# Orion-AI-Lab/KuroSiwo

Measured on AMD Instinct MI355X. Metric: SAR tiles/sec (224x224, SNUNet-ECAM change-detection train step), higher is better.
Workload: dtype bf16; 1 GPU; BASELINE.json configs[1]: SNUNet-ECAM CD, 2 dates x 2-ch GRD 224x224, per-GPU batch 32, ce+dice loss, Adam lr 1e-3, fwd+loss+bwd+optimizer; global_batch=32, base_channel=32, parallelism=dp1, hip_streams=3

## Files before the change

### include/ksmi.h

```cpp
#ifndef KSMI_H
#define KSMI_H
#include <stddef.h>
#include <stdint.h>

#ifdef __cplusplus
extern "C" {
#endif

#define KSMI_ABI_VERSION 7
#define KSMI_F32 0
#define KSMI_BF16 1
#define KSMI_E_ARG (-1)
#define KSMI_E_UNSUPPORTED (-2)
#define KSMI_MAX_SRC 6
#define KSMI_MAX_CHUNKS 72

int ksmi_abi_version(void);
const char* ksmi_last_error(void);
int ksmi_set_knob(const char* name, const char* value);
int ksmi_chunk_elems(int dtype);

#define KSMI_OP_CALL 0
#define KSMI_OP_ORDER 1
#define KSMI_OP_WAIT_SIDE 2
// ... 163 lines not shown
                              void* dout_g, const void* out, const void* z, const float* mean, const float* rstd, const float* gamma,
                              void* dz, double count, int64_t npix, int C, int dtype, void* stream);
int ksmi_bn_bwd_fin_apply_add(float* partial, int rows, int Cstride, float* sums, float* dgamma, float* dbeta, int accumulate,
                              void* r_di, const void* g, const void* i, const float* mean, const float* rstd, const float* gamma,
                              float* bias_partial, int bias_rows, double count, int64_t npix, int C, int dtype, void* stream);
int ksmi_channel_sum(const void* x, float* partial, int rows, int64_t npix, int C, int dtype, void* stream);
int ksmi_colsum(const void* x, int64_t rows, int C, float* out, int accumulate, int dtype, void* stream);

int ksmi_maxpool2x2_forward(const void* x, void* y, int B, int H, int W, int C, int dtype, void* stream);
int ksmi_maxpool2x2_backward(const void* x, const void* dy, void* dx, int accumulate,
                             int B, int H, int W, int C, int dtype, void* stream);

int ksmi_ecam_pool(const void* const x[4], float* avg, float* mx, int32_t* argmax,
                   float* workspace, int B, int HW, int C, int dtype, void* stream);
size_t ksmi_ecam_pool_workspace(int B, int HW, int C);
int ksmi_ecam_mlp(const float* avg, const float* mx, const float* ca_fc1, const float* ca_fc2,
                  const float* ca1_fc1, const float* ca1_fc2, float* ca, float* ca1,
                  float* hidden , int B, int C, void* stream);
int ksmi_ecam_final_forward(const void* const x[4], const float* ca, const float* ca1, const float* wf,
                            const float* bias, float* logits, int B, int HW, int C, int ncls, int dtype, void* stream);
int ksmi_ecam_final_backward_reduce(const void* const x[4], const float* dlogits, const float* ca, const float* ca1,
                                    const float* wf, float* dca, float* dca1, float* dwf, float* dbias,
                                    float* workspace, int B, int HW, int C, int ncls, int dtype, void* stream);
size_t ksmi_ecam_bwd_workspace(int B, int HW, int C, int ncls);
int ksmi_ecam_mlp_backward(const float* avg, const float* mx, const float* hidden, const float* ca, const float* ca1,
                           const float* dca, const float* dca1, const float* ca_fc1, const float* ca_fc2,
                           const float* ca1_fc1, const float* ca1_fc2, float* davg, float* dmax,
                           float* g_ca_fc1, float* g_ca_fc2, float* g_ca1_fc1, float* g_ca1_fc2,
                           float* workspace, int B, int C, void* stream);
size_t ksmi_ecam_mlp_bwd_workspace(int B, int C);
int ksmi_ecam_final_backward_dx(void* const dx[4], const float* dlogits, const float* ca, const float* wf,
                                const float* davg, const float* dmax, const int32_t* argmax,
                                int B, int HW, int C, int ncls, int dtype, void* stream);

size_t ksmi_loss_workspace(int B, int HW);
int ksmi_ce_dice_forward(const float* logits, const int64_t* labels, const float* class_w, int with_dice,
                         float* out3, float* workspace, int B, int HW, int ignore_index, void* stream);
int ksmi_ce_dice_backward(const float* logits, const int64_t* labels, const float* class_w, int with_dice,
                          const float* workspace, const float* grad_scale ,
                          float* dlogits, int B, int HW, int ignore_index, void* stream);

#define KSMI_LOSS_DICE 1
#define KSMI_LOSS_LOVASZ 2
#define KSMI_LOSS_FOCAL 3
size_t ksmi_seg_loss_workspace(int kind, int B, int HW);
int ksmi_seg_loss_forward(int kind, const float* logits, const int64_t* labels, const float* class_w, float gamma, float* out3,
                          void* workspace, int B, int HW, int ignore_index, void* stream);
int ksmi_seg_loss_backward(int kind, const float* logits, const int64_t* labels, const float* class_w, float gamma,
                           const void* workspace, const float* grad_scale ,
                           float* dlogits, int B, int HW, int ignore_index, void* stream);

int ksmi_argmax_confusion(const float* logits, const int64_t* labels, int64_t* pred , int64_t* cm,
                          int B, int C, int HW, int ignore_index, void* stream);
int ksmi_argmax_confusion_grouped(const float* logits, const int64_t* labels, int64_t* pred , int64_t* cm ,
                                  const int32_t* slot_a, int64_t* cms_a, const int32_t* slot_b, int64_t* cms_b,
                                  int B, int C, int HW, int ignore_index, void* stream);

int ksmi_adam_step(float* p, const float* g, float* m, float* v, int64_t n, int64_t* step_count,
                   float lr, float beta1, float beta2, float eps, float weight_decay, float grad_scale, void* stream);
int ksmi_adamw_step(float* p, const float* g, float* m, float* v, int64_t n, int64_t* step_count,
                    float lr, float beta1, float beta2, float eps, float weight_decay, float grad_scale, void* stream);
int ksmi_adam_step_mirror(float* p, const float* g, float* m, float* v, int64_t n, int64_t* step_count,
                          float lr, float beta1, float beta2, float eps, float weight_decay, float grad_scale, int decoupled,
                          void* mirror_bf16, void* stream);
int ksmi_sgd_step(float* p, const float* g, float* mom, int64_t n, int64_t* step_count,
                  float lr, float momentum, float weight_decay, float grad_scale, void* stream);
// ... 62 lines not shown
int ksmi_bnrelu_bwd_apply_scaled(void* dout_g, const void* out, const void* z, const float* mean, const float* rstd, const float* gamma,
                                 const float* sums, void* dz, double count, int64_t npix, int C, float alpha, int dtype, void* stream);
int ksmi_absdiff_forward(const void* a, const void* b, void* y, int64_t n, int dtype, void* stream);
int ksmi_absdiff_backward(const void* a, const void* b, const void* dy, void* da, void* db, int accumulate_a, int accumulate_b, int64_t n,
                          int dtype, void* stream);
int ksmi_sr_attention_forward_drop(const void* q, const void* kv, void* out, int B, int Nq, int Nk, int H, int C, float scale,
                                   uint32_t drop_thr, float drop_inv_keep, uint32_t site, const uint32_t* rng_state, int dtype, void* stream);
int ksmi_sr_attention_backward_drop(const void* q, const void* kv, const void* out, const void* dout, void* dq, void* dkv, void* workspace,
                                    int B, int Nq, int Nk, int H, int C, float scale, uint32_t drop_thr, float drop_inv_keep, uint32_t site,
                                    const uint32_t* rng_state, int dtype, void* stream);
int ksmi_bilinear_forward(const void* x, const void* add, void* y, int B, int Hi, int Wi, int Ho, int Wo, int C, int dtype, void* stream);
int ksmi_bilinear_backward(const void* dy, void* dx, int accumulate, int B, int Hi, int Wi, int Ho, int Wo, int C, int dtype, void* stream);
int ksmi_bn_bwd_reduce(const void* dy, const void* x, const float* mean, const float* rstd, float* partial, int rows, int64_t npix, int C,
                       int dtype, void* stream);
int ksmi_bn_bwd_apply(const void* dy, const void* r, const float* mean, const float* rstd, const float* gamma, const float* sums,
                      void* dv, int relu_mask, double count, int64_t npix, int C, int dtype, void* stream);
int ksmi_maxpool3x3s2_forward(const void* x, void* y, int B, int H, int W, int C, int dtype, void* stream);
int ksmi_maxpool3x3s2_backward(const void* x, const void* dy, void* dx, int accumulate, int B, int H, int W, int C, int dtype, void* stream);
int ksmi_maxpool3x3s2_forward_idx(const void* x, void* y, void* idx, int B, int H, int W, int C, int dtype, void* stream);
int ksmi_maxpool3x3s2_backward_idx(const void* idx, const void* dy, void* dx, int accumulate, int B, int H, int W, int C, int dtype, void* stream);
int ksmi_affine(const void* x, const float* scale, const float* shift, void* y, int64_t npix, int C, int relu, float alpha, int dtype,
                void* stream);
int ksmi_out_to_nchw(const void* x, float* y, int B, int C, int Cs, int64_t HW, int act, int dtype, void* stream);
int ksmi_dout_to_nhwc(const float* dy, const float* y, void* dx, int B, int C, int Cs, int64_t HW, int act, int dtype, void* stream);

int ksmi_cast_bf16(const float* src, void* dst, int64_t n, void* stream);
int ksmi_up_gemm_supported(int B, int H, int W, int C, int dtype);
int ksmi_up_wgrad_supported(int B, int H, int W, int C, int dtype);
int ksmi_up_pack_weight(const float* wt, void* wb, int C, void* stream);
#define KSMI_UP_PACK_MAX 16
int ksmi_up_pack_weights_batched(const float* const* wt, void* const* wb, const int* C, int n, void* stream);
int ksmi_up_forward(const void* x, const void* wb, const float* bias, void* y, int B, int H, int W, int C, void* stream);
int ksmi_up_dgrad(const void* dy, const void* wb, void* dx, int accumulate, int B, int H, int W, int C, void* stream);
size_t ksmi_up_wgrad_workspace(int B, int H, int W, int C);
int ksmi_up_wgrad(const void* x, const void* dy, float* workspace, float* grad, int accumulate, int B, int H, int W, int C, void* stream);

int ksmi_gemm_nt(const void* x, int x_rs, const void* w, int w_rs, const float* bias, const void* resid, int r_rs, void* y, int y_rs,
                 int rows, int K, int N, void* stream);
int ksmi_gemm_nn(const void* dy, int dy_rs, const void* w, int w_rs, void* dx, int dx_rs, int rows, int K, int N, int accumulate, void* stream);

int ksmi_bmm_f32(const float* a, const float* b, const float* bias, float* c, int nb1, int nb2, int M, int N, int K,
                 const int64_t* a_strides, const int64_t* b_strides, const int64_t* c_strides, float alpha, int accumulate, void* stream);
int ksmi_softmax_rows_f32(const float* x, float* y, int64_t rows, int n, float scale, void* stream);
int ksmi_softmax_rows_backward_f32(const float* y, const float* dy, float* dx, int64_t rows, int n, float scale, void* stream);
int ksmi_semantic_tokens_forward(const void* x, const float* wa, const float* pos, float* tokens, float* stats, int B, int dates, int N,
                                 int C, int L, int dtype, void* stream);
int ksmi_semantic_tokens_backward(const void* x, const float* wa, const float* stats, const float* dtokens, void* dx, float* dwa_partial,
                                  int B, int dates, int N, int C, int L, int accumulate, int dtype, void* stream);
int ksmi_token_cross_forward(const void* x, const float* gamma, const float* beta, const float* A, const float* Bv, const float* bo, void* y,
                             int B, int dates, int N, int C, int heads, int L, float scale, int dtype, void* stream);
size_t ksmi_token_cross_bwd_workspace(int B, int dates, int N);
int ksmi_token_cross_backward(const void* x, const float* gamma, const float* beta, const float* A, const float* Bv, void* g, float* dA,
                              float* dBv, float* dgamma, float* dbeta, float* dbo, int accumulate_ln, int accumulate_bo, float* workspace,
                              int B, int dates, int N, int C, int heads, int L, float scale, int dtype, void* stream);

int ksmi_sar_preprocess(const float* x, const float* mean, const float* stdv, float* y, int B, int C, int64_t HW, float clamp_input, void* stream);
int ksmi_augment_views(const float* x, const int32_t* params, const int32_t* fallback, const float* mean, const float* stdv, float* y, int B, int C,
                       int H, int W, float clamp_input, uint32_t mult_thr, float mult_lo, float mult_hi, uint32_t gauss_thr, float gauss_var_lo,
                       float gauss_var_hi, uint32_t cut_thr, int cut_holes, int cut_h, int cut_w, int op_order, const uint32_t* rng_state,
                       void* stream);
int ksmi_augment_masks(const void* x, void* y, const int32_t* params, const int32_t* fallback, int32_t* count, int B, int H, int W, int elem_bytes,
                       void* stream);

typedef struct ksmi_tiff_info {
  int32_t width, height, bands;
  int32_t bits, sample_format;
// ... 26 lines not shown
```

### kurosiwo_amd/_lib.py

```python
import ctypes as C
import os

_HERE = os.path.dirname(os.path.abspath(__file__))
LIB_PATH = os.path.join(_HERE, "libksmi.so")

KSMI_F32, KSMI_BF16 = 0, 1
LOSS_DICE, LOSS_LOVASZ, LOSS_FOCAL = 1, 2, 3
MAX_SRC, MAX_CHUNKS = 6, 72
ABI_VERSION = 7


class KsmiError(RuntimeError):
    pass


class Src(C.Structure):
    _fields_ = [("ptr", C.c_void_p), ("scale", C.c_void_p), ("shift", C.c_void_p),
                ("C", C.c_int32), ("c_off", C.c_int32), ("c_len", C.c_int32), ("relu", C.c_int32)]


class Dst(C.Structure):
    _fields_ = [("ptr", C.c_void_p), ("C", C.c_int32), ("c_off", C.c_int32), ("n_begin", C.c_int32),
                ("n_len", C.c_int32), ("accumulate", C.c_int32), ("pad_", C.c_int32)]

# ... 96 lines not shown
    "ksmi_bn_finalize": (_i, [_vp, _i, _i, _i, _d, _vp, _vp, _vp, _vp, _vp, _f, _f, _i, _vp, _vp, _vp, _vp, _vp]),
    "ksmi_bn_add_relu": (_i, [_vp, _vp, _vp, _vp, _vp, _i64, _i, _i, _vp]),
    "ksmi_bn_fused_supported": (_i, [_i, _i, _i]),
    "ksmi_bn_fused_max_rows": (_i, []),
    "ksmi_bn_fin_add_relu": (_i, [_vp, _i, _i, _i, _d, _vp, _vp, _vp, _vp, _vp, _f, _f, _vp, _vp, _vp, _vp, _vp, _vp, _vp, _vp, _i, _i, _i, _i, _vp]),
    "ksmi_bn_bwd_fin_apply_gated": (_i, [_vp, _i, _i, _vp, _vp, _vp, _i, _vp, _vp, _vp, _vp, _vp, _vp, _d, _i64, _i, _i, _vp]),
    "ksmi_bnrelu_bwd_fin_apply": (_i, [_vp, _i, _i, _vp, _vp, _vp, _i, _vp, _vp, _vp, _vp, _vp, _vp, _vp, _d, _i64, _i, _i, _vp]),
    "ksmi_bn_bwd_fin_apply_add": (_i, [_vp, _i, _i, _vp, _vp, _vp, _i, _vp, _vp, _vp, _vp, _vp, _vp, _vp, _i, _d, _i64, _i, _i, _vp]),
    "ksmi_bnrelu_bwd_reduce": (_i, [_vp, _vp, _vp, _vp, _vp, _vp, _i, _i64, _i, _i, _vp]),
    "ksmi_reduce_rows": (_i, [_vp, _i, _i, _i, _i, _vp, _vp, _vp, _i, _vp]),
    "ksmi_reduce_rows_batched": (_i, [_vp, _i, _vp]),
    "ksmi_reduce_rows_batched_wide": (_i, [_vp, _i, _i, _vp]),
    "ksmi_bnrelu_bwd_apply": (_i, [_vp, _vp, _vp, _vp, _vp, _vp, _vp, _vp, _d, _i64, _i, _i, _vp]),
    "ksmi_bn_bwd_apply_gated": (_i, [_vp, _vp, _vp, _vp, _vp, _vp, _vp, _d, _i64, _i, _i, _vp]),
    "ksmi_bn_bwd_apply_add": (_i, [_vp, _vp, _vp, _vp, _vp, _vp, _vp, _vp, _i, _d, _i64, _i, _i, _vp]),
    "ksmi_channel_sum": (_i, [_vp, _vp, _i, _i64, _i, _i, _vp]),
    "ksmi_colsum": (_i, [_vp, _i64, _i, _vp, _i, _i, _vp]),
    "ksmi_gather_rows": (_i, [_vp, _vp, _i, _vp, _vp, _i, _i, _i, _i, _i, _i, _vp]),
    "ksmi_scatter_rows": (_i, [_vp, _vp, _vp, _i, _vp, _vp, _i, _i, _i, _i, _i, _vp]),
    "ksmi_batch_sum": (_i, [_vp, _vp, _i, _i64, _i, _i, _vp]),
    "ksmi_mse_workspace": (C.c_size_t, []),
    "ksmi_mse_loss": (_i, [_vp, _vp, _vp, _f, _vp, _vp, _vp, _i64, _i, _vp]),
    "ksmi_maxpool2x2_forward": (_i, [_vp, _vp, _i, _i, _i, _i, _i, _vp]),
    "ksmi_maxpool2x2_backward": (_i, [_vp, _vp, _vp, _i, _i, _i, _i, _i, _i, _vp]),
    "ksmi_ecam_pool": (_i, [_P4, _vp, _vp, _vp, _vp, _i, _i, _i, _i, _vp]),
    "ksmi_ecam_pool_workspace": (_sz, [_i, _i, _i]),
    "ksmi_ecam_mlp": (_i, [_vp, _vp, _vp, _vp, _vp, _vp, _vp, _vp, _vp, _i, _i, _vp]),
    "ksmi_ecam_final_forward": (_i, [_P4, _vp, _vp, _vp, _vp, _vp, _i, _i, _i, _i, _i, _vp]),
    "ksmi_ecam_final_backward_reduce": (_i, [_P4, _vp, _vp, _vp, _vp, _vp, _vp, _vp, _vp, _vp, _i, _i, _i, _i, _i, _vp]),
    "ksmi_ecam_bwd_workspace": (_sz, [_i, _i, _i, _i]),
    "ksmi_ecam_mlp_backward": (_i, [_vp] * 18 + [_i, _i, _vp]),
    "ksmi_ecam_mlp_bwd_workspace": (_sz, [_i, _i]),
    "ksmi_ecam_final_backward_dx": (_i, [_P4, _vp, _vp, _vp, _vp, _vp, _vp, _i, _i, _i, _i, _i, _vp]),
    "ksmi_loss_workspace": (_sz, [_i, _i]),
    "ksmi_ce_dice_forward": (_i, [_vp, _vp, _vp, _i, _vp, _vp, _i, _i, _i, _vp]),
    "ksmi_ce_dice_backward": (_i, [_vp, _vp, _vp, _i, _vp, _vp, _vp, _i, _i, _i, _vp]),
    "ksmi_seg_loss_workspace": (_sz, [_i, _i, _i]),
    "ksmi_seg_loss_forward": (_i, [_i, _vp, _vp, _vp, _f, _vp, _vp, _i, _i, _i, _vp]),
    "ksmi_seg_loss_backward": (_i, [_i, _vp, _vp, _vp, _f, _vp, _vp, _vp, _i, _i, _i, _vp]),
    "ksmi_argmax_confusion": (_i, [_vp, _vp, _vp, _vp, _i, _i, _i, _i, _vp]),
    "ksmi_argmax_confusion_grouped": (_i, [_vp, _vp, _vp, _vp, _vp, _vp, _vp, _vp, _i, _i, _i, _i, _vp]),
    "ksmi_adam_step": (_i, [_vp, _vp, _vp, _vp, _i64, _vp, _f, _f, _f, _f, _f, _f, _vp]),
    "ksmi_adamw_step": (_i, [_vp, _vp, _vp, _vp, _i64, _vp, _f, _f, _f, _f, _f, _f, _vp]),
    "ksmi_adam_step_mirror": (_i, [_vp, _vp, _vp, _vp, _i64, _vp, _f, _f, _f, _f, _f, _f, _i, _vp, _vp]),
    "ksmi_sgd_step": (_i, [_vp, _vp, _vp, _i64, _vp, _f, _f, _f, _f, _vp]),
    "ksmi_layernorm_forward": (_i, [_vp, _vp, _vp, _vp, _vp, _vp, _i, _i, _f, _i, _vp]),
    "ksmi_layernorm_bwd_blocks": (_i, [_i]),
    "ksmi_layernorm_backward": (_i, [_vp, _vp, _vp, _vp, _vp, _vp, _i, _vp, _i, _i, _i, _vp]),
    "ksmi_gelu_forward": (_i, [_vp, _vp, _i64, _i, _vp]),
    "ksmi_gelu_backward": (_i, [_vp, _vp, _vp, _i64, _i, _vp]),
    "ksmi_add": (_i, [_vp, _vp, _vp, _i64, _i, _vp]),
    "ksmi_relu_backward": (_i, [_vp, _vp, _vp, _i64, _i, _vp]),
    "ksmi_relu_forward": (_i, [_vp, _vp, _i64, _i, _vp]),
    "ksmi_sar_preprocess": (_i, [_vp, _vp, _vp, _vp, _i, _i, _i64, C.c_float, _vp]),
    "ksmi_augment_views": (_i, [_vp, _vp, _vp, _vp, _vp, _vp, _i, _i, _i, _i, _f, C.c_uint32, _f, _f, C.c_uint32, _f, _f, C.c_uint32, _i, _i, _i, _i, _vp, _vp]),
    "ksmi_augment_masks": (_i, [_vp, _vp, _vp, _vp, _vp, _i, _i, _i, _i, _vp]),
    "ksmi_bmm_f32": (_i, [_vp, _vp, _vp, _vp, _i, _i, _i, _i, _i, C.POINTER(C.c_int64), C.POINTER(C.c_int64), C.POINTER(C.c_int64), C.c_float, _i, _vp]),
    "ksmi_softmax_rows_f32": (_i, [_vp, _vp, _i64, _i, C.c_float, _vp]),
    "ksmi_softmax_rows_backward_f32": (_i, [_vp, _vp, _vp, _i64, _i, C.c_float, _vp]),
    "ksmi_semantic_tokens_forward": (_i, [_vp, _vp, _vp, _vp, _vp, _i, _i, _i, _i, _i, _i, _vp]),
    "ksmi_semantic_tokens_backward": (_i, [_vp, _vp, _vp, _vp, _vp, _vp, _i, _i, _i, _i, _i, _i, _i, _vp]),
    "ksmi_token_cross_forward": (_i, [_vp, _vp, _vp, _vp, _vp, _vp, _vp, _i, _i, _i, _i, _i, _i, C.c_float, _i, _vp]),
    "ksmi_token_cross_bwd_workspace": (_sz, [_i, _i, _i]),
    "ksmi_token_cross_backward": (_i, [_vp, _vp, _vp, _vp, _vp, _vp, _vp, _vp, _vp, _vp, _vp, _i, _i, _vp, _i, _i, _i, _i, _i, _i, C.c_float, _i, _vp]),
    "ksmi_tiff_info_read": (_i, [C.c_char_p, C.POINTER(TiffInfo)]),
    "ksmi_tiff_read_f32": (_i, [C.c_char_p, _vp, _i64, C.POINTER(TiffInfo)]),
    "ksmi_tiff_read_native": (_i, [C.c_char_p, _vp, _i64, C.POINTER(TiffInfo)]),
    "ksmi_tile_batch_read": (_i, [C.POINTER(C.c_char_p), _i, _vp, _i, _i, _i]),
    "ksmi_tile_batch_read_bands": (_i, [C.POINTER(C.c_char_p), _i, _vp, _i, _i, _i, _i]),
    "ksmi_tiles_fill_nodata": (_i, [_vp, _i, _i, _i, _i]),
    "ksmi_cast_bf16": (_i, [_vp, _vp, _i64, _vp]),
    "ksmi_up_gemm_supported": (_i, [_i, _i, _i, _i, _i]),
    "ksmi_up_wgrad_supported": (_i, [_i, _i, _i, _i, _i]),
    "ksmi_up_pack_weight": (_i, [_vp, _vp, _i, _vp]),
    "ksmi_up_pack_weights_batched": (_i, [_vp, _vp, _vp, _i, _vp]),
    "ksmi_up_forward": (_i, [_vp, _vp, _vp, _vp, _i, _i, _i, _i, _vp]),
    "ksmi_up_dgrad": (_i, [_vp, _vp, _vp, _i, _i, _i, _i, _i, _vp]),
    "ksmi_up_wgrad_workspace": (C.c_size_t, [_i, _i, _i, _i]),
    "ksmi_up_wgrad": (_i, [_vp, _vp, _vp, _vp, _i, _i, _i, _i, _i, _vp]),
    "ksmi_gemm_nt": (_i, [_vp, _i, _vp, _i, _vp, _vp, _i, _vp, _i, _i, _i, _i, _vp]),
    "ksmi_gemm_nn": (_i, [_vp, _i, _vp, _i, _vp, _i, _i, _i, _i, _i, _vp]),
    "ksmi_im2col": (_i, [_vp, _vp] + [_i] * 11 + [_i, _i, _vp]),
    "ksmi_col2im": (_i, [_vp, _vp, _i] + [_i] * 11 + [_i, _vp]),
    "ksmi_im2col_tc": (_i, [_vp, _vp] + [_i] * 11 + [_i, _vp]),
    "ksmi_col2im_tc": (_i, [_vp, _vp, _i] + [_i] * 11 + [_i, _vp]),
    "ksmi_weight_to_tc": (_i, [_vp, _vp, _i, _i, _i, _i, _i, _vp]),
    "ksmi_grad_from_tc": (_i, [_vp, _vp, _i, _i, _i, _i, _i, _vp]),
    "ksmi_maxpool3x3s2_forward": (_i, [_vp, _vp, _i, _i, _i, _i, _i, _vp]),
    "ksmi_maxpool3x3s2_backward": (_i, [_vp, _vp, _vp, _i, _i, _i, _i, _i, _i, _vp]),
    "ksmi_maxpool3x3s2_forward_idx": (_i, [_vp, _vp, _vp, _i, _i, _i, _i, _i, _vp]),
    "ksmi_maxpool3x3s2_backward_idx": (_i, [_vp, _vp, _vp, _i, _i, _i, _i, _i, _i, _vp]),
    "ksmi_affine": (_i, [_vp, _vp, _vp, _vp, _i64, _i, _i, C.c_float, _i, _vp]),
    "ksmi_dwconv3x3_gelu_forward": (_i, [_vp, _vp, _vp, _vp, _vp, _i, _i, _i, _i, _i, _vp]),
    "ksmi_dwconv3x3_gelu_forward_drop": (_i, [_vp, _vp, _vp, _vp, _vp, _i, _i, _i, _i, C.c_uint32, C.c_float, C.c_uint32, _vp, _i, _vp]),
    "ksmi_gelu_backward_drop": (_i, [_vp, _vp, _vp, _i64, C.c_uint32, C.c_float, C.c_uint32, _vp, _i, _vp]),
    "ksmi_dwconv3x3_backward_input": (_i, [_vp, _vp, _vp, _i, _i, _i, _i, _i, _vp]),
    "ksmi_dwconv3x3_wgrad": (_i, [_vp, _vp, _vp, _i, _i, _i, _i, _i, _i, _vp]),
    "ksmi_sr_attention_forward": (_i, [_vp, _vp, _vp, _i, _i, _i, _i, _i, C.c_float, _i, _vp]),
    "ksmi_sr_attention_bwd_workspace": (C.c_size_t, [_i, _i, _i, _i, _i]),
    "ksmi_sr_attention_backward": (_i, [_vp, _vp, _vp, _vp, _vp, _vp, _vp, _i, _i, _i, _i, _i, C.c_float, _i, _vp]),
    "ksmi_attention_bwd_workspace": (C.c_size_t, [_i, _i, _i, _i, _i]),
    "ksmi_rng_advance": (_i, [_vp, _vp]),
    "ksmi_bn_relu_drop2d": (_i, [_vp, _vp, _vp, _vp, _i, _i64, _i, C.c_uint32, C.c_float, C.c_uint32, _vp, _i, _vp]),
    "ksmi_reduce_rows_scaled": (_i, [_vp, _i, _i, _i, _i, _vp, _vp, _vp, _i, C.c_float, _vp]),
    "ksmi_bnrelu_bwd_apply_scaled": (_i, [_vp, _vp, _vp, _vp, _vp, _vp, _vp, _vp, _d, _i64, _i, C.c_float, _i, _vp]),
    "ksmi_absdiff_forward": (_i, [_vp, _vp, _vp, _i64, _i, _vp]),
    "ksmi_absdiff_backward": (_i, [_vp, _vp, _vp, _vp, _vp, _i, _i, _i64, _i, _vp]),
    "ksmi_dropout_apply": (_i, [_vp, _vp, _vp, _i64, _i, _i, C.c_uint32, C.c_float, C.c_uint32, C.c_uint32, C.c_float, C.c_uint32, _vp, _i, _vp]),
    "ksmi_sr_attention_forward_drop": (_i, [_vp, _vp, _vp, _i, _i, _i, _i, _i, C.c_float, C.c_uint32, C.c_float, C.c_uint32, _vp, _i, _vp]),
    "ksmi_sr_attention_backward_drop": (_i, [_vp, _vp, _vp, _vp, _vp, _vp, _vp, _i, _i, _i, _i, _i, C.c_float, C.c_uint32, C.c_float, C.c_uint32,
# ... 83 lines not shown
```

### kurosiwo_amd/csrc/gemm2.hip

```cpp
#include "common.h"
#include "../../include/ksmi.h"
#include "errors.h"
#include "igemm_epilogue.h"

namespace {

struct Gemm2P {
  const bf16_t* a; int a_rs;
  const bf16_t* w; int w_rs;
  const float* bias; const bf16_t* resid; int r_rs;
  bf16_t* out; int o_rs;
  int rows, red, cols, accumulate;
  int mtiles, ntiles;
  int map_a, map_o, up_H, up_W, up_C, bias_mod;
};

__device__ __forceinline__ size_t up_row_base(int m, int H, int W, int C) {
  const int x = m % W, t = m / W, y = t % H, b = t / H;
  return ((size_t)(b * 2 * H + 2 * y) * (size_t)(2 * W) + (size_t)(2 * x)) * (size_t)C;
}
__device__ __forceinline__ size_t up_col_off(int c, int W, int C) { return c < 2 * C ? (size_t)c : (size_t)(c - 2 * C) + (size_t)(2 * W) * (size_t)C; }


__device__ __forceinline__ void glds16(const unsigned char* src, unsigned dst_wave_base) {
  unsigned keep;
  dst_wave_base = __builtin_amdgcn_readfirstlane(dst_wave_base);
  asm volatile("s_mov_b32 %0, m0\n\ts_mov_b32 m0, %2\n\ts_nop 0\n\tglobal_load_lds_dwordx4 %1, off\n\ts_mov_b32 m0, %0"
               : "=&s"(keep) : "v"(src), "s"(dst_wave_base) : "memory");
}
__device__ __forceinline__ void vm_wait(int n) {
#define KSMI_VMW(k) case k: asm volatile("s_waitcnt vmcnt(" #k ")" ::: "memory"); break;
  switch (n) {
    KSMI_VMW(1) KSMI_VMW(2) KSMI_VMW(3) KSMI_VMW(4) KSMI_VMW(5) KSMI_VMW(6) KSMI_VMW(7) KSMI_VMW(8) KSMI_VMW(9) KSMI_VMW(10)
    KSMI_VMW(11) KSMI_VMW(12) KSMI_VMW(13) KSMI_VMW(14) KSMI_VMW(15) KSMI_VMW(16) KSMI_VMW(17) KSMI_VMW(18) KSMI_VMW(19) KSMI_VMW(20)
    KSMI_VMW(21) KSMI_VMW(22) KSMI_VMW(23) KSMI_VMW(24) KSMI_VMW(25) KSMI_VMW(26) KSMI_VMW(27) KSMI_VMW(28) KSMI_VMW(29) KSMI_VMW(30)
    default: asm volatile("s_waitcnt vmcnt(0)" ::: "memory"); break;
  }
#undef KSMI_VMW
}
__device__ __forceinline__ void lgkm_wait0() { __builtin_amdgcn_s_waitcnt(0xC07F); }
__device__ __forceinline__ void lds_barrier() {
  lgkm_wait0();
  __builtin_amdgcn_s_barrier();
  asm volatile("" ::: "memory");
}

__device__ __forceinline__ int sw_a(int row) { return (row & 1) | ((row & 2) << 2); }
__device__ __forceinline__ int sw_b(int row) { return (row & 3) << 1; }
template <int MT> __device__ __forceinline__ int sw_bt(int row) { return MT == 3 ? 0 : sw_b(row); }

template <int MT>
__device__ __forceinline__ void store_row2(const Gemm2P& p, const f32x4 (&acc)[4][MT], int mt, int m, int c0, const float* bias16) {
  if (m >= p.rows) return;
  float v[16];
#pragma unroll
  for (int t = 0; t < 4; ++t)
#pragma unroll
    for (int r = 0; r < 4; ++r) v[t * 4 + r] = acc[t][mt][r] + bias16[t * 4 + r];
  bf16_t* op = p.map_o ? p.out + up_row_base(m, p.up_H, p.up_W, p.up_C) + up_col_off(c0, p.up_W, p.up_C) : p.out + (size_t)m * p.o_rs + c0;
  if (p.resid) {
    float a[8], b[8];
    vec_unpack<bf16_t>(*(const u32x4*)(p.resid + (size_t)m * p.r_rs + c0), a);
    vec_unpack<bf16_t>(*(const u32x4*)(p.resid + (size_t)m * p.r_rs + c0 + 8), b);
#pragma unroll
    for (int j = 0; j < 8; ++j) { v[j] += a[j]; v[8 + j] += b[j]; }
  }
  if (p.accumulate) {
    float a[8], b[8];
    vec_unpack<bf16_t>(*(const u32x4*)op, a);
    vec_unpack<bf16_t>(*(const u32x4*)(op + 8), b);
#pragma unroll
    for (int j = 0; j < 8; ++j) { v[j] += a[j]; v[8 + j] += b[j]; }
  }
  *(u32x4*)op = vec_pack<bf16_t>(v);
  *(u32x4*)(op + 8) = vec_pack<bf16_t>(v + 8);
}

template <int MT, bool TRW, int NS>
__global__ __launch_bounds__(256, 1) void gemm2_kernel(const Gemm2P p) {
  constexpr int TM = 32 * MT, KS = 64, XB = TM * 128, WB = 128 * 128, STAGE = XB + WB;
  constexpr int NQ = STAGE / 1024, NI = NQ / 4;
  extern __shared__ __attribute__((aligned(16))) unsigned char smem[];
  const int tid = threadIdx.x, lane = tid & 63, wave = tid >> 6, g = lane >> 4, l15 = lane & 15;
  const int wn = wave >> 1, wm = wave & 1;
  const unsigned t = xcd_remap(blockIdx.x, gridDim.x);
  const int mt_i = t / p.ntiles, nt_i = t - mt_i * p.ntiles;
  const int m0 = mt_i * TM, n0 = nt_i * 128;
  const int nsteps = p.red / KS;
  const unsigned lds0 = (unsigned)(uintptr_t)smem;

  const unsigned char* src[NI];
  int step_bytes[NI];
  size_t jump[NI];
  const int jump_step = p.map_a ? (2 * p.up_C) / KS : 0x7fffffff;
#pragma unroll
  for (int i = 0; i < NI; ++i) {
    const int q = wave + 4 * i;
    jump[i] = 0;
    if (q * 8 < TM) {
      const int row = q * 8 + (lane >> 3), slot = lane & 7;
      const int chunk = slot ^ ((row >> 1) & 7);
      int m = m0 + row; if (m >= p.rows) m = p.rows - 1;
      src[i] = (const unsigned char*)(p.a + (p.map_a ? up_row_base(m, p.up_H, p.up_W, p.up_C) : (size_t)m * p.a_rs) + chunk * 8);
      step_bytes[i] = KS * 2;
      jump[i] = p.map_a ? ((size_t)(2 * p.up_W) * p.up_C - (size_t)(2 * p.up_C)) * 2 : 0;
    } else if constexpr (!TRW) {
      const int j = q * 8 - TM + (lane >> 3), slot = lane & 7;
      const int chunk = slot ^ ((j >> 1) & 7);
      const int h = j >> 6, jj = j & 63;
      int n = n0 + h * 64 + ((jj >> 2) & 3) * 16 + (jj >> 4) * 4 + (jj & 3); if (n >= p.cols) n = p.cols - 1;
      src[i] = (const unsigned char*)(p.w + (size_t)n * p.w_rs + chunk * 8);
// ... 64 lines not shown

  const int pre = nsteps < NS ? nsteps : NS;
  for (int s = 0; s < pre; ++s) issue(s, s);
  vm_wait((pre - 1) * NI);
  lds_barrier();
  u32x4 fwA[4], fxA[MT], fwB[4], fxB[MT];
  load_frags(0, 0, fwA, fxA);
  int cur = 0;
  for (int s = 0; s + 1 < nsteps; ++s) {
    lgkm_wait0();
    __builtin_amdgcn_sched_barrier(0);
    load_frags(cur, 1, fwB, fxB);
    __builtin_amdgcn_sched_barrier(0);
    mma_all(acc, fwA, fxA);
    __builtin_amdgcn_sched_barrier(0);
    if (s + NS <= nsteps) vm_wait((NS - 2) * NI); else vm_wait((nsteps - s - 2) * NI);
    lds_barrier();
    if (s + NS < nsteps) issue(s + NS, cur);
    cur = cur + 1 == NS ? 0 : cur + 1;
    load_frags(cur, 0, fwA, fxA);
    __builtin_amdgcn_sched_barrier(0);
    mma_all(acc2, fwB, fxB);
    __builtin_amdgcn_sched_barrier(0);
  }
  load_frags(cur, 1, fwB, fxB);
  mma_all(acc, fwA, fxA);
  mma_all(acc2, fwB, fxB);
#pragma unroll
  for (int a = 0; a < 4; ++a)
#pragma unroll
    for (int b = 0; b < MT; ++b) acc[a][b] += acc2[a][b];

  const int c0 = n0 + wn * 64 + g * 16;
  if (c0 >= p.cols) return;
  float bias16[16];
#pragma unroll
  for (int j = 0; j < 16; ++j) bias16[j] = p.bias ? p.bias[p.bias_mod ? (c0 + j) % p.bias_mod : c0 + j] : 0.f;
#pragma unroll
  for (int mt = 0; mt < MT; ++mt) store_row2<MT>(p, acc, mt, m0 + wm * 16 * MT + mt * 16 + l15, c0, bias16);
}

template <int MT, bool TRW, int NS>
int launch2n(const Gemm2P& p, hipStream_t st) {
  constexpr int lds = NS * (32 * MT * 128 + 128 * 128);
  static_assert(lds <= 160 * 1024, "LDS ring");
  auto kfn = gemm2_kernel<MT, TRW, NS>; KSMI_NOTE(kfn);
  static bool attr = false;
  if (!attr) { (void)hipFuncSetAttribute((const void*)kfn, hipFuncAttributeMaxDynamicSharedMemorySize, lds); attr = true; }
  hipLaunchKernelGGL(kfn, dim3(p.mtiles * p.ntiles), dim3(256), lds, st, p);
  return ksmi_check_launch(TRW ? "gemm2_nn" : "gemm2_nt");
}

struct Tile2 { int mt, ns; };
inline Tile2 pick_tile(int rows, int ntiles) {
  static const int f_mt = ksmi_knob_int("KSMI_GEMM2_MT", 0);
  static const int f_ns = ksmi_knob_int("KSMI_GEMM2_NS", 0);
  static const struct { int mt, ns, slots; double round_us; } cand[] = {
      {2, 3, 512, 13.0}, {4, 3, 256, 13.8}, {2, 2, 768, 15.5}, {3, 2, 512, 16.0}, {5, 3, 256, 16.3}, {6, 3, 256, 18.0},
      {4, 2, 512, 19.0}, {7, 3, 256, 21.0}, {8, 3, 256, 23.0}};
  Tile2 best = {4, 3}; double bc = 1e30;
  for (const auto& c : cand) {
    if ((f_mt && c.mt != f_mt) || (f_ns && f_ns <= 3 && c.ns != f_ns)) continue;
    const long wgs = (long)((rows + 32 * c.mt - 1) / (32 * c.mt)) * ntiles;
    const double cost = (double)((wgs + c.slots - 1) / c.slots) * c.round_us;
    if (cost < bc) { bc = cost; best = {c.mt, c.ns}; }
  }
  if (f_mt && bc == 1e30) best = {f_mt, f_mt >= 5 ? 3 : 2};
  if (f_ns) best.ns = f_ns;
  return best;
}

template <int MT, bool TRW>
int launch2(const Gemm2P& p, int ns, hipStream_t st) {
  constexpr int stage = 32 * MT * 128 + 128 * 128;
  if (ns <= 2) return launch2n<MT, TRW, 2>(p, st);
  if constexpr (5 * stage <= 160 * 1024) { if (ns >= 5) return launch2n<MT, TRW, 5>(p, st); }
  if constexpr (4 * stage <= 160 * 1024) { if (ns >= 4) return launch2n<MT, TRW, 4>(p, st); }
  return launch2n<MT, TRW, 3>(p, st);
}

template <bool TRW>
int dispatch2(Gemm2P& p, hipStream_t st) {
  p.ntiles = p.cols / 128;
  const Tile2 t = pick_tile(p.rows, p.ntiles);
  p.mtiles = (p.rows + 32 * t.mt - 1) / (32 * t.mt);
  switch (t.mt) {
    case 2: return launch2<2, TRW>(p, t.ns, st);
    case 3: return launch2<3, TRW>(p, t.ns, st);
    case 4: return launch2<4, TRW>(p, t.ns, st);
    case 5: return launch2<5, TRW>(p, t.ns, st);
    case 6: return launch2<6, TRW>(p, t.ns, st);
    case 7: return launch2<7, TRW>(p, t.ns, st);
    default: return launch2<8, TRW>(p, t.ns, st);
  }
}

struct Gemm2T {
  const bf16_t* a; int a_rs, a_cols;
  const bf16_t* b; int b_rs, b_cols;
  float* out; int64_t o_rs; int64_t split_stride; int accumulate;
  int rows, rows_per_split, atiles, btiles;
  const unsigned char* zero;
  float* bias; int bias_acc;
  int map_a, up_H, up_W, up_C;
  float* bias_rows; int64_t bias_rs;
};
__device__ __attribute__((aligned(64))) unsigned char gemm2_zero_page[64];
KSMI_DEVICE_SYMBOL_GETTER(gemm2_zero, gemm2_zero_page)

template <int MT, int NS, int SPL, bool BIASA = false>
__global__ __launch_bounds__(256 * SPL, 1) void gemm2_tn_kernel(const Gemm2T p) {
  static_assert(!BIASA || SPL == 1, "A-side column sums: one wave group");
  constexpr int TB = 32 * MT, KS = 64, AB = 64 * 256, BROW = TB * 2, BB = 64 * BROW, STAGE = AB + BB;
  constexpr int NQ = STAGE / 1024, NI = NQ / 4, BGM = BROW / 32 - 1, AU = 16, BU = BROW / 16;
  static_assert(NQ % 4 == 0, "whole DMA rounds");
  extern __shared__ __attribute__((aligned(16))) unsigned char smem[];
  const int tid = threadIdx.x, lane = tid & 63, wave_all = tid >> 6, g = lane >> 4, l15 = lane & 15;
  const int grp = SPL == 1 ? 0 : wave_all >> 2, wave = wave_all & 3;
  const int wn = wave >> 1, wm = wave & 1;
  const int tile = blockIdx.x, split = blockIdx.y;
  const int bt = tile / p.atiles, at = tile - bt * p.atiles;
  const int a0 = at * 128, b0 = bt * TB;
  const int wg_begin = split * p.rows_per_split;
  const int wg_end = min(p.rows, wg_begin + p.rows_per_split);
  const int steps_wg = (max(wg_end - wg_begin, 0) + KS - 1) / KS;
  const int nsteps = (steps_wg + SPL - 1) / SPL;
  const int m_begin = wg_begin + grp * nsteps * KS;
// ... 183 lines not shown
}

}

int ksmi_gemm2_nt(const void* x, int x_rs, const void* w, int w_rs, const float* bias, const void* resid, int r_rs, void* y, int y_rs,
                  int rows, int K, int N, hipStream_t st) {
  static const bool off = ksmi_knob_is_set("KSMI_GEMM2_OFF");
  if (off || K % 64 || N % 128 || rows < 64 || K < 128) return 1;
  Gemm2P p = {(const bf16_t*)x, x_rs, (const bf16_t*)w, w_rs, bias, (const bf16_t*)resid, r_rs, (bf16_t*)y, y_rs, rows, K, N, 0, 0, 0};
  return dispatch2<false>(p, st);
}

int ksmi_gemm2_nn(const void* dy, int dy_rs, const void* w, int w_rs, void* dx, int dx_rs, int rows, int K, int N, int accumulate,
                  hipStream_t st) {
  static const bool off = ksmi_knob_is_set("KSMI_GEMM2_OFF");
  if (off || N % 64 || K % 128 || rows < 64 || N < 128) return 1;
  Gemm2P p = {(const bf16_t*)dy, dy_rs, (const bf16_t*)w, w_rs, nullptr, nullptr, 0, (bf16_t*)dx, dx_rs, rows, N, K, accumulate, 0, 0};
  return dispatch2<true>(p, st);
}

int ksmi_gemm2_up_forward(const void* x, const void* wb, const float* bias, void* y, int B, int H, int W, int C, hipStream_t st) {
  if (C % 64 || C < 128 || B * H * W < 64) return 1;
  Gemm2P p = {(const bf16_t*)x, C, (const bf16_t*)wb, C, bias, nullptr, 0, (bf16_t*)y, 0, B * H * W, C, 4 * C, 0, 0, 0};
  p.map_o = 1; p.up_H = H; p.up_W = W; p.up_C = C; p.bias_mod = C;
  return dispatch2<false>(p, st);
}
int ksmi_gemm2_up_dgrad(const void* dy, const void* wb, void* dx, int accumulate, int B, int H, int W, int C, hipStream_t st) {
  if (C % 128 || C < 128 || B * H * W < 64) return 1;
  Gemm2P p = {(const bf16_t*)dy, 0, (const bf16_t*)wb, C, nullptr, nullptr, 0, (bf16_t*)dx, C, B * H * W, 4 * C, C, accumulate, 0, 0};
  p.map_a = 1; p.up_H = H; p.up_W = W; p.up_C = C;
  return dispatch2<true>(p, st);
}

template <int MT, int NS, int SPL = 1, bool BIASA = false>
static void launch_tn(dim3 grid, const Gemm2T& p, hipStream_t st) {
  constexpr int lds = SPL * NS * (64 * 256 + 64 * 64 * MT);
  static_assert(lds <= 160 * 1024, "LDS ring");
  static_assert(SPL == 1 || (4 * MT + MT) * 256 * 16 <= lds, "exchange area");
  auto kfn = gemm2_tn_kernel<MT, NS, SPL, BIASA>; KSMI_NOTE(kfn);
  static bool attr = false;
  if (!attr) { (void)hipFuncSetAttribute((const void*)kfn, hipFuncAttributeMaxDynamicSharedMemorySize, lds); attr = true; }
  hipLaunchKernelGGL(kfn, grid, dim3(256 * SPL), lds, st, p);
}

bool ksmi_gemm2_tn_spl(int tiles_times_splits, int steps_per_split) {
  static const int f = ksmi_knob_int("KSMI_TN_SPL", 0);
  if (f <= 0) return false;
  if (f == 1) return steps_per_split >= 2;
  return tiles_times_splits <= 256 && steps_per_split >= 12;
}

bool ksmi_gemm2_tn_enabled(int K, int N, int rows_per_split) {
  static const bool off = ksmi_knob_is_set("KSMI_GEMM2_OFF") || ksmi_knob_is_set("KSMI_GEMM2_TN_OFF");
  return !(off || K % 8 || N % 8 || K < 64 || N < 64 || rows_per_split % 64);
}

int ksmi_gemm2_tn(const void* x, int x_rs, const void* dy, int dy_rs, float* slab, int npad, float* grad, int64_t g_rs, int rows, int K, int N,
                  int Kslab, int nsplit, int rows_per_split, int btile, int accumulate, float* bias_grad, int bias_accumulate, hipStream_t st) {
  if (!ksmi_gemm2_tn_enabled(K, N, rows_per_split)) return 1;
  const unsigned char* const zero_page = gemm2_zero();
  if (!zero_page) return ksmi_fail(KSMI_E_UNSUPPORTED, "gemm2: zero page");
  Gemm2T p = {};
  p.rows = rows; p.rows_per_split = rows_per_split; p.zero = zero_page;
  if (nsplit == 1 && grad) {
    p.a = (const bf16_t*)x; p.a_rs = x_rs; p.a_cols = K; p.b = (const bf16_t*)dy; p.b_rs = dy_rs; p.b_cols = N;
    p.out = grad; p.o_rs = g_rs; p.split_stride = 0; p.accumulate = accumulate;
// ... 117 lines not shown
  if (rc) return rc;
  launch_up_wgrad_reduce(slab, nsplit, C, grad, accumulate, st);
  return ksmi_check_launch("up_wgrad_reduce");
}

extern "C" {
int ksmi_up_gemm_supported(int B, int H, int W, int C, int dtype) {
  static const bool off = ksmi_knob_is_set("KSMI_GEMM2_OFF");
  return !off && dtype == KSMI_BF16 && C >= 128 && C % 128 == 0 && (int64_t)B * H * W >= 64 && (int64_t)B * H * W * 112 < ((int64_t)1 << 32) ? 1 : 0;
}
int ksmi_up_wgrad_supported(int B, int H, int W, int C, int dtype) {
  static const bool off = ksmi_knob_is_set("KSMI_GEMM2_OFF");
  return !off && dtype == KSMI_BF16 && C >= 64 && C % 64 == 0 && (int64_t)B * H * W >= 64 && (int64_t)B * H * W * 112 < ((int64_t)1 << 32) ? 1 : 0;
}
int ksmi_up_pack_weight(const float* wt, void* wb, int C, void* stream) { return ksmi_gemm2_up_pack(wt, wb, C, (hipStream_t)stream); }
int ksmi_up_pack_weights_batched(const float* const* wt, void* const* wb, const int* C, int n, void* stream) {
  if (!wt || !wb || !C || n < 1 || n > KSMI_UP_PACK_MAX) return ksmi_fail(KSMI_E_ARG, "up_pack_weights_batched: 1 .. KSMI_UP_PACK_MAX tensors");
  UpPackBatch b = {};
  for (int i = 0; i < n; ++i) {
    if (!wt[i] || !wb[i] || C[i] < 1) return ksmi_fail(KSMI_E_ARG, "up_pack_weights_batched: bad entry");
    b.wt[i] = wt[i]; b.wb[i] = (bf16_t*)wb[i]; b.C[i] = C[i];
  }
  hipLaunchKernelGGL(up_pack_batched_kernel, dim3(256, n), dim3(256), 0, (hipStream_t)stream, b);
  return ksmi_check_launch("up_pack_weights_batched");
}
int ksmi_up_forward(const void* x, const void* wb, const float* bias, void* y, int B, int H, int W, int C, void* stream) {
  const int rc = ksmi_gemm2_up_forward(x, wb, bias, y, B, H, W, C, (hipStream_t)stream);
  return rc == 1 ? ksmi_fail(KSMI_E_UNSUPPORTED, "up_forward: shape not covered (ksmi_up_gemm_supported)") : rc;
}
int ksmi_up_dgrad(const void* dy, const void* wb, void* dx, int accumulate, int B, int H, int W, int C, void* stream) {
  const int rc = ksmi_gemm2_up_dgrad(dy, wb, dx, accumulate, B, H, W, C, (hipStream_t)stream);
  return rc == 1 ? ksmi_fail(KSMI_E_UNSUPPORTED, "up_dgrad: shape not covered (ksmi_up_gemm_supported)") : rc;
}
size_t ksmi_up_wgrad_workspace(int B, int H, int W, int C) { return ksmi_gemm2_up_wgrad_workspace(B, H, W, C); }
int ksmi_up_wgrad(const void* x, const void* dy, float* workspace, float* grad, int accumulate, int B, int H, int W, int C, void* stream) {
  const int rc = ksmi_gemm2_up_wgrad(x, dy, workspace, grad, accumulate, B, H, W, C, (hipStream_t)stream);
  return rc == 1 ? ksmi_fail(KSMI_E_UNSUPPORTED, "up_wgrad: shape not covered (ksmi_up_gemm_supported)") : rc;
}
}
```

### kurosiwo_amd/csrc/head.hip

```cpp
#include "common.h"
#include "../../include/ksmi.h"
#include "errors.h"

namespace {

constexpr int kThreads = 256;
constexpr int kPoolSplit = 64;
constexpr int kBwdSplit = 64;

template <typename T>
__global__ __launch_bounds__(256) void ecam_pool_kernel(const T* x0, const T* x1, const T* x2, const T* x3,
                                                        float* psum, float* pmax, int* pidx, int HW, int C) {
  constexpr int VEC = ElemTraits<T>::kVec;
  const int CV = C / VEC;
  const int npl = kThreads / CV;
  const int b = blockIdx.y, sp = blockIdx.x, S = gridDim.x;
  const int cv = threadIdx.x % CV, pl = threadIdx.x / CV;
  const bool active = (int)threadIdx.x < npl * CV;
  const int per = (HW + S - 1) / S;
  const int p0 = sp * per, p1 = min(HW, p0 + per);
  const T* xs[4] = {x0, x1, x2, x3};
  float s[5][VEC], m[5][VEC];
  int mi[5][VEC];
#pragma unroll
// ... 346 lines not shown
  int i = blockIdx.x * blockDim.x + threadIdx.x;
  if (i < C4 * H1) {
    const int j = i % H1, c = i / H1;
    float a = 0.f;
    for (int b = 0; b < B; ++b) a += ds[b * C5 + c] * (hidden[(size_t)b * 2 * HT + j] + hidden[(size_t)b * 2 * HT + HT + j]);
    gw2[i] = a;
    return;
  }
  i -= C4 * H1;
  if (i < C * H2) {
    const int j = i % H2, c = i / H2;
    float a = 0.f;
    for (int b = 0; b < B; ++b) a += ds[b * C5 + C4 + c] * (hidden[(size_t)b * 2 * HT + H1 + j] + hidden[(size_t)b * 2 * HT + HT + H1 + j]);
    gv2[i] = a;
    return;
  }
  i -= C * H2;
  if (i < H1 * C4) {
    const int c = i % C4, j = i / C4;
    float a = 0.f;
    for (int b = 0; b < B; ++b) a += dh[(b * 2 + 0) * HT + j] * avg[b * C5 + c] + dh[(b * 2 + 1) * HT + j] * mx[b * C5 + c];
    gw1[i] = a;
    return;
  }
  i -= H1 * C4;
  if (i < H2 * C) {
    const int c = i % C, j = i / C;
    float a = 0.f;
    for (int b = 0; b < B; ++b) a += dh[(b * 2 + 0) * HT + H1 + j] * avg[b * C5 + C4 + c] + dh[(b * 2 + 1) * HT + H1 + j] * mx[b * C5 + C4 + c];
    gv1[i] = a;
  }
}

template <typename T, int NCLS>
__global__ __launch_bounds__(256) void ecam_bwd_dx_kernel(T* d0, T* d1, T* d2, T* d3, const float* dl, const float* ca,
                                                          const float* wf, const float* davg, int HW, int C) {
  constexpr int VEC = ElemTraits<T>::kVec;
  extern __shared__ float sm[];
  const int b = blockIdx.y, C4 = 4 * C;
  float* weff = sm;
  float* cst = sm + NCLS * C4;
  const float inv = 1.f / (float)HW;
  for (int i = threadIdx.x; i < NCLS * C4; i += blockDim.x) weff[i] = wf[i] * ca[(size_t)b * C4 + (i % C4)];
  for (int i = threadIdx.x; i < C4; i += blockDim.x) cst[i] = (davg[(size_t)b * 5 * C + i] + davg[(size_t)b * 5 * C + C4 + (i % C)]) * inv;
  __syncthreads();
  const int CV = C / VEC, tpp = 4 * CV;
  const int ppb = blockDim.x / tpp;
  const int q = threadIdx.x % tpp, pl = threadIdx.x / tpp;
  const int s = q / CV, c0 = (q - s * CV) * VEC;
  if (pl >= ppb) return;
  float w[NCLS][VEC], k0[VEC];
#pragma unroll
  for (int j = 0; j < VEC; ++j) {
    k0[j] = cst[s * C + c0 + j];
#pragma unroll
    for (int k = 0; k < NCLS; ++k) w[k][j] = weff[k * C4 + s * C + c0 + j];
  }
  T* dst = (s == 0 ? d0 : s == 1 ? d1 : s == 2 ? d2 : d3) + (int64_t)b * HW * C + c0;
  for (int p = blockIdx.x * ppb + pl; p < HW; p += gridDim.x * ppb) {
    float d[NCLS], v[VEC];
#pragma unroll
    for (int k = 0; k < NCLS; ++k) d[k] = dl[((int64_t)b * NCLS + k) * HW + p];
#pragma unroll
    for (int j = 0; j < VEC; ++j) {
      float a = k0[j];
#pragma unroll
      for (int k = 0; k < NCLS; ++k) a += w[k][j] * d[k];
      v[j] = a;
    }
    *(u32x4*)(dst + (int64_t)p * C) = vec_pack<T>(v);
  }
}

template <typename T>
__global__ void ecam_bwd_max_scatter_kernel(T* d0, T* d1, T* d2, T* d3, const float* dmax, const int* argmax, int B, int HW, int C) {
  const int i = blockIdx.x * blockDim.x + threadIdx.x;
  if (i >= B * C) return;
  const int b = i / C, cc = i - b * C;
  T* ds[4] = {d0, d1, d2, d3};
  for (int s = 0; s < 4; ++s) {
    const int c = s * C + cc;
    T* q = ds[s] + ((int64_t)b * HW + argmax[b * 5 * C + c]) * C + cc;
    ElemTraits<T>::st(q, ElemTraits<T>::ld(q) + dmax[b * 5 * C + c]);
  }
  const int pi = argmax[b * 5 * C + 4 * C + cc];
  const float g = dmax[b * 5 * C + 4 * C + cc];
  for (int s = 0; s < 4; ++s) {
    T* q = ds[s] + ((int64_t)b * HW + pi) * C + cc;
    ElemTraits<T>::st(q, ElemTraits<T>::ld(q) + g);
  }
}

constexpr int kLossSplit = 32;
struct Px3 { float p0, p1, p2; };
__device__ __forceinline__ Px3 softmax3(float a, float b, float c, float& lse) {
  const float m = fmaxf(a, fmaxf(b, c));
  const float e0 = expf(a - m), e1 = expf(b - m), e2 = expf(c - m);
  const float s = e0 + e1 + e2;
  lse = m + logf(s);
  const float r = 1.f / s;
  return {e0 * r, e1 * r, e2 * r};
}

__global__ __launch_bounds__(256) void ce_dice_fwd_kernel(const float* logits, const int64_t* labels, const float* cw,
                                                          float* part, int HW, int ignore_index) {
  const int b = blockIdx.y, sp = blockIdx.x, S = gridDim.x;
  const int per = (HW + S - 1) / S;
  const int p0 = sp * per, p1 = min(HW, p0 + per);
  const float w0 = cw[0], w1 = cw[1], w2 = cw[2];
  const float one = 1.0f + 1e-6f, eps = 1e-6f;
  float wn = 0.f, ws = 0.f, it = 0.f, cd = 0.f;
  const float* lg = logits + (int64_t)b * 3 * HW;
  for (int p = p0 + threadIdx.x; p < p1; p += blockDim.x) {
    const float a = lg[p], bb = lg[HW + p], c = lg[2 * HW + p];
    const int64_t t = labels[(int64_t)b * HW + p];
    float lse;
    const Px3 q = softmax3(a, bb, c, lse);
    const bool valid = t != ignore_index;
    const int t0 = valid ? (int)t : 0;
    const float xt = t0 == 0 ? a : (t0 == 1 ? bb : c);
// ... 191 lines not shown
  float* pg = workspace; float* pd = pg + (size_t)B * kBwdSplit * 3 * 4 * C;
  float* gb = pd + (size_t)B * kBwdSplit * 3; float* db = gb + (size_t)B * 3 * 4 * C;
  KSMI_DT(dtype,
          hipLaunchKernelGGL((ecam_bwd_reduce_kernel<bf16_t, 3>), dim3(kBwdSplit, B), dim3(256), 0, (hipStream_t)stream,
                             (const bf16_t*)x[0], (const bf16_t*)x[1], (const bf16_t*)x[2], (const bf16_t*)x[3], dlogits, pg, pd, HW, C),
          hipLaunchKernelGGL((ecam_bwd_reduce_kernel<float, 3>), dim3(kBwdSplit, B), dim3(256), 0, (hipStream_t)stream,
                             (const float*)x[0], (const float*)x[1], (const float*)x[2], (const float*)x[3], dlogits, pg, pd, HW, C));
  int rc = ksmi_check_launch("ecam_bwd_reduce");
  if (rc) return rc;
  hipLaunchKernelGGL(ecam_bwd_finish_kernel<3>, dim3(B), dim3(256), (size_t)(3 * 4 * C + 3) * sizeof(float), (hipStream_t)stream, pg, pd, ca, ca1,
                     wf, dca, dca1, gb, db, kBwdSplit, C);
  hipLaunchKernelGGL(ecam_bwd_wf_kernel<3>, dim3((3 * 4 * C + 255) / 256), dim3(256), 0, (hipStream_t)stream, gb, db, ca, ca1, dwf, dbias, B, C);
  return ksmi_check_launch("ecam_bwd_finish");
}

size_t ksmi_ecam_mlp_bwd_workspace(int B, int C) {
  return ((size_t)B * 5 * C + (size_t)B * 2 * ((4 * C) / 16 + C / 4)) * sizeof(float);
}

int ksmi_ecam_mlp_backward(const float* avg, const float* mx, const float* hidden, const float* ca, const float* ca1,
                           const float* dca, const float* dca1, const float* ca_fc1, const float* ca_fc2, const float* ca1_fc1,
                           const float* ca1_fc2, float* davg, float* dmax, float* g_ca_fc1, float* g_ca_fc2, float* g_ca1_fc1,
                           float* g_ca1_fc2, float* workspace, int B, int C, void* stream) {
  if (C % 16 || !workspace) return ksmi_fail(KSMI_E_ARG, "ecam_mlp_backward: bad args");
  const int C4 = 4 * C, HT = C4 / 16 + C / 4;
  hipLaunchKernelGGL(ecam_mlp_bwd_kernel, dim3(B), dim3(256), (size_t)(5 * C + 2 * HT) * sizeof(float), (hipStream_t)stream, hidden, ca, ca1, dca,
                     dca1, ca_fc1, ca_fc2, ca1_fc1, ca1_fc2, davg, dmax, workspace, B, C);
  const int items = 2 * (C4 * (C4 / 16) + C * (C / 4));
  hipLaunchKernelGGL(ecam_mlp_wgrad_kernel, dim3((items + 255) / 256), dim3(256), 0, (hipStream_t)stream, avg, mx, hidden, workspace, g_ca_fc1,
                     g_ca_fc2, g_ca1_fc1, g_ca1_fc2, B, C);
  return ksmi_check_launch("ecam_mlp_bwd");
}

int ksmi_ecam_final_backward_dx(void* const dx[4], const float* dlogits, const float* ca, const float* wf, const float* davg,
                                const float* dmax, const int32_t* argmax, int B, int HW, int C, int ncls, int dtype, void* stream) {
  if (ncls != 3 || !ecam_c_ok(C, dtype)) return ksmi_fail(KSMI_E_UNSUPPORTED, "ecam_final_bwd_dx: ncls must be 3");
  const size_t lds = (size_t)(3 * 4 * C + 4 * C) * sizeof(float);
  const int tpp = 4 * C / (dtype == KSMI_BF16 ? 8 : 4);
  if (tpp > 256) return ksmi_fail(KSMI_E_UNSUPPORTED, "ecam_final_bwd_dx: C too large for the (pixel, source, vector) thread map");
  const int ppb = 256 / tpp, trips = 8;
  int gx = (HW + ppb * trips - 1) / (ppb * trips);
  if (gx < 1) gx = 1;
  const dim3 grid(gx, B);
  KSMI_DT(dtype,
          hipLaunchKernelGGL((ecam_bwd_dx_kernel<bf16_t, 3>), grid, dim3(256), lds, (hipStream_t)stream, (bf16_t*)dx[0], (bf16_t*)dx[1],
                             (bf16_t*)dx[2], (bf16_t*)dx[3], dlogits, ca, wf, davg, HW, C),
          hipLaunchKernelGGL((ecam_bwd_dx_kernel<float, 3>), grid, dim3(256), lds, (hipStream_t)stream, (float*)dx[0], (float*)dx[1],
                             (float*)dx[2], (float*)dx[3], dlogits, ca, wf, davg, HW, C));
  int rc = ksmi_check_launch("ecam_bwd_dx");
  if (rc) return rc;
  const int tot = B * C;
  KSMI_DT(dtype,
          hipLaunchKernelGGL(ecam_bwd_max_scatter_kernel<bf16_t>, dim3((tot + 255) / 256), dim3(256), 0, (hipStream_t)stream,
                             (bf16_t*)dx[0], (bf16_t*)dx[1], (bf16_t*)dx[2], (bf16_t*)dx[3], dmax, argmax, B, HW, C),
          hipLaunchKernelGGL(ecam_bwd_max_scatter_kernel<float>, dim3((tot + 255) / 256), dim3(256), 0, (hipStream_t)stream,
                             (float*)dx[0], (float*)dx[1], (float*)dx[2], (float*)dx[3], dmax, argmax, B, HW, C));
  return ksmi_check_launch("ecam_bwd_max_scatter");
}

size_t ksmi_loss_workspace(int B, int HW) { (void)HW; return ((size_t)B * kLossSplit * 4 + 1 + 2 * (size_t)B) * sizeof(float); }

int ksmi_ce_dice_forward(const float* logits, const int64_t* labels, const float* class_w, int with_dice, float* out3,
                         float* workspace, int B, int HW, int ignore_index, void* stream) {
  if (!logits || !labels || !class_w || !out3 || !workspace || B < 1 || HW < 1) return ksmi_fail(KSMI_E_ARG, "ce_dice_forward: bad args");
  float* part = workspace; float* coef = workspace + (size_t)B * kLossSplit * 4;
  hipLaunchKernelGGL(ce_dice_fwd_kernel, dim3(kLossSplit, B), dim3(256), 0, (hipStream_t)stream, logits, labels, class_w, part, HW, ignore_index);
  hipLaunchKernelGGL(ce_dice_finish_kernel, dim3(1), dim3(64), 0, (hipStream_t)stream, part, coef, out3, B, kLossSplit, with_dice);
  return ksmi_check_launch("ce_dice_fwd");
}

int ksmi_ce_dice_backward(const float* logits, const int64_t* labels, const float* class_w, int with_dice, const float* workspace,
                          const float* grad_scale, float* dlogits, int B, int HW, int ignore_index, void* stream) {
  if (!logits || !labels || !class_w || !dlogits || !workspace) return ksmi_fail(KSMI_E_ARG, "ce_dice_backward: bad args");
  const float* coef = workspace + (size_t)B * kLossSplit * 4;
  const dim3 grid((HW + 255) / 256 > 128 ? 128 : (HW + 255) / 256, B);
  hipLaunchKernelGGL(ce_dice_bwd_kernel, grid, dim3(256), 0, (hipStream_t)stream, logits, labels, class_w, coef, grad_scale, dlogits, HW,
                     ignore_index, with_dice);
  return ksmi_check_launch("ce_dice_bwd");
}

int ksmi_argmax_confusion(const float* logits, const int64_t* labels, int64_t* pred, int64_t* cm, int B, int C, int HW,
                          int ignore_index, void* stream) {
  if (!logits || !labels || !cm || C < 1 || C > 4) return ksmi_fail(KSMI_E_ARG, "argmax_confusion: 1 <= C <= 4");
  const dim3 grid((HW + 255) / 256 > 128 ? 128 : (HW + 255) / 256, B);
  hipLaunchKernelGGL(argmax_confusion_kernel, grid, dim3(256), 0, (hipStream_t)stream, logits, labels, pred, (unsigned long long*)cm, C, HW, ignore_index);
  return ksmi_check_launch("argmax_confusion");
}

int ksmi_argmax_confusion_grouped(const float* logits, const int64_t* labels, int64_t* pred, int64_t* cm, const int32_t* slot_a,
                                  int64_t* cms_a, const int32_t* slot_b, int64_t* cms_b, int B, int C, int HW, int ignore_index,
// ... 11 lines not shown
```

### kurosiwo_amd/csrc/thunks_gen.h

```cpp
#pragma once
#include <stddef.h>
#include <stdint.h>
#include <string.h>

typedef int (*ksmi_thunk_fn)(const void* fn, const uint64_t* a, void* stream);
static inline float ksmi_slot_f32(uint64_t v) { uint32_t w = (uint32_t)v; float f; memcpy(&f, &w, 4); return f; }
static inline double ksmi_slot_f64(uint64_t v) { double d; memcpy(&d, &v, 8); return d; }

static int ksmi_thunk_0(const void* fn, const uint64_t* a, void* st) {
  typedef int (*F)(int, void*, void*, void*, float, void*, void*, int, int, int, void*);
  (void)a; return ((F)fn)((int)(int64_t)a[0], (void*)(uintptr_t)a[1], (void*)(uintptr_t)a[2], (void*)(uintptr_t)a[3], ksmi_slot_f32(a[4]), (void*)(uintptr_t)a[5], (void*)(uintptr_t)a[6], (int)(int64_t)a[7], (int)(int64_t)a[8], (int)(int64_t)a[9], st);
}
static int ksmi_thunk_1(const void* fn, const uint64_t* a, void* st) {
  typedef int (*F)(int, void*, void*, void*, float, void*, void*, void*, int, int, int, void*);
  (void)a; return ((F)fn)((int)(int64_t)a[0], (void*)(uintptr_t)a[1], (void*)(uintptr_t)a[2], (void*)(uintptr_t)a[3], ksmi_slot_f32(a[4]), (void*)(uintptr_t)a[5], (void*)(uintptr_t)a[6], (void*)(uintptr_t)a[7], (int)(int64_t)a[8], (int)(int64_t)a[9], (int)(int64_t)a[10], st);
}
static int ksmi_thunk_2(const void* fn, const uint64_t* a, void* st) {
  typedef int (*F)(int, void*, void*, void*, size_t, void*, void*);
  (void)a; return ((F)fn)((int)(int64_t)a[0], (void*)(uintptr_t)a[1], (void*)(uintptr_t)a[2], (void*)(uintptr_t)a[3], (size_t)a[4], (void*)(uintptr_t)a[5], st);
}
static int ksmi_thunk_3(const void* fn, const uint64_t* a, void* st) {
  typedef int (*F)(void*, void*);
  (void)a; return ((F)fn)((void*)(uintptr_t)a[0], st);
}
// ... 132 lines not shown
static int ksmi_thunk_37(const void* fn, const uint64_t* a, void* st) {
  typedef int (*F)(void*, void*, void*, int, int, int, int, int, float, int, void*);
  (void)a; return ((F)fn)((void*)(uintptr_t)a[0], (void*)(uintptr_t)a[1], (void*)(uintptr_t)a[2], (int)(int64_t)a[3], (int)(int64_t)a[4], (int)(int64_t)a[5], (int)(int64_t)a[6], (int)(int64_t)a[7], ksmi_slot_f32(a[8]), (int)(int64_t)a[9], st);
}
static int ksmi_thunk_38(const void* fn, const uint64_t* a, void* st) {
  typedef int (*F)(void*, void*, void*, int, int, int, int, int, float, unsigned int, float, unsigned int, void*, int, void*);
  (void)a; return ((F)fn)((void*)(uintptr_t)a[0], (void*)(uintptr_t)a[1], (void*)(uintptr_t)a[2], (int)(int64_t)a[3], (int)(int64_t)a[4], (int)(int64_t)a[5], (int)(int64_t)a[6], (int)(int64_t)a[7], ksmi_slot_f32(a[8]), (unsigned int)a[9], ksmi_slot_f32(a[10]), (unsigned int)a[11], (void*)(uintptr_t)a[12], (int)(int64_t)a[13], st);
}
static int ksmi_thunk_39(const void* fn, const uint64_t* a, void* st) {
  typedef int (*F)(void*, void*, void*, int, int, int, int, int, int, void*);
  (void)a; return ((F)fn)((void*)(uintptr_t)a[0], (void*)(uintptr_t)a[1], (void*)(uintptr_t)a[2], (int)(int64_t)a[3], (int)(int64_t)a[4], (int)(int64_t)a[5], (int)(int64_t)a[6], (int)(int64_t)a[7], (int)(int64_t)a[8], st);
}
static int ksmi_thunk_40(const void* fn, const uint64_t* a, void* st) {
  typedef int (*F)(void*, void*, void*, int, int, int, int, int, int, int, void*);
  (void)a; return ((F)fn)((void*)(uintptr_t)a[0], (void*)(uintptr_t)a[1], (void*)(uintptr_t)a[2], (int)(int64_t)a[3], (int)(int64_t)a[4], (int)(int64_t)a[5], (int)(int64_t)a[6], (int)(int64_t)a[7], (int)(int64_t)a[8], (int)(int64_t)a[9], st);
}
static int ksmi_thunk_41(const void* fn, const uint64_t* a, void* st) {
  typedef int (*F)(void*, void*, void*, int, int, int, long long, int, int, void*);
  (void)a; return ((F)fn)((void*)(uintptr_t)a[0], (void*)(uintptr_t)a[1], (void*)(uintptr_t)a[2], (int)(int64_t)a[3], (int)(int64_t)a[4], (int)(int64_t)a[5], (long long)a[6], (int)(int64_t)a[7], (int)(int64_t)a[8], st);
}
static int ksmi_thunk_42(const void* fn, const uint64_t* a, void* st) {
  typedef int (*F)(void*, void*, void*, int, void*, void*, int, int, int, void*);
  (void)a; return ((F)fn)((void*)(uintptr_t)a[0], (void*)(uintptr_t)a[1], (void*)(uintptr_t)a[2], (int)(int64_t)a[3], (void*)(uintptr_t)a[4], (void*)(uintptr_t)a[5], (int)(int64_t)a[6], (int)(int64_t)a[7], (int)(int64_t)a[8], st);
}
static int ksmi_thunk_43(const void* fn, const uint64_t* a, void* st) {
  typedef int (*F)(void*, void*, void*, int, void*, void*, int, int, int, int, int, void*);
  (void)a; return ((F)fn)((void*)(uintptr_t)a[0], (void*)(uintptr_t)a[1], (void*)(uintptr_t)a[2], (int)(int64_t)a[3], (void*)(uintptr_t)a[4], (void*)(uintptr_t)a[5], (int)(int64_t)a[6], (int)(int64_t)a[7], (int)(int64_t)a[8], (int)(int64_t)a[9], (int)(int64_t)a[10], st);
}
static int ksmi_thunk_44(const void* fn, const uint64_t* a, void* st) {
  typedef int (*F)(void*, void*, void*, int, void*, void*, void*, int, int, int, void*);
  (void)a; return ((F)fn)((void*)(uintptr_t)a[0], (void*)(uintptr_t)a[1], (void*)(uintptr_t)a[2], (int)(int64_t)a[3], (void*)(uintptr_t)a[4], (void*)(uintptr_t)a[5], (void*)(uintptr_t)a[6], (int)(int64_t)a[7], (int)(int64_t)a[8], (int)(int64_t)a[9], st);
}
static int ksmi_thunk_45(const void* fn, const uint64_t* a, void* st) {
  typedef int (*F)(void*, void*, void*, long long, int, void*);
  (void)a; return ((F)fn)((void*)(uintptr_t)a[0], (void*)(uintptr_t)a[1], (void*)(uintptr_t)a[2], (long long)a[3], (int)(int64_t)a[4], st);
}
static int ksmi_thunk_46(const void* fn, const uint64_t* a, void* st) {
  typedef int (*F)(void*, void*, void*, long long, int, float, void*);
  (void)a; return ((F)fn)((void*)(uintptr_t)a[0], (void*)(uintptr_t)a[1], (void*)(uintptr_t)a[2], (long long)a[3], (int)(int64_t)a[4], ksmi_slot_f32(a[5]), st);
}
static int ksmi_thunk_47(const void* fn, const uint64_t* a, void* st) {
  typedef int (*F)(void*, void*, void*, long long, int, int, unsigned int, float, unsigned int, unsigned int, float, unsigned int, void*, int, void*);
  (void)a; return ((F)fn)((void*)(uintptr_t)a[0], (void*)(uintptr_t)a[1], (void*)(uintptr_t)a[2], (long long)a[3], (int)(int64_t)a[4], (int)(int64_t)a[5], (unsigned int)a[6], ksmi_slot_f32(a[7]), (unsigned int)a[8], (unsigned int)a[9], ksmi_slot_f32(a[10]), (unsigned int)a[11], (void*)(uintptr_t)a[12], (int)(int64_t)a[13], st);
}
static int ksmi_thunk_48(const void* fn, const uint64_t* a, void* st) {
  typedef int (*F)(void*, void*, void*, long long, void*, float, float, float, float, void*);
  (void)a; return ((F)fn)((void*)(uintptr_t)a[0], (void*)(uintptr_t)a[1], (void*)(uintptr_t)a[2], (long long)a[3], (void*)(uintptr_t)a[4], ksmi_slot_f32(a[5]), ksmi_slot_f32(a[6]), ksmi_slot_f32(a[7]), ksmi_slot_f32(a[8]), st);
}
static int ksmi_thunk_49(const void* fn, const uint64_t* a, void* st) {
  typedef int (*F)(void*, void*, void*, long long, unsigned int, float, unsigned int, void*, int, void*);
  (void)a; return ((F)fn)((void*)(uintptr_t)a[0], (void*)(uintptr_t)a[1], (void*)(uintptr_t)a[2], (long long)a[3], (unsigned int)a[4], ksmi_slot_f32(a[5]), (unsigned int)a[6], (void*)(uintptr_t)a[7], (int)(int64_t)a[8], st);
}
static int ksmi_thunk_50(const void* fn, const uint64_t* a, void* st) {
  typedef int (*F)(void*, void*, void*, void*, int, int, int, int, void*);
  (void)a; return ((F)fn)((void*)(uintptr_t)a[0], (void*)(uintptr_t)a[1], (void*)(uintptr_t)a[2], (void*)(uintptr_t)a[3], (int)(int64_t)a[4], (int)(int64_t)a[5], (int)(int64_t)a[6], (int)(int64_t)a[7], st);
}
static int ksmi_thunk_51(const void* fn, const uint64_t* a, void* st) {
  typedef int (*F)(void*, void*, void*, void*, int, int, int, int, int, void*);
  (void)a; return ((F)fn)((void*)(uintptr_t)a[0], (void*)(uintptr_t)a[1], (void*)(uintptr_t)a[2], (void*)(uintptr_t)a[3], (int)(int64_t)a[4], (int)(int64_t)a[5], (int)(int64_t)a[6], (int)(int64_t)a[7], (int)(int64_t)a[8], st);
}
static int ksmi_thunk_52(const void* fn, const uint64_t* a, void* st) {
  typedef int (*F)(void*, void*, void*, void*, int, int, int, int, int, void*, void*, void*, float, int, void*);
  (void)a; return ((F)fn)((void*)(uintptr_t)a[0], (void*)(uintptr_t)a[1], (void*)(uintptr_t)a[2], (void*)(uintptr_t)a[3], (int)(int64_t)a[4], (int)(int64_t)a[5], (int)(int64_t)a[6], (int)(int64_t)a[7], (int)(int64_t)a[8], (void*)(uintptr_t)a[9], (void*)(uintptr_t)a[10], (void*)(uintptr_t)a[11], ksmi_slot_f32(a[12]), (int)(int64_t)a[13], st);
}
static int ksmi_thunk_53(const void* fn, const uint64_t* a, void* st) {
  typedef int (*F)(void*, void*, void*, void*, int, int, long long, float, void*);
  (void)a; return ((F)fn)((void*)(uintptr_t)a[0], (void*)(uintptr_t)a[1], (void*)(uintptr_t)a[2], (void*)(uintptr_t)a[3], (int)(int64_t)a[4], (int)(int64_t)a[5], (long long)a[6], ksmi_slot_f32(a[7]), st);
}
static int ksmi_thunk_54(const void* fn, const uint64_t* a, void* st) {
  typedef int (*F)(void*, void*, void*, void*, int, long long, int, unsigned int, float, unsigned int, void*, int, void*);
  (void)a; return ((F)fn)((void*)(uintptr_t)a[0], (void*)(uintptr_t)a[1], (void*)(uintptr_t)a[2], (void*)(uintptr_t)a[3], (int)(int64_t)a[4], (long long)a[5], (int)(int64_t)a[6], (unsigned int)a[7], ksmi_slot_f32(a[8]), (unsigned int)a[9], (void*)(uintptr_t)a[10], (int)(int64_t)a[11], st);
}
static int ksmi_thunk_55(const void* fn, const uint64_t* a, void* st) {
  typedef int (*F)(void*, void*, void*, void*, long long, int, int, float, int, void*);
  (void)a; return ((F)fn)((void*)(uintptr_t)a[0], (void*)(uintptr_t)a[1], (void*)(uintptr_t)a[2], (void*)(uintptr_t)a[3], (long long)a[4], (int)(int64_t)a[5], (int)(int64_t)a[6], ksmi_slot_f32(a[7]), (int)(int64_t)a[8], st);
}
static int ksmi_thunk_56(const void* fn, const uint64_t* a, void* st) {
  typedef int (*F)(void*, void*, void*, void*, long long, void*, float, float, float, float, float, float, void*);
  (void)a; return ((F)fn)((void*)(uintptr_t)a[0], (void*)(uintptr_t)a[1], (void*)(uintptr_t)a[2], (void*)(uintptr_t)a[3], (long long)a[4], (void*)(uintptr_t)a[5], ksmi_slot_f32(a[6]), ksmi_slot_f32(a[7]), ksmi_slot_f32(a[8]), ksmi_slot_f32(a[9]), ksmi_slot_f32(a[10]), ksmi_slot_f32(a[11]), st);
}
static int ksmi_thunk_57(const void* fn, const uint64_t* a, void* st) {
  typedef int (*F)(void*, void*, void*, void*, long long, void*, float, float, float, float, float, float, int, void*, void*);
  (void)a; return ((F)fn)((void*)(uintptr_t)a[0], (void*)(uintptr_t)a[1], (void*)(uintptr_t)a[2], (void*)(uintptr_t)a[3], (long long)a[4], (void*)(uintptr_t)a[5], ksmi_slot_f32(a[6]), ksmi_slot_f32(a[7]), ksmi_slot_f32(a[8]), ksmi_slot_f32(a[9]), ksmi_slot_f32(a[10]), ksmi_slot_f32(a[11]), (int)(int64_t)a[12], (void*)(uintptr_t)a[13], st);
}
static int ksmi_thunk_58(const void* fn, const uint64_t* a, void* st) {
  typedef int (*F)(void*, void*, void*, void*, void*, int, int, int, int, void*);
  (void)a; return ((F)fn)((void*)(uintptr_t)a[0], (void*)(uintptr_t)a[1], (void*)(uintptr_t)a[2], (void*)(uintptr_t)a[3], (void*)(uintptr_t)a[4], (int)(int64_t)a[5], (int)(int64_t)a[6], (int)(int64_t)a[7], (int)(int64_t)a[8], st);
}
static int ksmi_thunk_59(const void* fn, const uint64_t* a, void* st) {
  typedef int (*F)(void*, void*, void*, void*, void*, int, int, int, int, int, void*);
  (void)a; return ((F)fn)((void*)(uintptr_t)a[0], (void*)(uintptr_t)a[1], (void*)(uintptr_t)a[2], (void*)(uintptr_t)a[3], (void*)(uintptr_t)a[4], (int)(int64_t)a[5], (int)(int64_t)a[6], (int)(int64_t)a[7], (int)(int64_t)a[8], (int)(int64_t)a[9], st);
}
static int ksmi_thunk_60(const void* fn, const uint64_t* a, void* st) {
  typedef int (*F)(void*, void*, void*, void*, void*, int, int, int, int, int, int, void*);
  (void)a; return ((F)fn)((void*)(uintptr_t)a[0], (void*)(uintptr_t)a[1], (void*)(uintptr_t)a[2], (void*)(uintptr_t)a[3], (void*)(uintptr_t)a[4], (int)(int64_t)a[5], (int)(int64_t)a[6], (int)(int64_t)a[7], (int)(int64_t)a[8], (int)(int64_t)a[9], (int)(int64_t)a[10], st);
}
static int ksmi_thunk_61(const void* fn, const uint64_t* a, void* st) {
  typedef int (*F)(void*, void*, void*, void*, void*, int, int, int, int, unsigned int, float, unsigned int, void*, int, void*);
  (void)a; return ((F)fn)((void*)(uintptr_t)a[0], (void*)(uintptr_t)a[1], (void*)(uintptr_t)a[2], (void*)(uintptr_t)a[3], (void*)(uintptr_t)a[4], (int)(int64_t)a[5], (int)(int64_t)a[6], (int)(int64_t)a[7], (int)(int64_t)a[8], (unsigned int)a[9], ksmi_slot_f32(a[10]), (unsigned int)a[11], (void*)(uintptr_t)a[12], (int)(int64_t)a[13], st);
}
static int ksmi_thunk_62(const void* fn, const uint64_t* a, void* st) {
  typedef int (*F)(void*, void*, void*, void*, void*, int, int, long long, int, void*);
  (void)a; return ((F)fn)((void*)(uintptr_t)a[0], (void*)(uintptr_t)a[1], (void*)(uintptr_t)a[2], (void*)(uintptr_t)a[3], (void*)(uintptr_t)a[4], (int)(int64_t)a[5], (int)(int64_t)a[6], (long long)a[7], (int)(int64_t)a[8], st);
}
static int ksmi_thunk_63(const void* fn, const uint64_t* a, void* st) {
  typedef int (*F)(void*, void*, void*, void*, void*, int, long long, int, int, void*);
  (void)a; return ((F)fn)((void*)(uintptr_t)a[0], (void*)(uintptr_t)a[1], (void*)(uintptr_t)a[2], (void*)(uintptr_t)a[3], (void*)(uintptr_t)a[4], (int)(int64_t)a[5], (long long)a[6], (int)(int64_t)a[7], (int)(int64_t)a[8], st);
}
static int ksmi_thunk_64(const void* fn, const uint64_t* a, void* st) {
  typedef int (*F)(void*, void*, void*, void*, void*, long long, int, int, void*);
  (void)a; return ((F)fn)((void*)(uintptr_t)a[0], (void*)(uintptr_t)a[1], (void*)(uintptr_t)a[2], (void*)(uintptr_t)a[3], (void*)(uintptr_t)a[4], (long long)a[5], (int)(int64_t)a[6], (int)(int64_t)a[7], st);
}
static int ksmi_thunk_65(const void* fn, const uint64_t* a, void* st) {
  typedef int (*F)(void*, void*, void*, void*, void*, void*, int, int, float, int, void*);
  (void)a; return ((F)fn)((void*)(uintptr_t)a[0], (void*)(uintptr_t)a[1], (void*)(uintptr_t)a[2], (void*)(uintptr_t)a[3], (void*)(uintptr_t)a[4], (void*)(uintptr_t)a[5], (int)(int64_t)a[6], (int)(int64_t)a[7], ksmi_slot_f32(a[8]), (int)(int64_t)a[9], st);
}
static int ksmi_thunk_66(const void* fn, const uint64_t* a, void* st) {
  typedef int (*F)(void*, void*, void*, void*, void*, void*, int, int, int, int, float, int, void*);
  (void)a; return ((F)fn)((void*)(uintptr_t)a[0], (void*)(uintptr_t)a[1], (void*)(uintptr_t)a[2], (void*)(uintptr_t)a[3], (void*)(uintptr_t)a[4], (void*)(uintptr_t)a[5], (int)(int64_t)a[6], (int)(int64_t)a[7], (int)(int64_t)a[8], (int)(int64_t)a[9], ksmi_slot_f32(a[10]), (int)(int64_t)a[11], st);
}
static int ksmi_thunk_67(const void* fn, const uint64_t* a, void* st) {
  typedef int (*F)(void*, void*, void*, void*, void*, void*, int, int, int, int, float, unsigned int, float, float, unsigned int, float, float, unsigned int, int, int, int, int, void*, void*);
  (void)a; return ((F)fn)((void*)(uintptr_t)a[0], (void*)(uintptr_t)a[1], (void*)(uintptr_t)a[2], (void*)(uintptr_t)a[3], (void*)(uintptr_t)a[4], (void*)(uintptr_t)a[5], (int)(int64_t)a[6], (int)(int64_t)a[7], (int)(int64_t)a[8], (int)(int64_t)a[9], ksmi_slot_f32(a[10]), (unsigned int)a[11], ksmi_slot_f32(a[12]), ksmi_slot_f32(a[13]), (unsigned int)a[14], ksmi_slot_f32(a[15]), ksmi_slot_f32(a[16]), (unsigned int)a[17], (int)(int64_t)a[18], (int)(int64_t)a[19], (int)(int64_t)a[20], (int)(int64_t)a[21], (void*)(uintptr_t)a[22], st);
}
static int ksmi_thunk_68(const void* fn, const uint64_t* a, void* st) {
  typedef int (*F)(void*, void*, void*, void*, void*, void*, int, int, int, int, int, void*);
  (void)a; return ((F)fn)((void*)(uintptr_t)a[0], (void*)(uintptr_t)a[1], (void*)(uintptr_t)a[2], (void*)(uintptr_t)a[3], (void*)(uintptr_t)a[4], (void*)(uintptr_t)a[5], (int)(int64_t)a[6], (int)(int64_t)a[7], (int)(int64_t)a[8], (int)(int64_t)a[9], (int)(int64_t)a[10], st);
}
static int ksmi_thunk_69(const void* fn, const uint64_t* a, void* st) {
  typedef int (*F)(void*, void*, void*, void*, void*, void*, int, int, int, int, int, int, int, void*);
  (void)a; return ((F)fn)((void*)(uintptr_t)a[0], (void*)(uintptr_t)a[1], (void*)(uintptr_t)a[2], (void*)(uintptr_t)a[3], (void*)(uintptr_t)a[4], (void*)(uintptr_t)a[5], (int)(int64_t)a[6], (int)(int64_t)a[7], (int)(int64_t)a[8], (int)(int64_t)a[9], (int)(int64_t)a[10], (int)(int64_t)a[11], (int)(int64_t)a[12], st);
}
static int ksmi_thunk_70(const void* fn, const uint64_t* a, void* st) {
  typedef int (*F)(void*, void*, void*, void*, void*, void*, int, long long, int, int, void*);
  (void)a; return ((F)fn)((void*)(uintptr_t)a[0], (void*)(uintptr_t)a[1], (void*)(uintptr_t)a[2], (void*)(uintptr_t)a[3], (void*)(uintptr_t)a[4], (void*)(uintptr_t)a[5], (int)(int64_t)a[6], (long long)a[7], (int)(int64_t)a[8], (int)(int64_t)a[9], st);
}
static int ksmi_thunk_71(const void* fn, const uint64_t* a, void* st) {
  typedef int (*F)(void*, void*, void*, void*, void*, void*, int, void*, int, int, int, void*);
  (void)a; return ((F)fn)((void*)(uintptr_t)a[0], (void*)(uintptr_t)a[1], (void*)(uintptr_t)a[2], (void*)(uintptr_t)a[3], (void*)(uintptr_t)a[4], (void*)(uintptr_t)a[5], (int)(int64_t)a[6], (void*)(uintptr_t)a[7], (int)(int64_t)a[8], (int)(int64_t)a[9], (int)(int64_t)a[10], st);
}
static int ksmi_thunk_72(const void* fn, const uint64_t* a, void* st) {
  typedef int (*F)(void*, void*, void*, void*, void*, void*, void*, double, long long, int, int, void*);
  (void)a; return ((F)fn)((void*)(uintptr_t)a[0], (void*)(uintptr_t)a[1], (void*)(uintptr_t)a[2], (void*)(uintptr_t)a[3], (void*)(uintptr_t)a[4], (void*)(uintptr_t)a[5], (void*)(uintptr_t)a[6], ksmi_slot_f64(a[7]), (long long)a[8], (int)(int64_t)a[9], (int)(int64_t)a[10], st);
}
static int ksmi_thunk_73(const void* fn, const uint64_t* a, void* st) {
  typedef int (*F)(void*, void*, void*, void*, void*, void*, void*, int, double, long long, int, int, void*);
  (void)a; return ((F)fn)((void*)(uintptr_t)a[0], (void*)(uintptr_t)a[1], (void*)(uintptr_t)a[2], (void*)(uintptr_t)a[3], (void*)(uintptr_t)a[4], (void*)(uintptr_t)a[5], (void*)(uintptr_t)a[6], (int)(int64_t)a[7], ksmi_slot_f64(a[8]), (long long)a[9], (int)(int64_t)a[10], (int)(int64_t)a[11], st);
}
static int ksmi_thunk_74(const void* fn, const uint64_t* a, void* st) {
  typedef int (*F)(void*, void*, void*, void*, void*, void*, void*, int, int, int, int, int, void*);
  (void)a; return ((F)fn)((void*)(uintptr_t)a[0], (void*)(uintptr_t)a[1], (void*)(uintptr_t)a[2], (void*)(uintptr_t)a[3], (void*)(uintptr_t)a[4], (void*)(uintptr_t)a[5], (void*)(uintptr_t)a[6], (int)(int64_t)a[7], (int)(int64_t)a[8], (int)(int64_t)a[9], (int)(int64_t)a[10], (int)(int64_t)a[11], st);
}
static int ksmi_thunk_75(const void* fn, const uint64_t* a, void* st) {
  typedef int (*F)(void*, void*, void*, void*, void*, void*, void*, int, int, int, int, int, float, int, void*);
  (void)a; return ((F)fn)((void*)(uintptr_t)a[0], (void*)(uintptr_t)a[1], (void*)(uintptr_t)a[2], (void*)(uintptr_t)a[3], (void*)(uintptr_t)a[4], (void*)(uintptr_t)a[5], (void*)(uintptr_t)a[6], (int)(int64_t)a[7], (int)(int64_t)a[8], (int)(int64_t)a[9], (int)(int64_t)a[10], (int)(int64_t)a[11], ksmi_slot_f32(a[12]), (int)(int64_t)a[13], st);
}
static int ksmi_thunk_76(const void* fn, const uint64_t* a, void* st) {
  typedef int (*F)(void*, void*, void*, void*, void*, void*, void*, int, int, int, int, int, float, unsigned int, float, unsigned int, void*, int, void*);
  (void)a; return ((F)fn)((void*)(uintptr_t)a[0], (void*)(uintptr_t)a[1], (void*)(uintptr_t)a[2], (void*)(uintptr_t)a[3], (void*)(uintptr_t)a[4], (void*)(uintptr_t)a[5], (void*)(uintptr_t)a[6], (int)(int64_t)a[7], (int)(int64_t)a[8], (int)(int64_t)a[9], (int)(int64_t)a[10], (int)(int64_t)a[11], ksmi_slot_f32(a[12]), (unsigned int)a[13], ksmi_slot_f32(a[14]), (unsigned int)a[15], (void*)(uintptr_t)a[16], (int)(int64_t)a[17], st);
}
static int ksmi_thunk_77(const void* fn, const uint64_t* a, void* st) {
  typedef int (*F)(void*, void*, void*, void*, void*, void*, void*, int, int, int, int, int, int, float, int, void*);
  (void)a; return ((F)fn)((void*)(uintptr_t)a[0], (void*)(uintptr_t)a[1], (void*)(uintptr_t)a[2], (void*)(uintptr_t)a[3], (void*)(uintptr_t)a[4], (void*)(uintptr_t)a[5], (void*)(uintptr_t)a[6], (int)(int64_t)a[7], (int)(int64_t)a[8], (int)(int64_t)a[9], (int)(int64_t)a[10], (int)(int64_t)a[11], (int)(int64_t)a[12], ksmi_slot_f32(a[13]), (int)(int64_t)a[14], st);
}
static int ksmi_thunk_78(const void* fn, const uint64_t* a, void* st) {
  typedef int (*F)(void*, void*, void*, void*, void*, void*, void*, void*, double, long long, int, float, int, void*);
  (void)a; return ((F)fn)((void*)(uintptr_t)a[0], (void*)(uintptr_t)a[1], (void*)(uintptr_t)a[2], (void*)(uintptr_t)a[3], (void*)(uintptr_t)a[4], (void*)(uintptr_t)a[5], (void*)(uintptr_t)a[6], (void*)(uintptr_t)a[7], ksmi_slot_f64(a[8]), (long long)a[9], (int)(int64_t)a[10], ksmi_slot_f32(a[11]), (int)(int64_t)a[12], st);
}
static int ksmi_thunk_79(const void* fn, const uint64_t* a, void* st) {
  typedef int (*F)(void*, void*, void*, void*, void*, void*, void*, void*, double, long long, int, int, void*);
  (void)a; return ((F)fn)((void*)(uintptr_t)a[0], (void*)(uintptr_t)a[1], (void*)(uintptr_t)a[2], (void*)(uintptr_t)a[3], (void*)(uintptr_t)a[4], (void*)(uintptr_t)a[5], (void*)(uintptr_t)a[6], (void*)(uintptr_t)a[7], ksmi_slot_f64(a[8]), (long long)a[9], (int)(int64_t)a[10], (int)(int64_t)a[11], st);
}
static int ksmi_thunk_80(const void* fn, const uint64_t* a, void* st) {
  typedef int (*F)(void*, void*, void*, void*, void*, void*, void*, void*, int, double, long long, int, int, void*);
  (void)a; return ((F)fn)((void*)(uintptr_t)a[0], (void*)(uintptr_t)a[1], (void*)(uintptr_t)a[2], (void*)(uintptr_t)a[3], (void*)(uintptr_t)a[4], (void*)(uintptr_t)a[5], (void*)(uintptr_t)a[6], (void*)(uintptr_t)a[7], (int)(int64_t)a[8], ksmi_slot_f64(a[9]), (long long)a[10], (int)(int64_t)a[11], (int)(int64_t)a[12], st);
}
static int ksmi_thunk_81(const void* fn, const uint64_t* a, void* st) {
  typedef int (*F)(void*, void*, void*, void*, void*, void*, void*, void*, int, int, int, int, void*);
  (void)a; return ((F)fn)((void*)(uintptr_t)a[0], (void*)(uintptr_t)a[1], (void*)(uintptr_t)a[2], (void*)(uintptr_t)a[3], (void*)(uintptr_t)a[4], (void*)(uintptr_t)a[5], (void*)(uintptr_t)a[6], (void*)(uintptr_t)a[7], (int)(int64_t)a[8], (int)(int64_t)a[9], (int)(int64_t)a[10], (int)(int64_t)a[11], st);
}
static int ksmi_thunk_82(const void* fn, const uint64_t* a, void* st) {
  typedef int (*F)(void*, void*, void*, void*, void*, void*, void*, void*, void*, int, int, void*);
  (void)a; return ((F)fn)((void*)(uintptr_t)a[0], (void*)(uintptr_t)a[1], (void*)(uintptr_t)a[2], (void*)(uintptr_t)a[3], (void*)(uintptr_t)a[4], (void*)(uintptr_t)a[5], (void*)(uintptr_t)a[6], (void*)(uintptr_t)a[7], (void*)(uintptr_t)a[8], (int)(int64_t)a[9], (int)(int64_t)a[10], st);
}
static int ksmi_thunk_83(const void* fn, const uint64_t* a, void* st) {
  typedef int (*F)(void*, void*, void*, void*, void*, void*, void*, void*, void*, void*, int, int, int, int, int, void*);
  (void)a; return ((F)fn)((void*)(uintptr_t)a[0], (void*)(uintptr_t)a[1], (void*)(uintptr_t)a[2], (void*)(uintptr_t)a[3], (void*)(uintptr_t)a[4], (void*)(uintptr_t)a[5], (void*)(uintptr_t)a[6], (void*)(uintptr_t)a[7], (void*)(uintptr_t)a[8], (void*)(uintptr_t)a[9], (int)(int64_t)a[10], (int)(int64_t)a[11], (int)(int64_t)a[12], (int)(int64_t)a[13], (int)(int64_t)a[14], st);
}
static int ksmi_thunk_84(const void* fn, const uint64_t* a, void* st) {
  typedef int (*F)(void*, void*, void*, void*, void*, void*, void*, void*, void*, void*, void*, int, int, void*, int, int, int, int, int, int, float, int, void*);
  (void)a; return ((F)fn)((void*)(uintptr_t)a[0], (void*)(uintptr_t)a[1], (void*)(uintptr_t)a[2], (void*)(uintptr_t)a[3], (void*)(uintptr_t)a[4], (void*)(uintptr_t)a[5], (void*)(uintptr_t)a[6], (void*)(uintptr_t)a[7], (void*)(uintptr_t)a[8], (void*)(uintptr_t)a[9], (void*)(uintptr_t)a[10], (int)(int64_t)a[11], (int)(int64_t)a[12], (void*)(uintptr_t)a[13], (int)(int64_t)a[14], (int)(int64_t)a[15], (int)(int64_t)a[16], (int)(int64_t)a[17], (int)(int64_t)a[18], (int)(int64_t)a[19], ksmi_slot_f32(a[20]), (int)(int64_t)a[21], st);
}
static int ksmi_thunk_85(const void* fn, const uint64_t* a, void* st) {
  typedef int (*F)(void*, void*, void*, void*, void*, void*, void*, void*, void*, void*, void*, void*, void*, void*, void*, void*, void*, void*, int, int, void*);
  (void)a; return ((F)fn)((void*)(uintptr_t)a[0], (void*)(uintptr_t)a[1], (void*)(uintptr_t)a[2], (void*)(uintptr_t)a[3], (void*)(uintptr_t)a[4], (void*)(uintptr_t)a[5], (void*)(uintptr_t)a[6], (void*)(uintptr_t)a[7], (void*)(uintptr_t)a[8], (void*)(uintptr_t)a[9], (void*)(uintptr_t)a[10], (void*)(uintptr_t)a[11], (void*)(uintptr_t)a[12], (void*)(uintptr_t)a[13], (void*)(uintptr_t)a[14], (void*)(uintptr_t)a[15], (void*)(uintptr_t)a[16], (void*)(uintptr_t)a[17], (int)(int64_t)a[18], (int)(int64_t)a[19], st);
}
static int ksmi_thunk_86(const void* fn, const uint64_t* a, void* st) {
  typedef int (*F)(void*, void*, void*, void*, size_t, int, int, int, int, int, int, int, void*);
  (void)a; return ((F)fn)((void*)(uintptr_t)a[0], (void*)(uintptr_t)a[1], (void*)(uintptr_t)a[2], (void*)(uintptr_t)a[3], (size_t)a[4], (int)(int64_t)a[5], (int)(int64_t)a[6], (int)(int64_t)a[7], (int)(int64_t)a[8], (int)(int64_t)a[9], (int)(int64_t)a[10], (int)(int64_t)a[11], st);
}
static int ksmi_thunk_87(const void* fn, const uint64_t* a, void* st) {
  typedef int (*F)(void*, size_t, void*);
  (void)a; return ((F)fn)((void*)(uintptr_t)a[0], (size_t)a[1], st);
}

static const int ksmi_n_thunks = 88;
static const char* const ksmi_thunk_sigs[] = {"ipppfppiii", "ipppfpppiii", "ipppzp", "p", "pi", "pii", "piiidpppppffipppp", "piiidpppppffppppppppiiii", "piiiipppi", "piiiipppif", "piipppippppppdlii", "piipppipppppppdlii", "piipppipppppppidlii", "pipipiiiii", "pipippipiiii", "plipii", "pp", "ppi", "ppiiii", "ppiiiii", "ppiiiiii", "ppiiiiiiii", "ppiiiiiiiiiiii", "ppiiiiiiiiiiiii", "ppiiili", "ppiiilii", "ppilii", "ppipiiiiipppi", "ppippiiiiii", "ppippppiiiiipppi", "ppl", "ppli", "pplif", "pppfpppli", "pppi", "pppiiiifi", "pppiiiii", "pppiiiiifi", "pppiiiiifufupi", "pppiiiiii", "pppiiiiiii", "pppiiilii", "pppippiii", "pppippiiiii", "pppipppiii", "pppli", "ppplif", "pppliiufuufupi", "ppplpffff", "ppplufupi", "ppppiiii", "ppppiiiii", "ppppiiiiipppfi", "ppppiilf", "ppppiliufupi", "ppppliifi", "pppplpffffff", "pppplpffffffip", "pppppiiii", "pppppiiiii", "pppppiiiiii", "pppppiiiiufupi", "pppppiili", "pppppilii", "ppppplii", "ppppppiifi", "ppppppiiiifi", "ppppppiiiifuffuffuiiiip", "ppppppiiiii", "ppppppiiiiiii", "ppppppilii", "ppppppipiii", "pppppppdlii", "pppppppidlii", "pppppppiiiii", "pppppppiiiiifi", "pppppppiiiiifufupi", "pppppppiiiiiifi", "ppppppppdlifi", "ppppppppdlii", "ppppppppidlii", "ppppppppiiii", "pppppppppii", "ppppppppppiiiii", "pppppppppppiipiiiiiifi", "ppppppppppppppppppii", "ppppziiiiiii", "pz"};
static const ksmi_thunk_fn ksmi_thunks[] = {ksmi_thunk_0, ksmi_thunk_1, ksmi_thunk_2, ksmi_thunk_3, ksmi_thunk_4, ksmi_thunk_5, ksmi_thunk_6, ksmi_thunk_7, ksmi_thunk_8, ksmi_thunk_9, ksmi_thunk_10, ksmi_thunk_11, ksmi_thunk_12, ksmi_thunk_13, ksmi_thunk_14, ksmi_thunk_15, ksmi_thunk_16, ksmi_thunk_17, ksmi_thunk_18, ksmi_thunk_19, ksmi_thunk_20, ksmi_thunk_21, ksmi_thunk_22, ksmi_thunk_23, ksmi_thunk_24, ksmi_thunk_25, ksmi_thunk_26, ksmi_thunk_27, ksmi_thunk_28, ksmi_thunk_29, ksmi_thunk_30, ksmi_thunk_31, ksmi_thunk_32, ksmi_thunk_33, ksmi_thunk_34, ksmi_thunk_35, ksmi_thunk_36, ksmi_thunk_37, ksmi_thunk_38, ksmi_thunk_39, ksmi_thunk_40, ksmi_thunk_41, ksmi_thunk_42, ksmi_thunk_43, ksmi_thunk_44, ksmi_thunk_45, ksmi_thunk_46, ksmi_thunk_47, ksmi_thunk_48, ksmi_thunk_49, ksmi_thunk_50, ksmi_thunk_51, ksmi_thunk_52, ksmi_thunk_53, ksmi_thunk_54, ksmi_thunk_55, ksmi_thunk_56, ksmi_thunk_57, ksmi_thunk_58, ksmi_thunk_59, ksmi_thunk_60, ksmi_thunk_61, ksmi_thunk_62, ksmi_thunk_63, ksmi_thunk_64, ksmi_thunk_65, ksmi_thunk_66, ksmi_thunk_67, ksmi_thunk_68, ksmi_thunk_69, ksmi_thunk_70, ksmi_thunk_71, ksmi_thunk_72, ksmi_thunk_73, ksmi_thunk_74, ksmi_thunk_75, ksmi_thunk_76, ksmi_thunk_77, ksmi_thunk_78, ksmi_thunk_79, ksmi_thunk_80, ksmi_thunk_81, ksmi_thunk_82, ksmi_thunk_83, ksmi_thunk_84, ksmi_thunk_85, ksmi_thunk_86, ksmi_thunk_87};
```

### kurosiwo_amd/runtime.py

```python
import ctypes as C
import functools

import torch

from . import _lib
from ._lib import KSMI_BF16, KSMI_F32, ConvDesc, Dst, PackDesc, Src, WgradDesc, check

DT = {torch.float32: KSMI_F32, torch.bfloat16: KSMI_BF16}


def require_gpu(t):
    if not t.is_cuda:
        raise _lib.KsmiError("kurosiwo_amd runs on an MI355X (HIP) device only: got a CPU tensor. "
                             "There is no CPU fallback; use the reference repo for CPU runs.")


def stream_ptr():
    return C.c_void_p(torch.cuda.current_stream().cuda_stream)


def ptr(t):
    return C.c_void_p(t.data_ptr()) if t is not None else C.c_void_p(0)


def chunk_elems(dtype):
    return 32 if dtype == torch.bfloat16 else 16


def vec_elems(dtype):
    return 8 if dtype == torch.bfloat16 else 4


class Act:

    def __init__(self, name, B, H, W, Cch, dtype, device, needs_grad=True):
        self.name, self.B, self.H, self.W, self.C = name, B, H, W, Cch
        self.t = torch.empty((B, H, W, Cch), dtype=dtype, device=device)
        self.g = None
        self.needs_grad = needs_grad
        self.ginit = False
        self.consumers = []
        self.dtype, self.device = dtype, device

    def grad(self):
        if self.g is None:
            self.g = torch.empty_like(self.t)
        return self.g

    def take_acc_flag(self):
        acc = 1 if self.ginit else 0
        self.ginit = True
        return acc


class SrcSpec:
    def __init__(self, tensor, Cch, c_off=0, c_len=None, scale=None, shift=None, relu=0, k_real=None):
        self.tensor, self.C, self.c_off = tensor, Cch, c_off
        self.c_len = Cch - c_off if c_len is None else c_len
        self.k_real = self.c_len if k_real is None else k_real
        self.scale, self.shift, self.relu = scale, shift, relu


@functools.lru_cache(maxsize=None)
def choose_patch(H, W, stride=1, KH=3, KW=3, max_pix=256, max_halo=512):
    import os
    if os.environ.get("KSMI_PATCH"):
        th, tw = (int(v) for v in os.environ["KSMI_PATCH"].split(","))
        return min(th, H), min(tw, W)
    best = None
    for tw in range(1, min(W, 256) + 1):
        for th in range(1, min(H, max_pix // tw) + 1):
            hp = ((th - 1) * stride + KH) * ((tw - 1) * stride + KW)
            if hp > max_halo:
                continue
            tiles = -(-H // th) * -(-W // tw)
            cost = tiles * 256 * (1.0 + 0.15 * hp / 256.0)
            key = (cost, hp)
            if best is None or key < best[0]:
                best = (key, th, tw)
    return best[1], best[2]


def choose_patch_wgrad(H, W, stride=1, KH=3, KW=3, max_pix=256, max_halo=512):
    import os
# ... 191 lines not shown
```

### kurosiwo_amd/snunet_plan.py

```python
import ctypes as C
import os

import torch

from . import _lib
from .plan_base import PlanBase, _Saved
from .runtime import Act, SrcSpec, conv_npad, conv_stats_rows, make_conv, make_pack, make_wgrad, packed_weight_numel
from .snunet import BN_EPS, BN_MOMENTUM


class SNUNetPlan(PlanBase):
    side_wgrad = True
    two_lanes = True
    bn_fused = os.environ.get("KSMI_BN_FUSED", "1") != "0"
    im2col_late = os.environ.get("KSMI_IM2COL_LATE", "1") != "0"
    up_gemm = os.environ.get("KSMI_UP_GEMM", "1") != "0"
    up_wgrad64 = os.environ.get("KSMI_UP_WGRAD64", "1") != "0"
    up_wgrad128 = os.environ.get("KSMI_UP_WGRAD128", "1") != "0"
    pack_kind = "pack_weights_batched"

    def __init__(self, model, B, H, W, dtype, training, with_backward, tail=0, sync_bn=False):
        self._init_lists(model, dtype, with_backward)
        self.B, self.H, self.W = B, H, W
        from . import distributed as _D
        self.sync_bn = bool(sync_bn) and training
        self.bn_world = _D.world_size() if self.sync_bn else 1
        if self.sync_bn:
            self.bn_fused = False
        self.training = training
        self._up_packs = []
        self._rowsums = []
        n, c = model.base_channel, model.in_channels
        self.n = n
        f = [n, 2 * n, 4 * n, 8 * n, 16 * n]
        self.tail = tail
        self.xA = torch.empty((B, c - tail, H, W), dtype=torch.float32, device=self.dev)
        self.xB = torch.empty_like(self.xA)
        self.xtail = torch.empty((B, tail, H, W), dtype=torch.float32, device=self.dev) if tail else None
        self.logits = torch.empty((B, 3, H, W), dtype=torch.float32, device=self.dev)
        self.dlogits = torch.empty_like(self.logits) if with_backward else None
        self.bwd_builders = []

        def A(name, lvl, ch):
            return Act(name, B, H >> lvl, W >> lvl, ch, dtype, self.dev)

        L = self._lane
        L(0); x0_0A, p0A = self._block("conv0_0", "A", [self.xA], A("x0_0A", 0, f[0]), first=True, pool="p0A")
        self._handover(0, 1, back=(1, 0))
        L(1); x0_0B, p0B = self._block("conv0_0", "B", [self.xB], A("x0_0B", 0, f[0]), first=True, pool="p0B")
        L(0); x1_0A, p1A = self._block("conv1_0", "A", [self._pool_at(x0_0A, p0A, "p0A")], A("x1_0A", 1, f[1]), pool="p1A")
        self._handover(0, 1, back=(1, 0))
        L(1); x1_0B, p1B = self._block("conv1_0", "B", [self._pool_at(x0_0B, p0B, "p0B")], A("x1_0B", 1, f[1]), pool="p1B")
        L(0); x2_0A, p2A = self._block("conv2_0", "A", [self._pool_at(x1_0A, p1A, "p1A")], A("x2_0A", 2, f[2]), pool="p2A")
        self._handover(0, 1, back=(1, 0))
        L(1); x2_0B, p2B = self._block("conv2_0", "B", [self._pool_at(x1_0B, p1B, "p1B")], A("x2_0B", 2, f[2]), pool="p2B")
        L(0); x3_0A = self._block("conv3_0", "A", [self._pool_at(x2_0A, p2A, "p2A")], A("x3_0A", 3, f[3]))
        self._handover(0, 1, back=(1, 0))
        L(1); x3_0B, p3B = self._block("conv3_0", "B", [self._pool_at(x2_0B, p2B, "p2B")], A("x3_0B", 3, f[3]), pool="p3B")
        x4_0B = self._block("conv4_0", "B", [self._pool_at(x3_0B, p3B, "p3B")], A("x4_0B", 4, f[4]))
        self._handover(1, 0, back=(0, 1))

        self._handover(0, 1, back=(1, 0))
        L(0); x0_1 = self._block("conv0_1", "", [x0_0A, x0_0B, self._up("Up1_0", x1_0B)], A("x0_1", 0, f[0]))
        L(1); x1_1 = self._block("conv1_1", "", [x1_0A, x1_0B, self._up("Up2_0", x2_0B)], A("x1_1", 1, f[1]))
        u1_1 = self._up("Up1_1", x1_1)
        self._handover(1, 0, back=(0, 1))
        L(0); x0_2 = self._block("conv0_2", "", [x0_0A, x0_0B, x0_1, u1_1], A("x0_2", 0, f[0]))
        L(1); x2_1 = self._block("conv2_1", "", [x2_0A, x2_0B, self._up("Up3_0", x3_0B)], A("x2_1", 2, f[2]))
        x1_2 = self._block("conv1_2", "", [x1_0A, x1_0B, x1_1, self._up("Up2_1", x2_1)], A("x1_2", 1, f[1]))
        u1_2 = self._up("Up1_2", x1_2)
        self._handover(1, 0, back=(0, 1))
        L(0); x0_3 = self._block("conv0_3", "", [x0_0A, x0_0B, x0_1, x0_2, u1_2], A("x0_3", 0, f[0]))
        L(1); x3_1 = self._block("conv3_1", "", [x3_0A, x3_0B, self._up("Up4_0", x4_0B)], A("x3_1", 3, f[3]))
        x2_2 = self._block("conv2_2", "", [x2_0A, x2_0B, x2_1, self._up("Up3_1", x3_1)], A("x2_2", 2, f[2]))
# ... 13 lines not shown

    def _before_pack_table(self):
        if self._rowsums:
            nr = len(self._rowsums)
            arr_r = (_lib.RowsumDesc * nr)(*[r for r, _ in self._rowsums])
            raw_r = bytes(C.string_at(C.addressof(arr_r), C.sizeof(arr_r)))
            rtable = torch.frombuffer(bytearray(raw_r), dtype=torch.uint8).to(self.dev)
            self.keep.append(rtable)
            self.bwd.add("ksmi_reduce_rows_batched", lambda: (rtable.data_ptr(), nr))
            self._mark(*[k for _, k in self._rowsums])
        for i in range(0, len(self._up_packs), 16):
            grp = self._up_packs[i:i + 16]
            wt_a = (C.c_void_p * len(grp))(*[w.data_ptr() for w, _, _ in grp])
            wb_a = (C.c_void_p * len(grp))(*[b.data_ptr() for _, b, _ in grp])
            c_a = (C.c_int * len(grp))(*[c for _, _, c in grp])
            self.keep += [wt_a, wb_a, c_a]
            self.packs.add("ksmi_up_pack_weights_batched", lambda wt_a=wt_a, wb_a=wb_a, c_a=c_a, k=len(grp): (wt_a, wb_a, c_a, k),
                           {"kind": "up_pack_weight", "bytes": sum(4 * c * c * 6 for _, _, c in grp), "flops": 0})

    def _lane(self, lane):
        self.fwd.cur_lane = self.bwd.cur_lane = lane

    def _level(self, H):
        lvl = {self.H >> k: k for k in range(5)}.get(H)
        self._stage(None if lvl is None else f"L{lvl}")

    def _sname(self, name):
        return name if self.fwd.cur_lane == 0 else f"{name}@{self.fwd.cur_lane}"

    def _handover(self, src, dst, back):
        self.fwd.add_wait(src, dst)
        a, b = back
        self.bwd_builders.append((0, lambda: self.bwd.add_wait(a, b)))

    def _rows(self, npix):
        return max(1, min(512, npix // 256))

    def _rowsum_at_end(self, key, partial, rows, K, k, Cstride, Cc):
        r = _lib.RowsumDesc()
        r.partial = partial.data_ptr() if partial is not None else None
        r.dst = self.m._g(key).data_ptr()
        r.rows, r.K, r.k, r.Cstride, r.C = (rows if partial is not None else 0), K, k, Cstride, Cc
        r.accumulate, r.head, r.next = 0, 1, -1
        if self._acc_param(key):
            prev = [q for q, kk in self._rowsums if kk == key][-1]
            prev.next, r.head = len(self._rowsums), 0
        if partial is not None:
            self.keep.append(partial)
        self._rowsums.append((r, key))

    def _conv(self, ll, d, tag="fwd", name=""):
        self.keep.append(d)
        meta, ktot, _ = self._conv_meta(d, tag, f",BN{32 if d.Npad >= 32 else 16}")
        meta["tag"] = f"K={ktot} N={d.N} {d.Hout}x{d.Wout} nsrc={d.nsrc}"
        ll.add("ksmi_conv_forward", lambda: (C.byref(d), self.dt), meta)

    def _side_ix(self, key):
        if os.environ.get("KSMI_SIDE2", "0") != "1":
            return 0
        if not hasattr(self, "_side_of"):
            self._side_of = {}
        if key not in self._side_of:
            self._side_of[key] = len(self._side_of) & 1
        return self._side_of[key]

    def _wgrad(self, d, ws, key, side_tag=None):
# ... 80 lines not shown
    def _up_conv_forward(self, x, y, wkey, bkey, B, H, W, Cc):
        d, table = make_conv([SrcSpec(x.t, Cc)], [(y.t, Cc, 0, 0, 4 * Cc, 0)], x.t, self.m._p(bkey), None,
                             B, H, W, H, W, 1, 1, 1, 0, 4 * Cc, self.dtype, ps_cout=Cc)
        wpk = self._packed(wkey, table, 1, 4 * Cc, Cc, Cc * 4, 4, 1, 0, 0)
        d.wpk = wpk.data_ptr()
        self._conv(self.fwd, d)

    def _up(self, name, x):
        Cc, B, H, W = x.C, x.B, x.H, x.W
        y = Act(name, B, 2 * H, 2 * W, Cc, self.dtype, self.dev)
        self._level(2 * H)
        wkey, bkey = f"{name}.up.weight", f"{name}.up.bias"
        up_gemm = (self.up_gemm and self.dtype == torch.bfloat16 and bool(self.lib.ksmi_up_gemm_supported(B, H, W, Cc, self.dt)))
        up_fwd_gemm = up_gemm and Cc >= 256
        up_wgrad_gemm = up_fwd_gemm or (self.up_gemm and ((self.up_wgrad64 and Cc == 64) or (self.up_wgrad128 and Cc == 128))
                                        and self.dtype == torch.bfloat16 and bool(self.lib.ksmi_up_wgrad_supported(B, H, W, Cc, self.dt)))
        es = self._es()
        if up_gemm:
            wb = torch.empty(4 * Cc * Cc, dtype=torch.bfloat16, device=self.dev)
            self.keep.append(wb)
            self._up_packs.append((self.m._p(wkey), wb, Cc))
        if up_fwd_gemm:
            self.fwd.add("ksmi_up_forward", lambda: (x.t.data_ptr(), wb.data_ptr(), self.m._p(bkey).data_ptr(), y.t.data_ptr(), B, H, W, Cc),
                         {"kind": "up_gemm_fwd", "bytes": B * H * W * Cc * 5 * es, "flops": 2 * B * H * W * Cc * 4 * Cc, "tag": f"K={Cc} N={4 * Cc} {H}x{W}"})
        else:
            self._up_conv_forward(x, y, wkey, bkey, B, H, W, Cc)

        def build_bwd():
            self._level(2 * H)
            fused_bias = self._emit_dgrad(y, bias_key=bkey)
            gy = y.grad()
            s2 = [SrcSpec(gy, Cc)]
            acc = x.take_acc_flag()
            if up_gemm:
                gx = x.grad()
                self.bwd.add("ksmi_up_dgrad", lambda: (gy.data_ptr(), wb.data_ptr(), gx.data_ptr(), acc, B, H, W, Cc),
                             {"kind": "up_gemm_dgrad", "bytes": B * H * W * Cc * (5 + acc) * es, "flops": 2 * B * H * W * Cc * 4 * Cc,
                              "tag": f"K={4 * Cc} N={Cc} {H}x{W}"})
            else:
                d2, t2 = make_conv(s2, [(x.grad(), Cc, 0, 0, Cc, acc)], gy, None, None,
                                   B, 2 * H, 2 * W, H, W, 2, 2, 2, 0, Cc, self.dtype)
                w2 = self._packed(wkey, t2, 4, Cc, Cc, 4, Cc * 4, 0, 1, 0)
                d2.wpk = w2.data_ptr()
                self._conv(self.bwd, d2, "dgrad")
            if up_wgrad_gemm:
                six = self._side_ix(wkey)
                sW = self._sname("wgrad" + ("_s2" if six else ""))
                self.need(sW, self.lib.ksmi_up_wgrad_workspace(B, H, W, Cc))
                a_w = self._acc_param(wkey)
                self.bwd.add("ksmi_up_wgrad", lambda: (x.t.data_ptr(), gy.data_ptr(), self.scr(sW), self.m._g(wkey).data_ptr(), a_w, B, H, W, Cc),
                             {"kind": "up_gemm_wgrad", "bytes": B * H * W * Cc * 5 * es + 16 * Cc * Cc, "flops": 2 * B * H * W * Cc * 4 * Cc,
                              "tag": f"{wkey} K={Cc} N={4 * Cc} {H}x{W}", "side": True, "side_ix": six})
                self._mark(wkey)
            else:
                dw, ws = make_wgrad(s2, x.t, Cc, 0, Cc, self.m._g(wkey), 4, Cc * 4, 1, self._acc_param(wkey),
                                    B, 2 * H, 2 * W, H, W, 2, 2, 2, 0, self.dtype)
                self._wgrad(dw, ws, wkey)
            if not fused_bias:
                npix = B * 4 * H * W
                rows = self._rows(npix)
                pb = torch.empty(rows * Cc, dtype=torch.float32, device=self.dev)
                self.bwd.add("ksmi_channel_sum", lambda: (gy.data_ptr(), pb.data_ptr(), rows, npix, Cc, self.dt))
                self._rowsum_at_end(bkey, pb, rows, 1, 0, Cc, Cc)
        self.bwd_builders.append((self.fwd.cur_lane, build_bwd))
        return y

    def _block(self, name, branch, sources, out, first=False, pool=None):
# ... 52 lines not shown
            self.fwd.add("ksmi_bn_finalize", lambda: (stats(), rows, cpad, Cc, gcount, P(f"{bn}.weight"), P(f"{bn}.bias"),
                                                      Bf(f"{bn}.running_mean"), Bf(f"{bn}.running_var"), nbt,
                                                      BN_MOMENTUM, BN_EPS, 1 if training else 0,
                                                      sv.mean, sv.rstd, sv.scale, sv.shift))
        bn_fin("bn1", sv1, rows1, cpad1)

        src2 = [SrcSpec(i_act.t, Cc, scale=sv1.scale_t, shift=sv1.shift_t, relu=1)]
        d2, t2 = make_conv(src2, [(z_act.t, Cc, 0, 0, Cc, 0)], z_act.t, m._p(f"{name}.conv2.bias"), None,
                           B, H, W, H, W, 3, 3, 1, 1, Cc, dtype)
        w2 = self._packed(f"{name}.conv2.weight", t2, 9, Cc, Cc, 9, Cc * 9, 0, 1, 0)
        d2.wpk = w2.data_ptr()
        rows2 = conv_stats_rows(d2, dtype)
        if training:
            self.need(sS, rows2 * 2 * Npad * 4)
            self.patch(d2, "stats", sS)
        self._conv(self.fwd, d2)
        fused = training and self.bn_fused and bool(self.lib.ksmi_bn_fused_supported(Cc, Npad, dt))
        pooled = None
        if fused:
            if pool is not None:
                pooled = Act(pool, B, H // 2, W // 2, Cc, dtype, self.dev)
            nbt2 = m._c(f"{name}.bn2.num_batches_tracked").data_ptr()
            pp = pooled.t.data_ptr() if pooled is not None else None
            self.fwd.add("ksmi_bn_fin_add_relu", lambda: (stats(), rows2, Npad, Cc, float(npix), P("bn2.weight"), P("bn2.bias"),
                                                          Bf("bn2.running_mean"), Bf("bn2.running_var"), nbt2, BN_MOMENTUM, BN_EPS,
                                                          sv2.mean, sv2.rstd, sv2.scale, sv2.shift, z_act.t.data_ptr(), i_act.t.data_ptr(),
                                                          out.t.data_ptr(), pp, B, H, W, dt),
                         {"kind": "bn_fin_add_relu", "bytes": npix * Cc * self._es() * (3.25 if pooled is not None else 3), "flops": 0})
        else:
            bn_fin("bn2", sv2, rows2, Npad)
            self.fwd.add("ksmi_bn_add_relu", lambda: (z_act.t.data_ptr(), i_act.t.data_ptr(), sv2.scale, sv2.shift,
                                                      out.t.data_ptr(), npix, Cc, dt))

        def build_bwd():
            self._level(H)
            gated = self._emit_dgrad(out, gate=(out.t, z_act.t, sv2)) if os.environ.get("KSMI_NO_GATE") is None else self._emit_dgrad(out)
            gated = gated if isinstance(gated, tuple) else None
            rows = self._rows(npix)
            self.need(sR, rows * 2 * Cc * 4)
            sums1 = torch.zeros((2, Cc), dtype=torch.float32, device=self.dev)
            sums2 = torch.zeros((2, Cc), dtype=torch.float32, device=self.dev)
            dz = torch.empty_like(z_act.t)
            r = torch.empty_like(i_act.t)
            self.keep += [sums1, sums2, dz, r]
            gout = out.grad().data_ptr()
            s1p, s2p = sums1.data_ptr(), sums2.data_ptr()
            a_bn2 = self._acc_param(f"{name}.bn2")
            es = self._es()
            if gated is not None:
                gst, grows, gpad = gated
                if fused and self.lib.ksmi_bn_fused_supported(Cc, gpad, dt):
                    self.bwd.add("ksmi_bn_bwd_fin_apply_gated", lambda: (gst.data_ptr(), grows, gpad, s2p, G("bn2.weight"), G("bn2.bias"), a_bn2,
                                                                         gout, z_act.t.data_ptr(), sv2.mean, sv2.rstd, P("bn2.weight"),
                                                                         dz.data_ptr(), float(npix), npix, Cc, dt),
                                 {"kind": "bn_bwd_fin_apply_gated", "bytes": npix * Cc * es * 3, "flops": 0})
                    self._mark(f"{name}.bn2.weight", f"{name}.bn2.bias")
                else:
                    self.bwd.add("ksmi_reduce_rows", lambda: (gst.data_ptr(), grows, 2, gpad, Cc, s2p, G("bn2.weight"), G("bn2.bias"), a_bn2))
                    self._mark(f"{name}.bn2.weight", f"{name}.bn2.bias")
                    if self.sync_bn:
                        self.bwd.add_allreduce(lambda: sums2)
                    self.bwd.add("ksmi_bn_bwd_apply_gated", lambda: (gout, z_act.t.data_ptr(), sv2.mean, sv2.rstd, P("bn2.weight"), s2p,
                                                                     dz.data_ptr(), gcount, npix, Cc, dt))
            else:
                self.bwd.add("ksmi_bnrelu_bwd_reduce", lambda: (gout, out.t.data_ptr(), z_act.t.data_ptr(), sv2.mean, sv2.rstd,
                                                                self.scr(sR), rows, npix, Cc, dt))
                if fused:
                    self.bwd.add("ksmi_bnrelu_bwd_fin_apply", lambda: (self.scr(sR), rows, Cc, s2p, G("bn2.weight"), G("bn2.bias"), a_bn2,
                                                                       gout, out.t.data_ptr(), z_act.t.data_ptr(), sv2.mean, sv2.rstd,
                                                                       P("bn2.weight"), dz.data_ptr(), float(npix), npix, Cc, dt),
                                 {"kind": "bnrelu_bwd_fin_apply", "bytes": npix * Cc * es * 5, "flops": 0})
                    self._mark(f"{name}.bn2.weight", f"{name}.bn2.bias")
                else:
                    self.bwd.add("ksmi_reduce_rows", lambda: (self.scr(sR), rows, 2, Cc, Cc, s2p, G("bn2.weight"), G("bn2.bias"), a_bn2))
                    self._mark(f"{name}.bn2.weight", f"{name}.bn2.bias")
                    if self.sync_bn:
                        self.bwd.add_allreduce(lambda: sums2)
# ... 61 lines not shown
    def _head(self, xs):
        m, B, n = self.m, self.B, self.n
        HW = self.H * self.W
        dev, dt = self.dev, self.dt
        self._stage("head")
        f32 = dict(dtype=torch.float32, device=dev)
        avg, mx = torch.zeros((B, 5 * n), **f32), torch.zeros((B, 5 * n), **f32)
        argmax = torch.zeros((B, 5 * n), dtype=torch.int32, device=dev)
        ca, ca1 = torch.zeros((B, 4 * n), **f32), torch.zeros((B, n), **f32)
        hidden = torch.zeros((B, 2, 4 * n // 16 + n // 4), **f32)
        xarr = (C.c_void_p * 4)(*[a.t.data_ptr() for a in xs])
        ws_pool = torch.empty(self.lib.ksmi_ecam_pool_workspace(B, HW, n), dtype=torch.uint8, device=dev)
        self.keep += [avg, mx, argmax, ca, ca1, hidden, xarr, ws_pool]
        self.head = dict(avg=avg, mx=mx, argmax=argmax, ca=ca, ca1=ca1)
        P = lambda key: m._p(key).data_ptr()
        G = lambda key: m._g(key).data_ptr()
        T0 = B * HW * n * self._es()
        self.fwd.add("ksmi_ecam_pool", lambda: (xarr, avg.data_ptr(), mx.data_ptr(), argmax.data_ptr(), ws_pool.data_ptr(), B, HW, n, dt),
                     {"kind": "ecam_pool", "bytes": 4 * T0, "flops": 0})
        self.fwd.add("ksmi_ecam_mlp", lambda: (avg.data_ptr(), mx.data_ptr(), P("ca.fc1.weight"), P("ca.fc2.weight"),
                                               P("ca1.fc1.weight"), P("ca1.fc2.weight"), ca.data_ptr(), ca1.data_ptr(),
                                               hidden.data_ptr(), B, n))
        self.fwd.add("ksmi_ecam_final_forward", lambda: (xarr, ca.data_ptr(), ca1.data_ptr(), P("conv_final.weight"),
                                                         P("conv_final.bias"), self.logits.data_ptr(), B, HW, n, 3, dt),
                     {"kind": "ecam_final_forward", "bytes": 4 * T0 + B * HW * 3 * 4, "flops": 2 * B * HW * 4 * n * 3})

        def build_bwd():
            self._stage("head")
            dca, dca1 = torch.zeros((B, 4 * n), **f32), torch.zeros((B, n), **f32)
            davg, dmax = torch.zeros((B, 5 * n), **f32), torch.zeros((B, 5 * n), **f32)
            ws_b = torch.empty(self.lib.ksmi_ecam_bwd_workspace(B, HW, n, 3), dtype=torch.uint8, device=dev)
            ws_m = torch.empty(self.lib.ksmi_ecam_mlp_bwd_workspace(B, n), dtype=torch.uint8, device=dev)
            garr = (C.c_void_p * 4)(*[a.grad().data_ptr() for a in xs])
            for a in xs:
                a.take_acc_flag()
            for key in ("conv_final.weight", "conv_final.bias", "ca.fc1.weight", "ca.fc2.weight", "ca1.fc1.weight", "ca1.fc2.weight"):
                self._acc_param(key)
            self.keep += [dca, dca1, davg, dmax, ws_b, ws_m, garr]
            dl = self.dlogits.data_ptr()
            self.bwd.add("ksmi_ecam_final_backward_reduce", lambda: (
                xarr, dl, ca.data_ptr(), ca1.data_ptr(), P("conv_final.weight"), dca.data_ptr(), dca1.data_ptr(),
                G("conv_final.weight"), G("conv_final.bias"), ws_b.data_ptr(), B, HW, n, 3, dt),
                {"kind": "ecam_final_backward_reduce", "bytes": 4 * T0 + B * HW * 3 * 4, "flops": 2 * B * HW * 4 * n * 3})
            self._mark("conv_final.weight", "conv_final.bias")
            self.bwd.add("ksmi_ecam_mlp_backward", lambda: (
                avg.data_ptr(), mx.data_ptr(), hidden.data_ptr(), ca.data_ptr(), ca1.data_ptr(), dca.data_ptr(), dca1.data_ptr(),
                P("ca.fc1.weight"), P("ca.fc2.weight"), P("ca1.fc1.weight"), P("ca1.fc2.weight"), davg.data_ptr(), dmax.data_ptr(),
                G("ca.fc1.weight"), G("ca.fc2.weight"), G("ca1.fc1.weight"), G("ca1.fc2.weight"), ws_m.data_ptr(), B, n))
            self._mark("ca.fc1.weight", "ca.fc2.weight", "ca1.fc1.weight", "ca1.fc2.weight")
            self.bwd.add("ksmi_ecam_final_backward_dx", lambda: (
                garr, dl, ca.data_ptr(), P("conv_final.weight"), davg.data_ptr(), dmax.data_ptr(), argmax.data_ptr(), B, HW, n, 3, dt),
                {"kind": "ecam_final_backward_dx", "bytes": 4 * T0 + B * HW * 3 * 4, "flops": 2 * B * HW * 4 * n * 3})
        self.bwd_builders.append((self.fwd.cur_lane, build_bwd))

    def run_forward(self, xA, xB, tail=None):
        if (tail is None) != (self.xtail is None):
            raise _lib.KsmiError("plan and call disagree about the shared tail channels (DEM)")
        return self._run_forward(self.logits, (xA, self.xA), (xB, self.xB), *([] if tail is None else [(tail, self.xtail)]))
```

Baseline: 2175 tiles/s.

## Fuse ReLU gating and BN-backward partial sums into up-dgrad and ECAM dx producers

Adds gated variants of the upsample dgrad GEMM and the ECAM head dx kernel. They apply the residual block's ReLU mask and accumulate the BN backward partial sums (sum of g and sum of g times the normalized z) in the epilogue, writing per-tile stats rows. The block backward then consumes these precomputed stats instead of re-reading the gradient to gate and reduce it. This removes a separate pass over large activation gradients. In exchange the epilogues read two extra bf16 tensors, the dx kernel gets a larger LDS footprint and fewer grid blocks, and the max-scatter for the gated source is folded into the kernel. Ordering assertions guard against multiple gradient producers.

```diff
diff --git a/include/ksmi.h b/include/ksmi.h
--- a/include/ksmi.h
+++ b/include/ksmi.h
@@ -219,6 +219,11 @@
 int ksmi_ecam_final_backward_dx(void* const dx[4], const float* dlogits, const float* ca, const float* wf,
                                 const float* davg, const float* dmax, const int32_t* argmax,
                                 int B, int HW, int C, int ncls, int dtype, void* stream);
+int ksmi_ecam_gate_rows(int B, int HW, int C, int dtype);
+int ksmi_ecam_final_backward_dx_gated(void* const dx[4], const float* dlogits, const float* ca, const float* wf,
+                                      const float* davg, const float* dmax, const int32_t* argmax,
+                                      const void* gate_out, const void* gate_z, const float* g_mean, const float* g_rstd,
+                                      float* stats, int B, int HW, int C, int ncls, int dtype, void* stream);
 
 size_t ksmi_loss_workspace(int B, int HW);
 int ksmi_ce_dice_forward(const float* logits, const int64_t* labels, const float* class_w, int with_dice,
@@ -347,6 +352,9 @@
 int ksmi_up_pack_weights_batched(const float* const* wt, void* const* wb, const int* C, int n, void* stream);
 int ksmi_up_forward(const void* x, const void* wb, const float* bias, void* y, int B, int H, int W, int C, void* stream);
 int ksmi_up_dgrad(const void* dy, const void* wb, void* dx, int accumulate, int B, int H, int W, int C, void* stream);
+int ksmi_up_dgrad_gate_rows(int B, int H, int W, int C);
+int ksmi_up_dgrad_gated(const void* dy, const void* wb, void* dx, int accumulate, const void* gate_out, const void* gate_z,
+                        const float* g_mean, const float* g_rstd, float* stats, int B, int H, int W, int C, void* stream);
 size_t ksmi_up_wgrad_workspace(int B, int H, int W, int C);
 int ksmi_up_wgrad(const void* x, const void* dy, float* workspace, float* grad, int accumulate, int B, int H, int W, int C, void* stream);
 
diff --git a/kurosiwo_amd/_lib.py b/kurosiwo_amd/_lib.py
--- a/kurosiwo_amd/_lib.py
+++ b/kurosiwo_amd/_lib.py
@@ -152,6 +152,8 @@
     "ksmi_ecam_mlp_backward": (_i, [_vp] * 18 + [_i, _i, _vp]),
     "ksmi_ecam_mlp_bwd_workspace": (_sz, [_i, _i]),
     "ksmi_ecam_final_backward_dx": (_i, [_P4, _vp, _vp, _vp, _vp, _vp, _vp, _i, _i, _i, _i, _i, _vp]),
+    "ksmi_ecam_gate_rows": (_i, [_i, _i, _i, _i]),
+    "ksmi_ecam_final_backward_dx_gated": (_i, [_P4, _vp, _vp, _vp, _vp, _vp, _vp, _vp, _vp, _vp, _vp, _vp, _i, _i, _i, _i, _i, _vp]),
     "ksmi_loss_workspace": (_sz, [_i, _i]),
     "ksmi_ce_dice_forward": (_i, [_vp, _vp, _vp, _i, _vp, _vp, _i, _i, _i, _vp]),
     "ksmi_ce_dice_backward": (_i, [_vp, _vp, _vp, _i, _vp, _vp, _vp, _i, _i, _i, _vp]),
@@ -196,6 +198,8 @@
     "ksmi_up_pack_weights_batched": (_i, [_vp, _vp, _vp, _i, _vp]),
     "ksmi_up_forward": (_i, [_vp, _vp, _vp, _vp, _i, _i, _i, _i, _vp]),
     "ksmi_up_dgrad": (_i, [_vp, _vp, _vp, _i, _i, _i, _i, _i, _vp]),
+    "ksmi_up_dgrad_gate_rows": (_i, [_i, _i, _i, _i]),
+    "ksmi_up_dgrad_gated": (_i, [_vp, _vp, _vp, _i, _vp, _vp, _vp, _vp, _vp, _i, _i, _i, _i, _vp]),
     "ksmi_up_wgrad_workspace": (C.c_size_t, [_i, _i, _i, _i]),
     "ksmi_up_wgrad": (_i, [_vp, _vp, _vp, _vp, _i, _i, _i, _i, _i, _vp]),
     "ksmi_gemm_nt": (_i, [_vp, _i, _vp, _i, _vp, _vp, _i, _vp, _i, _i, _i, _i, _vp]),
diff --git a/kurosiwo_amd/csrc/gemm2.hip b/kurosiwo_amd/csrc/gemm2.hip
--- a/kurosiwo_amd/csrc/gemm2.hip
+++ b/kurosiwo_amd/csrc/gemm2.hip
@@ -13,6 +13,7 @@
   int rows, red, cols, accumulate;
   int mtiles, ntiles;
   int map_a, map_o, up_H, up_W, up_C, bias_mod;
+  const bf16_t* gate_out; const bf16_t* gate_z; const float* g_mean; const float* g_rstd; float* stats;
 };
 
 __device__ __forceinline__ size_t up_row_base(int m, int H, int W, int C) {
@@ -76,7 +77,39 @@
   *(u32x4*)(op + 8) = vec_pack<bf16_t>(v + 8);
 }
 
-template <int MT, bool TRW, int NS>
+template <int MT>
+__device__ __forceinline__ void store_row2_gated(const Gemm2P& p, const f32x4 (&acc)[4][MT], int mt, int m, int c0, const float* mu,
+                                                 const float* rs, float* sg, float* sx) {
+  if (m >= p.rows) return;
+  float v[16], o[16], z[16];
+#pragma unroll
+  for (int t = 0; t < 4; ++t)
+#pragma unroll
+    for (int r = 0; r < 4; ++r) v[t * 4 + r] = acc[t][mt][r];
+  const size_t off = (size_t)m * p.o_rs + c0;
+  bf16_t* op = p.out + off;
+  vec_unpack<bf16_t>(*(const u32x4*)(p.gate_out + off), o);
+  vec_unpack<bf16_t>(*(const u32x4*)(p.gate_out + off + 8), o + 8);
+  vec_unpack<bf16_t>(*(const u32x4*)(p.gate_z + off), z);
+  vec_unpack<bf16_t>(*(const u32x4*)(p.gate_z + off + 8), z + 8);
+  if (p.accumulate) {
+    float a[8], b[8];
+    vec_unpack<bf16_t>(*(const u32x4*)op, a);
+    vec_unpack<bf16_t>(*(const u32x4*)(op + 8), b);
+#pragma unroll
+    for (int j = 0; j < 8; ++j) { v[j] += a[j]; v[8 + j] += b[j]; }
+  }
+#pragma unroll
+  for (int j = 0; j < 16; ++j) v[j] = o[j] > 0.f ? v[j] : 0.f;
+  const u32x4 lo = vec_pack<bf16_t>(v), hi = vec_pack<bf16_t>(v + 8);
+  *(u32x4*)op = lo;
+  *(u32x4*)(op + 8) = hi;
+  vec_unpack<bf16_t>(lo, v); vec_unpack<bf16_t>(hi, v + 8);
+#pragma unroll
+  for (int j = 0; j < 16; ++j) { sg[j] += v[j]; sx[j] += v[j] * ((z[j] - mu[j]) * rs[j]); }
+}
+
+template <int MT, bool TRW, int NS, bool GATE = false>
 __global__ __launch_bounds__(256, 1) void gemm2_kernel(const Gemm2P p) {
   constexpr int TM = 32 * MT, KS = 64, XB = TM * 128, WB = 128 * 128, STAGE = XB + WB;
   constexpr int NQ = STAGE / 1024, NI = NQ / 4;
@@ -207,6 +240,31 @@
     for (int b = 0; b < MT; ++b) acc[a][b] += acc2[a][b];
 
   const int c0 = n0 + wn * 64 + g * 16;
+  if constexpr (GATE) {
+    float mu[16], rs[16], sg[16], sx[16];
+#pragma unroll
+    for (int j = 0; j < 16; ++j) { mu[j] = p.g_mean[c0 + j]; rs[j] = p.g_rstd[c0 + j]; sg[j] = 0.f; sx[j] = 0.f; }
+#pragma unroll
+    for (int mt = 0; mt < MT; ++mt) store_row2_gated<MT>(p, acc, mt, m0 + wm * 16 * MT + mt * 16 + l15, c0, mu, rs, sg, sx);
+#pragma unroll
+    for (int o = 1; o < 16; o <<= 1)
+#pragma unroll
+      for (int j = 0; j < 16; ++j) { sg[j] += __shfl_xor(sg[j], o, 64); sx[j] += __shfl_xor(sx[j], o, 64); }
+    float* red = (float*)smem;
+    const int cl = wn * 64 + g * 16;
+    __syncthreads();
+    if (wm == 1 && l15 == 0) {
+#pragma unroll
+      for (int j = 0; j < 16; ++j) { red[cl + j] = sg[j]; red[128 + cl + j] = sx[j]; }
+    }
+    __syncthreads();
+    if (wm == 0 && l15 == 0) {
+      float* row = p.stats + (size_t)mt_i * 2 * p.cols + c0;
+#pragma unroll
+      for (int j = 0; j < 16; ++j) { row[j] = sg[j] + red[cl + j]; row[p.cols + j] = sx[j] + red[128 + cl + j]; }
+    }
+    return;
+  }
   if (c0 >= p.cols) return;
   float bias16[16];
 #pragma unroll
@@ -215,11 +273,11 @@
   for (int mt = 0; mt < MT; ++mt) store_row2<MT>(p, acc, mt, m0 + wm * 16 * MT + mt * 16 + l15, c0, bias16);
 }
 
-template <int MT, bool TRW, int NS>
+template <int MT, bool TRW, int NS, bool GATE = false>
 int launch2n(const Gemm2P& p, hipStream_t st) {
   constexpr int lds = NS * (32 * MT * 128 + 128 * 128);
   static_assert(lds <= 160 * 1024, "LDS ring");
-  auto kfn = gemm2_kernel<MT, TRW, NS>; KSMI_NOTE(kfn);
+  auto kfn = gemm2_kernel<MT, TRW, NS, GATE>; KSMI_NOTE(kfn);
   static bool attr = false;
   if (!attr) { (void)hipFuncSetAttribute((const void*)kfn, hipFuncAttributeMaxDynamicSharedMemorySize, lds); attr = true; }
   hipLaunchKernelGGL(kfn, dim3(p.mtiles * p.ntiles), dim3(256), lds, st, p);
@@ -268,6 +326,18 @@
     case 7: return launch2<7, TRW>(p, t.ns, st);
     default: return launch2<8, TRW>(p, t.ns, st);
   }
+}
+
+int dispatch2_gated(Gemm2P& p, hipStream_t st) {
+  p.ntiles = p.cols / 128;
+  const Tile2 t = pick_tile(p.rows, p.ntiles);
+  p.mtiles = (p.rows + 32 * t.mt - 1) / (32 * t.mt);
+#define KSMI_G2G(MM) case MM: return t.ns <= 2 ? launch2n<MM, true, 2, true>(p, st) : launch2n<MM, true, 3, true>(p, st)
+  switch (t.mt) {
+    KSMI_G2G(2); KSMI_G2G(3); KSMI_G2G(4); KSMI_G2G(5); KSMI_G2G(6); KSMI_G2G(7);
+    default: return launch2n<8, true, 3, true>(p, st);
+  }
+#undef KSMI_G2G
 }
 
 struct Gemm2T {
@@ -517,6 +587,20 @@
   return dispatch2<true>(p, st);
 }
 
+int ksmi_gemm2_up_dgrad_gated(const void* dy, const void* wb, void* dx, int accumulate, const void* gate_out, const void* gate_z,
+                              const float* g_mean, const float* g_rstd, float* stats, int B, int H, int W, int C, int* rows_out, hipStream_t st) {
+  if (C % 128 || C < 128 || B * H * W < 64) return 1;
+  Gemm2P p = {(const bf16_t*)dy, 0, (const bf16_t*)wb, C, nullptr, nullptr, 0, (bf16_t*)dx, C, B * H * W, 4 * C, C, accumulate, 0, 0};
+  p.map_a = 1; p.up_H = H; p.up_W = W; p.up_C = C;
+  if (rows_out) {
+    const Tile2 t = pick_tile(p.rows, p.cols / 128);
+    *rows_out = (p.rows + 32 * t.mt - 1) / (32 * t.mt);
+    return 0;
+  }
+  p.gate_out = (const bf16_t*)gate_out; p.gate_z = (const bf16_t*)gate_z; p.g_mean = g_mean; p.g_rstd = g_rstd; p.stats = stats;
+  return dispatch2_gated(p, st);
+}
+
 template <int MT, int NS, int SPL = 1, bool BIASA = false>
 static void launch_tn(dim3 grid, const Gemm2T& p, hipStream_t st) {
   constexpr int lds = SPL * NS * (64 * 256 + 64 * 64 * MT);
@@ -700,6 +784,16 @@
   const int rc = ksmi_gemm2_up_dgrad(dy, wb, dx, accumulate, B, H, W, C, (hipStream_t)stream);
   return rc == 1 ? ksmi_fail(KSMI_E_UNSUPPORTED, "up_dgrad: shape not covered (ksmi_up_gemm_supported)") : rc;
 }
+int ksmi_up_dgrad_gate_rows(int B, int H, int W, int C) {
+  int rows = 0;
+  return ksmi_gemm2_up_dgrad_gated(nullptr, nullptr, nullptr, 0, nullptr, nullptr, nullptr, nullptr, nullptr, B, H, W, C, &rows, nullptr) ? 0 : rows;
+}
+int ksmi_up_dgrad_gated(const void* dy, const void* wb, void* dx, int accumulate, const void* gate_out, const void* gate_z,
+                        const float* g_mean, const float* g_rstd, float* stats, int B, int H, int W, int C, void* stream) {
+  if (!gate_out || !gate_z || !g_mean || !g_rstd || !stats) return ksmi_fail(KSMI_E_ARG, "up_dgrad_gated: bad args");
+  const int rc = ksmi_gemm2_up_dgrad_gated(dy, wb, dx, accumulate, gate_out, gate_z, g_mean, g_rstd, stats, B, H, W, C, nullptr, (hipStream_t)stream);
+  return rc == 1 ? ksmi_fail(KSMI_E_UNSUPPORTED, "up_dgrad_gated: shape not covered (ksmi_up_dgrad_gate_rows)") : rc;
+}
 size_t ksmi_up_wgrad_workspace(int B, int H, int W, int C) { return ksmi_gemm2_up_wgrad_workspace(B, H, W, C); }
 int ksmi_up_wgrad(const void* x, const void* dy, float* workspace, float* grad, int accumulate, int B, int H, int W, int C, void* stream) {
   const int rc = ksmi_gemm2_up_wgrad(x, dy, workspace, grad, accumulate, B, H, W, C, (hipStream_t)stream);
diff --git a/kurosiwo_amd/csrc/head.hip b/kurosiwo_amd/csrc/head.hip
--- a/kurosiwo_amd/csrc/head.hip
+++ b/kurosiwo_amd/csrc/head.hip
@@ -402,9 +402,14 @@
   }
 }
 
-template <typename T, int NCLS>
+struct EcamGate {
+  const void* out; const void* z; const float* mean; const float* rstd;
+  const float* dmax; const int* argmax;
+  float* stats;
+};
+template <typename T, int NCLS, bool GATE>
 __global__ __launch_bounds__(256) void ecam_bwd_dx_kernel(T* d0, T* d1, T* d2, T* d3, const float* dl, const float* ca,
-                                                          const float* wf, const float* davg, int HW, int C) {
+                                                          const float* wf, const float* davg, int HW, int C, const EcamGate gt) {
   constexpr int VEC = ElemTraits<T>::kVec;
   extern __shared__ float sm[];
   const int b = blockIdx.y, C4 = 4 * C;
@@ -418,7 +423,8 @@
   const int ppb = blockDim.x / tpp;
   const int q = threadIdx.x % tpp, pl = threadIdx.x / tpp;
   const int s = q / CV, c0 = (q - s * CV) * VEC;
-  if (pl >= ppb) return;
+  const bool active = pl < ppb;
+  if (!GATE && !active) return;
   float w[NCLS][VEC], k0[VEC];
 #pragma unroll
   for (int j = 0; j < VEC; ++j) {
@@ -427,35 +433,85 @@
     for (int k = 0; k < NCLS; ++k) w[k][j] = weff[k * C4 + s * C + c0 + j];
   }
   T* dst = (s == 0 ? d0 : s == 1 ? d1 : s == 2 ? d2 : d3) + (int64_t)b * HW * C + c0;
-  for (int p = blockIdx.x * ppb + pl; p < HW; p += gridDim.x * ppb) {
-    float d[NCLS], v[VEC];
-#pragma unroll
-    for (int k = 0; k < NCLS; ++k) d[k] = dl[((int64_t)b * NCLS + k) * HW + p];
+  const bool gs = GATE && s == 3;
+  float sg[GATE ? VEC : 1], sx[GATE ? VEC : 1], mu[GATE ? VEC : 1], rs[GATE ? VEC : 1], dmc[GATE ? VEC : 1], dmi[GATE ? VEC : 1];
+  int amc[GATE ? VEC : 1], ami[GATE ? VEC : 1];
+  if constexpr (GATE) {
 #pragma unroll
     for (int j = 0; j < VEC; ++j) {
-      float a = k0[j];
-#pragma unroll
-      for (int k = 0; k < NCLS; ++k) a += w[k][j] * d[k];
-      v[j] = a;
-    }
-    *(u32x4*)(dst + (int64_t)p * C) = vec_pack<T>(v);
+      sg[j] = 0.f; sx[j] = 0.f;
+      const int ch = gs ? c0 + j : 0;
+      mu[j] = gt.mean[ch]; rs[j] = gt.rstd[ch];
+      const size_t ab = (size_t)b * 5 * C;
+      amc[j] = gt.argmax[ab + 3 * C + ch]; dmc[j] = gt.dmax[ab + 3 * C + ch];
+      ami[j] = gt.argmax[ab + 4 * C + ch]; dmi[j] = gt.dmax[ab + 4 * C + ch];
+    }
+  }
+  if (active) {
+    for (int p = blockIdx.x * ppb + pl; p < HW; p += gridDim.x * ppb) {
+      float d[NCLS], v[VEC];
+      u32x4 ro, rz;
+      if (gs) {
+        const int64_t off = ((int64_t)b * HW + p) * C + c0;
+        ro = *(const u32x4*)((const T*)gt.out + off); rz = *(const u32x4*)((const T*)gt.z + off);
+      }
+#pragma unroll
+      for (int k = 0; k < NCLS; ++k) d[k] = dl[((int64_t)b * NCLS + k) * HW + p];
+#pragma unroll
+      for (int j = 0; j < VEC; ++j) {
+        float a = k0[j];
+#pragma unroll
+        for (int k = 0; k < NCLS; ++k) a += w[k][j] * d[k];
+        v[j] = a;
+      }
+      if constexpr (GATE) {
+        if (gs) {
+          float o[VEC], zz[VEC];
+          vec_unpack<T>(ro, o); vec_unpack<T>(rz, zz);
+#pragma unroll
+          for (int j = 0; j < VEC; ++j) {
+            float g = ElemTraits<T>::cvt(v[j]);
+            if (p == amc[j]) g = ElemTraits<T>::cvt(g + dmc[j]);
+            if (p == ami[j]) g = ElemTraits<T>::cvt(g + dmi[j]);
+            g = o[j] > 0.f ? g : 0.f;
+            v[j] = g;
+            sg[j] += g; sx[j] += g * ((zz[j] - mu[j]) * rs[j]);
+          }
+        }
+      }
+      *(u32x4*)(dst + (int64_t)p * C) = vec_pack<T>(v);
+    }
+  }
+  if constexpr (GATE) {
+    float* red = sm + (NCLS + 1) * C4;
+    if (gs && active) {
+#pragma unroll
+      for (int j = 0; j < VEC; ++j) { red[(pl * 2 + 0) * C + c0 + j] = sg[j]; red[(pl * 2 + 1) * C + c0 + j] = sx[j]; }
+    }
+    __syncthreads();
+    float* row = gt.stats + ((size_t)blockIdx.y * gridDim.x + blockIdx.x) * 2 * C;
+    for (int i = threadIdx.x; i < 2 * C; i += blockDim.x) {
+      float a = 0.f;
+      for (int l = 0; l < ppb; ++l) a += red[l * 2 * C + i];
+      row[i] = a;
+    }
   }
 }
 
 template <typename T>
-__global__ void ecam_bwd_max_scatter_kernel(T* d0, T* d1, T* d2, T* d3, const float* dmax, const int* argmax, int B, int HW, int C) {
+__global__ void ecam_bwd_max_scatter_kernel(T* d0, T* d1, T* d2, T* d3, const float* dmax, const int* argmax, int B, int HW, int C, int nsrc) {
   const int i = blockIdx.x * blockDim.x + threadIdx.x;
   if (i >= B * C) return;
   const int b = i / C, cc = i - b * C;
   T* ds[4] = {d0, d1, d2, d3};
-  for (int s = 0; s < 4; ++s) {
+  for (int s = 0; s < nsrc; ++s) {
     const int c = s * C + cc;
     T* q = ds[s] + ((int64_t)b * HW + argmax[b * 5 * C + c]) * C + cc;
     ElemTraits<T>::st(q, ElemTraits<T>::ld(q) + dmax[b * 5 * C + c]);
   }
   const int pi = argmax[b * 5 * C + 4 * C + cc];
   const float g = dmax[b * 5 * C + 4 * C + cc];
-  for (int s = 0; s < 4; ++s) {
+  for (int s = 0; s < nsrc; ++s) {
     T* q = ds[s] + ((int64_t)b * HW + pi) * C + cc;
     ElemTraits<T>::st(q, ElemTraits<T>::ld(q) + g);
   }
@@ -713,30 +769,65 @@
   return ksmi_check_launch("ecam_mlp_bwd");
 }
 
+static int ecam_dx_grid(int HW, int C, int dtype, bool gate) {
+  const int tpp = 4 * C / (dtype == KSMI_BF16 ? 8 : 4);
+  const int ppb = 256 / tpp, trips = gate ? 32 : 8;
+  const int gx = (HW + ppb * trips - 1) / (ppb * trips);
+  return gx < 1 ? 1 : gx;
+}
+
+static int ecam_dx(void* const dx[4], const float* dlogits, const float* ca, const float* wf, const float* davg, const float* dmax,
+                   const int32_t* argmax, const EcamGate* gate, int B, int HW, int C, int ncls, int dtype, void* stream) {
+  if (ncls != 3 || !ecam_c_ok(C, dtype)) return ksmi_fail(KSMI_E_UNSUPPORTED, "ecam_final_bwd_dx: ncls must be 3");
+  const int tpp = 4 * C / (dtype == KSMI_BF16 ? 8 : 4);
+  if (tpp > 256) return ksmi_fail(KSMI_E_UNSUPPORTED, "ecam_final_bwd_dx: C too large for the (pixel, source, vector) thread map");
+  const int ppb = 256 / tpp;
+  const dim3 grid(ecam_dx_grid(HW, C, dtype, gate != nullptr), B);
+  if (gate) {
+    const size_t lds = (size_t)(3 * 4 * C + 4 * C + ppb * 2 * C) * sizeof(float);
+    KSMI_DT(dtype,
+            hipLaunchKernelGGL((ecam_bwd_dx_kernel<bf16_t, 3, true>), grid, dim3(256), lds, (hipStream_t)stream, (bf16_t*)dx[0], (bf16_t*)dx[1],
+                               (bf16_t*)dx[2], (bf16_t*)dx[3], dlogits, ca, wf, davg, HW, C, *gate),
+            hipLaunchKernelGGL((ecam_bwd_dx_kernel<float, 3, true>), grid, dim3(256), lds, (hipStream_t)stream, (float*)dx[0], (float*)dx[1],
+                               (float*)dx[2], (float*)dx[3], dlogits, ca, wf, davg, HW, C, *gate));
+  } else {
+    const size_t lds = (size_t)(3 * 4 * C + 4 * C) * sizeof(float);
+    const EcamGate none{};
+    KSMI_DT(dtype,
+            hipLaunchKernelGGL((ecam_bwd_dx_kernel<bf16_t, 3, false>), grid, dim3(256), lds, (hipStream_t)stream, (bf16_t*)dx[0], (bf16_t*)dx[1],
+                               (bf16_t*)dx[2], (bf16_t*)dx[3], dlogits, ca, wf, davg, HW, C, none),
+            hipLaunchKernelGGL((ecam_bwd_dx_kernel<float, 3, false>), grid, dim3(256), lds, (hipStream_t)stream, (float*)dx[0], (float*)dx[1],
+                               (float*)dx[2], (float*)dx[3], dlogits, ca, wf, davg, HW, C, none));
+  }
+  int rc = ksmi_check_launch("ecam_bwd_dx");
+  if (rc) return rc;
+  const int tot = B * C, nsrc = gate ? 3 : 4;
+  KSMI_DT(dtype,
+          hipLaunchKernelGGL(ecam_bwd_max_scatter_kernel<bf16_t>, dim3((tot + 255) / 256), dim3(256), 0, (hipStream_t)stream,
+                             (bf16_t*)dx[0], (bf16_t*)dx[1], (bf16_t*)dx[2], (bf16_t*)dx[3], dmax, argmax, B, HW, C, nsrc),
+          hipLaunchKernelGGL(ecam_bwd_max_scatter_kernel<float>, dim3((tot + 255) / 256), dim3(256), 0, (hipStream_t)stream,
+                             (float*)dx[0], (float*)dx[1], (float*)dx[2], (float*)dx[3], dmax, argmax, B, HW, C, nsrc));
+  return ksmi_check_launch("ecam_bwd_max_scatter");
+}
+
 int ksmi_ecam_final_backward_dx(void* const dx[4], const float* dlogits, const float* ca, const float* wf, const float* davg,
                                 const float* dmax, const int32_t* argmax, int B, int HW, int C, int ncls, int dtype, void* stream) {
-  if (ncls != 3 || !ecam_c_ok(C, dtype)) return ksmi_fail(KSMI_E_UNSUPPORTED, "ecam_final_bwd_dx: ncls must be 3");
-  const size_t lds = (size_t)(3 * 4 * C + 4 * C) * sizeof(float);
-  const int tpp = 4 * C / (dtype == KSMI_BF16 ? 8 : 4);
-  if (tpp > 256) return ksmi_fail(KSMI_E_UNSUPPORTED, "ecam_final_bwd_dx: C too large for the (pixel, source, vector) thread map");
-  const int ppb = 256 / tpp, trips = 8;
-  int gx = (HW + ppb * trips - 1) / (ppb * trips);
-  if (gx < 1) gx = 1;
-  const dim3 grid(gx, B);
-  KSMI_DT(dtype,
-          hipLaunchKernelGGL((ecam_bwd_dx_kernel<bf16_t, 3>), grid, dim3(256), lds, (hipStream_t)stream, (bf16_t*)dx[0], (bf16_t*)dx[1],
-                             (bf16_t*)dx[2], (bf16_t*)dx[3], dlogits, ca, wf, davg, HW, C),
-          hipLaunchKernelGGL((ecam_bwd_dx_kernel<float, 3>), grid, dim3(256), lds, (hipStream_t)stream, (float*)dx[0], (float*)dx[1],
-                             (float*)dx[2], (float*)dx[3], dlogits, ca, wf, davg, HW, C));
-  int rc = ksmi_check_launch("ecam_bwd_dx");
-  if (rc) return rc;
-  const int tot = B * C;
-  KSMI_DT(dtype,
-          hipLaunchKernelGGL(ecam_bwd_max_scatter_kernel<bf16_t>, dim3((tot + 255) / 256), dim3(256), 0, (hipStream_t)stream,
-                             (bf16_t*)dx[0], (bf16_t*)dx[1], (bf16_t*)dx[2], (bf16_t*)dx[3], dmax, argmax, B, HW, C),
-          hipLaunchKernelGGL(ecam_bwd_max_scatter_kernel<float>, dim3((tot + 255) / 256), dim3(256), 0, (hipStream_t)stream,
-                             (float*)dx[0], (float*)dx[1], (float*)dx[2], (float*)dx[3], dmax, argmax, B, HW, C));
-  return ksmi_check_launch("ecam_bwd_max_scatter");
+  return ecam_dx(dx, dlogits, ca, wf, davg, dmax, argmax, nullptr, B, HW, C, ncls, dtype, stream);
+}
+
+int ksmi_ecam_gate_rows(int B, int HW, int C, int dtype) {
+  if (B < 1 || HW < 1 || !ecam_c_ok(C, dtype) || 4 * C / (dtype == KSMI_BF16 ? 8 : 4) > 256) return 0;
+  return B * ecam_dx_grid(HW, C, dtype, true);
+}
+
+int ksmi_ecam_final_backward_dx_gated(void* const dx[4], const float* dlogits, const float* ca, const float* wf, const float* davg,
+                                      const float* dmax, const int32_t* argmax, const void* gate_out, const void* gate_z,
+                                      const float* g_mean, const float* g_rstd, float* stats, int B, int HW, int C, int ncls, int dtype,
+                                      void* stream) {
+  if (!gate_out || !gate_z || !g_mean || !g_rstd || !stats || !dmax || !argmax)
+    return ksmi_fail(KSMI_E_ARG, "ecam_final_bwd_dx_gated: bad args");
+  const EcamGate g{gate_out, gate_z, g_mean, g_rstd, dmax, argmax, stats};
+  return ecam_dx(dx, dlogits, ca, wf, davg, dmax, argmax, &g, B, HW, C, ncls, dtype, stream);
 }
 
 size_t ksmi_loss_workspace(int B, int HW) { (void)HW; return ((size_t)B * kLossSplit * 4 + 1 + 2 * (size_t)B) * sizeof(float); }
diff --git a/kurosiwo_amd/csrc/thunks_gen.h b/kurosiwo_amd/csrc/thunks_gen.h
--- a/kurosiwo_amd/csrc/thunks_gen.h
+++ b/kurosiwo_amd/csrc/thunks_gen.h
@@ -188,178 +188,186 @@
   (void)a; return ((F)fn)((void*)(uintptr_t)a[0], (void*)(uintptr_t)a[1], (void*)(uintptr_t)a[2], (int)(int64_t)a[3], (void*)(uintptr_t)a[4], (void*)(uintptr_t)a[5], (void*)(uintptr_t)a[6], (int)(int64_t)a[7], (int)(int64_t)a[8], (int)(int64_t)a[9], st);
 }
 static int ksmi_thunk_45(const void* fn, const uint64_t* a, void* st) {
+  typedef int (*F)(void*, void*, void*, int, void*, void*, void*, void*, void*, int, int, int, int, void*);
+  (void)a; return ((F)fn)((void*)(uintptr_t)a[0], (void*)(uintptr_t)a[1], (void*)(uintptr_t)a[2], (int)(int64_t)a[3], (void*)(uintptr_t)a[4], (void*)(uintptr_t)a[5], (void*)(uintptr_t)a[6], (void*)(uintptr_t)a[7], (void*)(uintptr_t)a[8], (int)(int64_t)a[9], (int)(int64_t)a[10], (int)(int64_t)a[11], (int)(int64_t)a[12], st);
+}
+static int ksmi_thunk_46(const void* fn, const uint64_t* a, void* st) {
   typedef int (*F)(void*, void*, void*, long long, int, void*);
   (void)a; return ((F)fn)((void*)(uintptr_t)a[0], (void*)(uintptr_t)a[1], (void*)(uintptr_t)a[2], (long long)a[3], (int)(int64_t)a[4], st);
 }
-static int ksmi_thunk_46(const void* fn, const uint64_t* a, void* st) {
+static int ksmi_thunk_47(const void* fn, const uint64_t* a, void* st) {
   typedef int (*F)(void*, void*, void*, long long, int, float, void*);
   (void)a; return ((F)fn)((void*)(uintptr_t)a[0], (void*)(uintptr_t)a[1], (void*)(uintptr_t)a[2], (long long)a[3], (int)(int64_t)a[4], ksmi_slot_f32(a[5]), st);
 }
-static int ksmi_thunk_47(const void* fn, const uint64_t* a, void* st) {
+static int ksmi_thunk_48(const void* fn, const uint64_t* a, void* st) {
   typedef int (*F)(void*, void*, void*, long long, int, int, unsigned int, float, unsigned int, unsigned int, float, unsigned int, void*, int, void*);
   (void)a; return ((F)fn)((void*)(uintptr_t)a[0], (void*)(uintptr_t)a[1], (void*)(uintptr_t)a[2], (long long)a[3], (int)(int64_t)a[4], (int)(int64_t)a[5], (unsigned int)a[6], ksmi_slot_f32(a[7]), (unsigned int)a[8], (unsigned int)a[9], ksmi_slot_f32(a[10]), (unsigned int)a[11], (void*)(uintptr_t)a[12], (int)(int64_t)a[13], st);
 }
-static int ksmi_thunk_48(const void* fn, const uint64_t* a, void* st) {
+static int ksmi_thunk_49(const void* fn, const uint64_t* a, void* st) {
   typedef int (*F)(void*, void*, void*, long long, void*, float, float, float, float, void*);
   (void)a; return ((F)fn)((void*)(uintptr_t)a[0], (void*)(uintptr_t)a[1], (void*)(uintptr_t)a[2], (long long)a[3], (void*)(uintptr_t)a[4], ksmi_slot_f32(a[5]), ksmi_slot_f32(a[6]), ksmi_slot_f32(a[7]), ksmi_slot_f32(a[8]), st);
 }
-static int ksmi_thunk_49(const void* fn, const uint64_t* a, void* st) {
+static int ksmi_thunk_50(const void* fn, const uint64_t* a, void* st) {
   typedef int (*F)(void*, void*, void*, long long, unsigned int, float, unsigned int, void*, int, void*);
   (void)a; return ((F)fn)((void*)(uintptr_t)a[0], (void*)(uintptr_t)a[1], (void*)(uintptr_t)a[2], (long long)a[3], (unsigned int)a[4], ksmi_slot_f32(a[5]), (unsigned int)a[6], (void*)(uintptr_t)a[7], (int)(int64_t)a[8], st);
 }
-static int ksmi_thunk_50(const void* fn, const uint64_t* a, void* st) {
+static int ksmi_thunk_51(const void* fn, const uint64_t* a, void* st) {
   typedef int (*F)(void*, void*, void*, void*, int, int, int, int, void*);
   (void)a; return ((F)fn)((void*)(uintptr_t)a[0], (void*)(uintptr_t)a[1], (void*)(uintptr_t)a[2], (void*)(uintptr_t)a[3], (int)(int64_t)a[4], (int)(int64_t)a[5], (int)(int64_t)a[6], (int)(int64_t)a[7], st);
 }
-static int ksmi_thunk_51(const void* fn, const uint64_t* a, void* st) {
+static int ksmi_thunk_52(const void* fn, const uint64_t* a, void* st) {
   typedef int (*F)(void*, void*, void*, void*, int, int, int, int, int, void*);
   (void)a; return ((F)fn)((void*)(uintptr_t)a[0], (void*)(uintptr_t)a[1], (void*)(uintptr_t)a[2], (void*)(uintptr_t)a[3], (int)(int64_t)a[4], (int)(int64_t)a[5], (int)(int64_t)a[6], (int)(int64_t)a[7], (int)(int64_t)a[8], st);
 }
-static int ksmi_thunk_52(const void* fn, const uint64_t* a, void* st) {
+static int ksmi_thunk_53(const void* fn, const uint64_t* a, void* st) {
   typedef int (*F)(void*, void*, void*, void*, int, int, int, int, int, void*, void*, void*, float, int, void*);
   (void)a; return ((F)fn)((void*)(uintptr_t)a[0], (void*)(uintptr_t)a[1], (void*)(uintptr_t)a[2], (void*)(uintptr_t)a[3], (int)(int64_t)a[4], (int)(int64_t)a[5], (int)(int64_t)a[6], (int)(int64_t)a[7], (int)(int64_t)a[8], (void*)(uintptr_t)a[9], (void*)(uintptr_t)a[10], (void*)(uintptr_t)a[11], ksmi_slot_f32(a[12]), (int)(int64_t)a[13], st);
 }
-static int ksmi_thunk_53(const void* fn, const uint64_t* a, void* st) {
+static int ksmi_thunk_54(const void* fn, const uint64_t* a, void* st) {
   typedef int (*F)(void*, void*, void*, void*, int, int, long long, float, void*);
   (void)a; return ((F)fn)((void*)(uintptr_t)a[0], (void*)(uintptr_t)a[1], (void*)(uintptr_t)a[2], (void*)(uintptr_t)a[3], (int)(int64_t)a[4], (int)(int64_t)a[5], (long long)a[6], ksmi_slot_f32(a[7]), st);
 }
-static int ksmi_thunk_54(const void* fn, const uint64_t* a, void* st) {
+static int ksmi_thunk_55(const void* fn, const uint64_t* a, void* st) {
   typedef int (*F)(void*, void*, void*, void*, int, long long, int, unsigned int, float, unsigned int, void*, int, void*);
   (void)a; return ((F)fn)((void*)(uintptr_t)a[0], (void*)(uintptr_t)a[1], (void*)(uintptr_t)a[2], (void*)(uintptr_t)a[3], (int)(int64_t)a[4], (long long)a[5], (int)(int64_t)a[6], (unsigned int)a[7], ksmi_slot_f32(a[8]), (unsigned int)a[9], (void*)(uintptr_t)a[10], (int)(int64_t)a[11], st);
 }
-static int ksmi_thunk_55(const void* fn, const uint64_t* a, void* st) {
+static int ksmi_thunk_56(const void* fn, const uint64_t* a, void* st) {
   typedef int (*F)(void*, void*, void*, void*, long long, int, int, float, int, void*);
   (void)a; return ((F)fn)((void*)(uintptr_t)a[0], (void*)(uintptr_t)a[1], (void*)(uintptr_t)a[2], (void*)(uintptr_t)a[3], (long long)a[4], (int)(int64_t)a[5], (int)(int64_t)a[6], ksmi_slot_f32(a[7]), (int)(int64_t)a[8], st);
 }
-static int ksmi_thunk_56(const void* fn, const uint64_t* a, void* st) {
+static int ksmi_thunk_57(const void* fn, const uint64_t* a, void* st) {
   typedef int (*F)(void*, void*, void*, void*, long long, void*, float, float, float, float, float, float, void*);
   (void)a; return ((F)fn)((void*)(uintptr_t)a[0], (void*)(uintptr_t)a[1], (void*)(uintptr_t)a[2], (void*)(uintptr_t)a[3], (long long)a[4], (void*)(uintptr_t)a[5], ksmi_slot_f32(a[6]), ksmi_slot_f32(a[7]), ksmi_slot_f32(a[8]), ksmi_slot_f32(a[9]), ksmi_slot_f32(a[10]), ksmi_slot_f32(a[11]), st);
 }
-static int ksmi_thunk_57(const void* fn, const uint64_t* a, void* st) {
+static int ksmi_thunk_58(const void* fn, const uint64_t* a, void* st) {
   typedef int (*F)(void*, void*, void*, void*, long long, void*, float, float, float, float, float, float, int, void*, void*);
   (void)a; return ((F)fn)((void*)(uintptr_t)a[0], (void*)(uintptr_t)a[1], (void*)(uintptr_t)a[2], (void*)(uintptr_t)a[3], (long long)a[4], (void*)(uintptr_t)a[5], ksmi_slot_f32(a[6]), ksmi_slot_f32(a[7]), ksmi_slot_f32(a[8]), ksmi_slot_f32(a[9]), ksmi_slot_f32(a[10]), ksmi_slot_f32(a[11]), (int)(int64_t)a[12], (void*)(uintptr_t)a[13], st);
 }
-static int ksmi_thunk_58(const void* fn, const uint64_t* a, void* st) {
+static int ksmi_thunk_59(const void* fn, const uint64_t* a, void* st) {
   typedef int (*F)(void*, void*, void*, void*, void*, int, int, int, int, void*);
   (void)a; return ((F)fn)((void*)(uintptr_t)a[0], (void*)(uintptr_t)a[1], (void*)(uintptr_t)a[2], (void*)(uintptr_t)a[3], (void*)(uintptr_t)a[4], (int)(int64_t)a[5], (int)(int64_t)a[6], (int)(int64_t)a[7], (int)(int64_t)a[8], st);
 }
-static int ksmi_thunk_59(const void* fn, const uint64_t* a, void* st) {
+static int ksmi_thunk_60(const void* fn, const uint64_t* a, void* st) {
   typedef int (*F)(void*, void*, void*, void*, void*, int, int, int, int, int, void*);
   (void)a; return ((F)fn)((void*)(uintptr_t)a[0], (void*)(uintptr_t)a[1], (void*)(uintptr_t)a[2], (void*)(uintptr_t)a[3], (void*)(uintptr_t)a[4], (int)(int64_t)a[5], (int)(int64_t)a[6], (int)(int64_t)a[7], (int)(int64_t)a[8], (int)(int64_t)a[9], st);
 }
-static int ksmi_thunk_60(const void* fn, const uint64_t* a, void* st) {
+static int ksmi_thunk_61(const void* fn, const uint64_t* a, void* st) {
   typedef int (*F)(void*, void*, void*, void*, void*, int, int, int, int, int, int, void*);
   (void)a; return ((F)fn)((void*)(uintptr_t)a[0], (void*)(uintptr_t)a[1], (void*)(uintptr_t)a[2], (void*)(uintptr_t)a[3], (void*)(uintptr_t)a[4], (int)(int64_t)a[5], (int)(int64_t)a[6], (int)(int64_t)a[7], (int)(int64_t)a[8], (int)(int64_t)a[9], (int)(int64_t)a[10], st);
 }
-static int ksmi_thunk_61(const void* fn, const uint64_t* a, void* st) {
+static int ksmi_thunk_62(const void* fn, const uint64_t* a, void* st) {
   typedef int (*F)(void*, void*, void*, void*, void*, int, int, int, int, unsigned int, float, unsigned int, void*, int, void*);
   (void)a; return ((F)fn)((void*)(uintptr_t)a[0], (void*)(uintptr_t)a[1], (void*)(uintptr_t)a[2], (void*)(uintptr_t)a[3], (void*)(uintptr_t)a[4], (int)(int64_t)a[5], (int)(int64_t)a[6], (int)(int64_t)a[7], (int)(int64_t)a[8], (unsigned int)a[9], ksmi_slot_f32(a[10]), (unsigned int)a[11], (void*)(uintptr_t)a[12], (int)(int64_t)a[13], st);
 }
-static int ksmi_thunk_62(const void* fn, const uint64_t* a, void* st) {
+static int ksmi_thunk_63(const void* fn, const uint64_t* a, void* st) {
   typedef int (*F)(void*, void*, void*, void*, void*, int, int, long long, int, void*);
   (void)a; return ((F)fn)((void*)(uintptr_t)a[0], (void*)(uintptr_t)a[1], (void*)(uintptr_t)a[2], (void*)(uintptr_t)a[3], (void*)(uintptr_t)a[4], (int)(int64_t)a[5], (int)(int64_t)a[6], (long long)a[7], (int)(int64_t)a[8], st);
 }
-static int ksmi_thunk_63(const void* fn, const uint64_t* a, void* st) {
+static int ksmi_thunk_64(const void* fn, const uint64_t* a, void* st) {
   typedef int (*F)(void*, void*, void*, void*, void*, int, long long, int, int, void*);
   (void)a; return ((F)fn)((void*)(uintptr_t)a[0], (void*)(uintptr_t)a[1], (void*)(uintptr_t)a[2], (void*)(uintptr_t)a[3], (void*)(uintptr_t)a[4], (int)(int64_t)a[5], (long long)a[6], (int)(int64_t)a[7], (int)(int64_t)a[8], st);
 }
-static int ksmi_thunk_64(const void* fn, const uint64_t* a, void* st) {
+static int ksmi_thunk_65(const void* fn, const uint64_t* a, void* st) {
   typedef int (*F)(void*, void*, void*, void*, void*, long long, int, int, void*);
   (void)a; return ((F)fn)((void*)(uintptr_t)a[0], (void*)(uintptr_t)a[1], (void*)(uintptr_t)a[2], (void*)(uintptr_t)a[3], (void*)(uintptr_t)a[4], (long long)a[5], (int)(int64_t)a[6], (int)(int64_t)a[7], st);
 }
-static int ksmi_thunk_65(const void* fn, const uint64_t* a, void* st) {
+static int ksmi_thunk_66(const void* fn, const uint64_t* a, void* st) {
   typedef int (*F)(void*, void*, void*, void*, void*, void*, int, int, float, int, void*);
   (void)a; return ((F)fn)((void*)(uintptr_t)a[0], (void*)(uintptr_t)a[1], (void*)(uintptr_t)a[2], (void*)(uintptr_t)a[3], (void*)(uintptr_t)a[4], (void*)(uintptr_t)a[5], (int)(int64_t)a[6], (int)(int64_t)a[7], ksmi_slot_f32(a[8]), (int)(int64_t)a[9], st);
 }
-static int ksmi_thunk_66(const void* fn, const uint64_t* a, void* st) {
+static int ksmi_thunk_67(const void* fn, const uint64_t* a, void* st) {
   typedef int (*F)(void*, void*, void*, void*, void*, void*, int, int, int, int, float, int, void*);
   (void)a; return ((F)fn)((void*)(uintptr_t)a[0], (void*)(uintptr_t)a[1], (void*)(uintptr_t)a[2], (void*)(uintptr_t)a[3], (void*)(uintptr_t)a[4], (void*)(uintptr_t)a[5], (int)(int64_t)a[6], (int)(int64_t)a[7], (int)(int64_t)a[8], (int)(int64_t)a[9], ksmi_slot_f32(a[10]), (int)(int64_t)a[11], st);
 }
-static int ksmi_thunk_67(const void* fn, const uint64_t* a, void* st) {
+static int ksmi_thunk_68(const void* fn, const uint64_t* a, void* st) {
   typedef int (*F)(void*, void*, void*, void*, void*, void*, int, int, int, int, float, unsigned int, float, float, unsigned int, float, float, unsigned int, int, int, int, int, void*, void*);
   (void)a; return ((F)fn)((void*)(uintptr_t)a[0], (void*)(uintptr_t)a[1], (void*)(uintptr_t)a[2], (void*)(uintptr_t)a[3], (void*)(uintptr_t)a[4], (void*)(uintptr_t)a[5], (int)(int64_t)a[6], (int)(int64_t)a[7], (int)(int64_t)a[8], (int)(int64_t)a[9], ksmi_slot_f32(a[10]), (unsigned int)a[11], ksmi_slot_f32(a[12]), ksmi_slot_f32(a[13]), (unsigned int)a[14], ksmi_slot_f32(a[15]), ksmi_slot_f32(a[16]), (unsigned int)a[17], (int)(int64_t)a[18], (int)(int64_t)a[19], (int)(int64_t)a[20], (int)(int64_t)a[21], (void*)(uintptr_t)a[22], st);
 }
-static int ksmi_thunk_68(const void* fn, const uint64_t* a, void* st) {
+static int ksmi_thunk_69(const void* fn, const uint64_t* a, void* st) {
   typedef int (*F)(void*, void*, void*, void*, void*, void*, int, int, int, int, int, void*);
   (void)a; return ((F)fn)((void*)(uintptr_t)a[0], (void*)(uintptr_t)a[1], (void*)(uintptr_t)a[2], (void*)(uintptr_t)a[3], (void*)(uintptr_t)a[4], (void*)(uintptr_t)a[5], (int)(int64_t)a[6], (int)(int64_t)a[7], (int)(int64_t)a[8], (int)(int64_t)a[9], (int)(int64_t)a[10], st);
 }
-static int ksmi_thunk_69(const void* fn, const uint64_t* a, void* st) {
+static int ksmi_thunk_70(const void* fn, const uint64_t* a, void* st) {
   typedef int (*F)(void*, void*, void*, void*, void*, void*, int, int, int, int, int, int, int, void*);
   (void)a; return ((F)fn)((void*)(uintptr_t)a[0], (void*)(uintptr_t)a[1], (void*)(uintptr_t)a[2], (void*)(uintptr_t)a[3], (void*)(uintptr_t)a[4], (void*)(uintptr_t)a[5], (int)(int64_t)a[6], (int)(int64_t)a[7], (int)(int64_t)a[8], (int)(int64_t)a[9], (int)(int64_t)a[10], (int)(int64_t)a[11], (int)(int64_t)a[12], st);
 }
-static int ksmi_thunk_70(const void* fn, const uint64_t* a, void* st) {
+static int ksmi_thunk_71(const void* fn, const uint64_t* a, void* st) {
   typedef int (*F)(void*, void*, void*, void*, void*, void*, int, long long, int, int, void*);
   (void)a; return ((F)fn)((void*)(uintptr_t)a[0], (void*)(uintptr_t)a[1], (void*)(uintptr_t)a[2], (void*)(uintptr_t)a[3], (void*)(uintptr_t)a[4], (void*)(uintptr_t)a[5], (int)(int64_t)a[6], (long long)a[7], (int)(int64_t)a[8], (int)(int64_t)a[9], st);
 }
-static int ksmi_thunk_71(const void* fn, const uint64_t* a, void* st) {
+static int ksmi_thunk_72(const void* fn, const uint64_t* a, void* st) {
   typedef int (*F)(void*, void*, void*, void*, void*, void*, int, void*, int, int, int, void*);
   (void)a; return ((F)fn)((void*)(uintptr_t)a[0], (void*)(uintptr_t)a[1], (void*)(uintptr_t)a[2], (void*)(uintptr_t)a[3], (void*)(uintptr_t)a[4], (void*)(uintptr_t)a[5], (int)(int64_t)a[6], (void*)(uintptr_t)a[7], (int)(int64_t)a[8], (int)(int64_t)a[9], (int)(int64_t)a[10], st);
 }
-static int ksmi_thunk_72(const void* fn, const uint64_t* a, void* st) {
+static int ksmi_thunk_73(const void* fn, const uint64_t* a, void* st) {
   typedef int (*F)(void*, void*, void*, void*, void*, void*, void*, double, long long, int, int, void*);
   (void)a; return ((F)fn)((void*)(uintptr_t)a[0], (void*)(uintptr_t)a[1], (void*)(uintptr_t)a[2], (void*)(uintptr_t)a[3], (void*)(uintptr_t)a[4], (void*)(uintptr_t)a[5], (void*)(uintptr_t)a[6], ksmi_slot_f64(a[7]), (long long)a[8], (int)(int64_t)a[9], (int)(int64_t)a[10], st);
 }
-static int ksmi_thunk_73(const void* fn, const uint64_t* a, void* st) {
+static int ksmi_thunk_74(const void* fn, const uint64_t* a, void* st) {
   typedef int (*F)(void*, void*, void*, void*, void*, void*, void*, int, double, long long, int, int, void*);
   (void)a; return ((F)fn)((void*)(uintptr_t)a[0], (void*)(uintptr_t)a[1], (void*)(uintptr_t)a[2], (void*)(uintptr_t)a[3], (void*)(uintptr_t)a[4], (void*)(uintptr_t)a[5], (void*)(uintptr_t)a[6], (int)(int64_t)a[7], ksmi_slot_f64(a[8]), (long long)a[9], (int)(int64_t)a[10], (int)(int64_t)a[11], st);
 }
-static int ksmi_thunk_74(const void* fn, const uint64_t* a, void* st) {
+static int ksmi_thunk_75(const void* fn, const uint64_t* a, void* st) {
   typedef int (*F)(void*, void*, void*, void*, void*, void*, void*, int, int, int, int, int, void*);
   (void)a; return ((F)fn)((void*)(uintptr_t)a[0], (void*)(uintptr_t)a[1], (void*)(uintptr_t)a[2], (void*)(uintptr_t)a[3], (void*)(uintptr_t)a[4], (void*)(uintptr_t)a[5], (void*)(uintptr_t)a[6], (int)(int64_t)a[7], (int)(int64_t)a[8], (int)(int64_t)a[9], (int)(int64_t)a[10], (int)(int64_t)a[11], st);
 }
-static int ksmi_thunk_75(const void* fn, const uint64_t* a, void* st) {
+static int ksmi_thunk_76(const void* fn, const uint64_t* a, void* st) {
   typedef int (*F)(void*, void*, void*, void*, void*, void*, void*, int, int, int, int, int, float, int, void*);
   (void)a; return ((F)fn)((void*)(uintptr_t)a[0], (void*)(uintptr_t)a[1], (void*)(uintptr_t)a[2], (void*)(uintptr_t)a[3], (void*)(uintptr_t)a[4], (void*)(uintptr_t)a[5], (void*)(uintptr_t)a[6], (int)(int64_t)a[7], (int)(int64_t)a[8], (int)(int64_t)a[9], (int)(int64_t)a[10], (int)(int64_t)a[11], ksmi_slot_f32(a[12]), (int)(int64_t)a[13], st);
 }
-static int ksmi_thunk_76(const void* fn, const uint64_t* a, void* st) {
+static int ksmi_thunk_77(const void* fn, const uint64_t* a, void* st) {
   typedef int (*F)(void*, void*, void*, void*, void*, void*, void*, int, int, int, int, int, float, unsigned int, float, unsigned int, void*, int, void*);
   (void)a; return ((F)fn)((void*)(uintptr_t)a[0], (void*)(uintptr_t)a[1], (void*)(uintptr_t)a[2], (void*)(uintptr_t)a[3], (void*)(uintptr_t)a[4], (void*)(uintptr_t)a[5], (void*)(uintptr_t)a[6], (int)(int64_t)a[7], (int)(int64_t)a[8], (int)(int64_t)a[9], (int)(int64_t)a[10], (int)(int64_t)a[11], ksmi_slot_f32(a[12]), (unsigned int)a[13], ksmi_slot_f32(a[14]), (unsigned int)a[15], (void*)(uintptr_t)a[16], (int)(int64_t)a[17], st);
 }
-static int ksmi_thunk_77(const void* fn, const uint64_t* a, void* st) {
+static int ksmi_thunk_78(const void* fn, const uint64_t* a, void* st) {
   typedef int (*F)(void*, void*, void*, void*, void*, void*, void*, int, int, int, int, int, int, float, int, void*);
   (void)a; return ((F)fn)((void*)(uintptr_t)a[0], (void*)(uintptr_t)a[1], (void*)(uintptr_t)a[2], (void*)(uintptr_t)a[3], (void*)(uintptr_t)a[4], (void*)(uintptr_t)a[5], (void*)(uintptr_t)a[6], (int)(int64_t)a[7], (int)(int64_t)a[8], (int)(int64_t)a[9], (int)(int64_t)a[10], (int)(int64_t)a[11], (int)(int64_t)a[12], ksmi_slot_f32(a[13]), (int)(int64_t)a[14], st);
 }
-static int ksmi_thunk_78(const void* fn, const uint64_t* a, void* st) {
+static int ksmi_thunk_79(const void* fn, const uint64_t* a, void* st) {
   typedef int (*F)(void*, void*, void*, void*, void*, void*, void*, void*, double, long long, int, float, int, void*);
   (void)a; return ((F)fn)((void*)(uintptr_t)a[0], (void*)(uintptr_t)a[1], (void*)(uintptr_t)a[2], (void*)(uintptr_t)a[3], (void*)(uintptr_t)a[4], (void*)(uintptr_t)a[5], (void*)(uintptr_t)a[6], (void*)(uintptr_t)a[7], ksmi_slot_f64(a[8]), (long long)a[9], (int)(int64_t)a[10], ksmi_slot_f32(a[11]), (int)(int64_t)a[12], st);
 }
-static int ksmi_thunk_79(const void* fn, const uint64_t* a, void* st) {
+static int ksmi_thunk_80(const void* fn, const uint64_t* a, void* st) {
   typedef int (*F)(void*, void*, void*, void*, void*, void*, void*, void*, double, long long, int, int, void*);
   (void)a; return ((F)fn)((void*)(uintptr_t)a[0], (void*)(uintptr_t)a[1], (void*)(uintptr_t)a[2], (void*)(uintptr_t)a[3], (void*)(uintptr_t)a[4], (void*)(uintptr_t)a[5], (void*)(uintptr_t)a[6], (void*)(uintptr_t)a[7], ksmi_slot_f64(a[8]), (long long)a[9], (int)(int64_t)a[10], (int)(int64_t)a[11], st);
 }
-static int ksmi_thunk_80(const void* fn, const uint64_t* a, void* st) {
+static int ksmi_thunk_81(const void* fn, const uint64_t* a, void* st) {
   typedef int (*F)(void*, void*, void*, void*, void*, void*, void*, void*, int, double, long long, int, int, void*);
   (void)a; return ((F)fn)((void*)(uintptr_t)a[0], (void*)(uintptr_t)a[1], (void*)(uintptr_t)a[2], (void*)(uintptr_t)a[3], (void*)(uintptr_t)a[4], (void*)(uintptr_t)a[5], (void*)(uintptr_t)a[6], (void*)(uintptr_t)a[7], (int)(int64_t)a[8], ksmi_slot_f64(a[9]), (long long)a[10], (int)(int64_t)a[11], (int)(int64_t)a[12], st);
 }
-static int ksmi_thunk_81(const void* fn, const uint64_t* a, void* st) {
+static int ksmi_thunk_82(const void* fn, const uint64_t* a, void* st) {
   typedef int (*F)(void*, void*, void*, void*, void*, void*, void*, void*, int, int, int, int, void*);
   (void)a; return ((F)fn)((void*)(uintptr_t)a[0], (void*)(uintptr_t)a[1], (void*)(uintptr_t)a[2], (void*)(uintptr_t)a[3], (void*)(uintptr_t)a[4], (void*)(uintptr_t)a[5], (void*)(uintptr_t)a[6], (void*)(uintptr_t)a[7], (int)(int64_t)a[8], (int)(int64_t)a[9], (int)(int64_t)a[10], (int)(int64_t)a[11], st);
 }
-static int ksmi_thunk_82(const void* fn, const uint64_t* a, void* st) {
+static int ksmi_thunk_83(const void* fn, const uint64_t* a, void* st) {
   typedef int (*F)(void*, void*, void*, void*, void*, void*, void*, void*, void*, int, int, void*);
   (void)a; return ((F)fn)((void*)(uintptr_t)a[0], (void*)(uintptr_t)a[1], (void*)(uintptr_t)a[2], (void*)(uintptr_t)a[3], (void*)(uintptr_t)a[4], (void*)(uintptr_t)a[5], (void*)(uintptr_t)a[6], (void*)(uintptr_t)a[7], (void*)(uintptr_t)a[8], (int)(int64_t)a[9], (int)(int64_t)a[10], st);
 }
-static int ksmi_thunk_83(const void* fn, const uint64_t* a, void* st) {
+static int ksmi_thunk_84(const void* fn, const uint64_t* a, void* st) {
   typedef int (*F)(void*, void*, void*, void*, void*, void*, void*, void*, void*, void*, int, int, int, int, int, void*);
   (void)a; return ((F)fn)((void*)(uintptr_t)a[0], (void*)(uintptr_t)a[1], (void*)(uintptr_t)a[2], (void*)(uintptr_t)a[3], (void*)(uintptr_t)a[4], (void*)(uintptr_t)a[5], (void*)(uintptr_t)a[6], (void*)(uintptr_t)a[7], (void*)(uintptr_t)a[8], (void*)(uintptr_t)a[9], (int)(int64_t)a[10], (int)(int64_t)a[11], (int)(int64_t)a[12], (int)(int64_t)a[13], (int)(int64_t)a[14], st);
 }
-static int ksmi_thunk_84(const void* fn, const uint64_t* a, void* st) {
+static int ksmi_thunk_85(const void* fn, const uint64_t* a, void* st) {
   typedef int (*F)(void*, void*, void*, void*, void*, void*, void*, void*, void*, void*, void*, int, int, void*, int, int, int, int, int, int, float, int, void*);
   (void)a; return ((F)fn)((void*)(uintptr_t)a[0], (void*)(uintptr_t)a[1], (void*)(uintptr_t)a[2], (void*)(uintptr_t)a[3], (void*)(uintptr_t)a[4], (void*)(uintptr_t)a[5], (void*)(uintptr_t)a[6], (void*)(uintptr_t)a[7], (void*)(uintptr_t)a[8], (void*)(uintptr_t)a[9], (void*)(uintptr_t)a[10], (int)(int64_t)a[11], (int)(int64_t)a[12], (void*)(uintptr_t)a[13], (int)(int64_t)a[14], (int)(int64_t)a[15], (int)(int64_t)a[16], (int)(int64_t)a[17], (int)(int64_t)a[18], (int)(int64_t)a[19], ksmi_slot_f32(a[20]), (int)(int64_t)a[21], st);
 }
-static int ksmi_thunk_85(const void* fn, const uint64_t* a, void* st) {
+static int ksmi_thunk_86(const void* fn, const uint64_t* a, void* st) {
+  typedef int (*F)(void*, void*, void*, void*, void*, void*, void*, void*, void*, void*, void*, void*, int, int, int, int, int, void*);
+  (void)a; return ((F)fn)((void*)(uintptr_t)a[0], (void*)(uintptr_t)a[1], (void*)(uintptr_t)a[2], (void*)(uintptr_t)a[3], (void*)(uintptr_t)a[4], (void*)(uintptr_t)a[5], (void*)(uintptr_t)a[6], (void*)(uintptr_t)a[7], (void*)(uintptr_t)a[8], (void*)(uintptr_t)a[9], (void*)(uintptr_t)a[10], (void*)(uintptr_t)a[11], (int)(int64_t)a[12], (int)(int64_t)a[13], (int)(int64_t)a[14], (int)(int64_t)a[15], (int)(int64_t)a[16], st);
+}
+static int ksmi_thunk_87(const void* fn, const uint64_t* a, void* st) {
   typedef int (*F)(void*, void*, void*, void*, void*, void*, void*, void*, void*, void*, void*, void*, void*, void*, void*, void*, void*, void*, int, int, void*);
   (void)a; return ((F)fn)((void*)(uintptr_t)a[0], (void*)(uintptr_t)a[1], (void*)(uintptr_t)a[2], (void*)(uintptr_t)a[3], (void*)(uintptr_t)a[4], (void*)(uintptr_t)a[5], (void*)(uintptr_t)a[6], (void*)(uintptr_t)a[7], (void*)(uintptr_t)a[8], (void*)(uintptr_t)a[9], (void*)(uintptr_t)a[10], (void*)(uintptr_t)a[11], (void*)(uintptr_t)a[12], (void*)(uintptr_t)a[13], (void*)(uintptr_t)a[14], (void*)(uintptr_t)a[15], (void*)(uintptr_t)a[16], (void*)(uintptr_t)a[17], (int)(int64_t)a[18], (int)(int64_t)a[19], st);
 }
-static int ksmi_thunk_86(const void* fn, const uint64_t* a, void* st) {
+static int ksmi_thunk_88(const void* fn, const uint64_t* a, void* st) {
   typedef int (*F)(void*, void*, void*, void*, size_t, int, int, int, int, int, int, int, void*);
   (void)a; return ((F)fn)((void*)(uintptr_t)a[0], (void*)(uintptr_t)a[1], (void*)(uintptr_t)a[2], (void*)(uintptr_t)a[3], (size_t)a[4], (int)(int64_t)a[5], (int)(int64_t)a[6], (int)(int64_t)a[7], (int)(int64_t)a[8], (int)(int64_t)a[9], (int)(int64_t)a[10], (int)(int64_t)a[11], st);
 }
-static int ksmi_thunk_87(const void* fn, const uint64_t* a, void* st) {
+static int ksmi_thunk_89(const void* fn, const uint64_t* a, void* st) {
   typedef int (*F)(void*, size_t, void*);
   (void)a; return ((F)fn)((void*)(uintptr_t)a[0], (size_t)a[1], st);
 }
 
-static const int ksmi_n_thunks = 88;
-static const char* const ksmi_thunk_sigs[] = {"ipppfppiii", "ipppfpppiii", "ipppzp", "p", "pi", "pii", "piiidpppppffipppp", "piiidpppppffppppppppiiii", "piiiipppi", "piiiipppif", "piipppippppppdlii", "piipppipppppppdlii", "piipppipppppppidlii", "pipipiiiii", "pipippipiiii", "plipii", "pp", "ppi", "ppiiii", "ppiiiii", "ppiiiiii", "ppiiiiiiii", "ppiiiiiiiiiiii", "ppiiiiiiiiiiiii", "ppiiili", "ppiiilii", "ppilii", "ppipiiiiipppi", "ppippiiiiii", "ppippppiiiiipppi", "ppl", "ppli", "pplif", "pppfpppli", "pppi", "pppiiiifi", "pppiiiii", "pppiiiiifi", "pppiiiiifufupi", "pppiiiiii", "pppiiiiiii", "pppiiilii", "pppippiii", "pppippiiiii", "pppipppiii", "pppli", "ppplif", "pppliiufuufupi", "ppplpffff", "ppplufupi", "ppppiiii", "ppppiiiii", "ppppiiiiipppfi", "ppppiilf", "ppppiliufupi", "ppppliifi", "pppplpffffff", "pppplpffffffip", "pppppiiii", "pppppiiiii", "pppppiiiiii", "pppppiiiiufupi", "pppppiili", "pppppilii", "ppppplii", "ppppppiifi", "ppppppiiiifi", "ppppppiiiifuffuffuiiiip", "ppppppiiiii", "ppppppiiiiiii", "ppppppilii", "ppppppipiii", "pppppppdlii", "pppppppidlii", "pppppppiiiii", "pppppppiiiiifi", "pppppppiiiiifufupi", "pppppppiiiiiifi", "ppppppppdlifi", "ppppppppdlii", "ppppppppidlii", "ppppppppiiii", "pppppppppii", "ppppppppppiiiii", "pppppppppppiipiiiiiifi", "ppppppppppppppppppii", "ppppziiiiiii", "pz"};
-static const ksmi_thunk_fn ksmi_thunks[] = {ksmi_thunk_0, ksmi_thunk_1, ksmi_thunk_2, ksmi_thunk_3, ksmi_thunk_4, ksmi_thunk_5, ksmi_thunk_6, ksmi_thunk_7, ksmi_thunk_8, ksmi_thunk_9, ksmi_thunk_10, ksmi_thunk_11, ksmi_thunk_12, ksmi_thunk_13, ksmi_thunk_14, ksmi_thunk_15, ksmi_thunk_16, ksmi_thunk_17, ksmi_thunk_18, ksmi_thunk_19, ksmi_thunk_20, ksmi_thunk_21, ksmi_thunk_22, ksmi_thunk_23, ksmi_thunk_24, ksmi_thunk_25, ksmi_thunk_26, ksmi_thunk_27, ksmi_thunk_28, ksmi_thunk_29, ksmi_thunk_30, ksmi_thunk_31, ksmi_thunk_32, ksmi_thunk_33, ksmi_thunk_34, ksmi_thunk_35, ksmi_thunk_36, ksmi_thunk_37, ksmi_thunk_38, ksmi_thunk_39, ksmi_thunk_40, ksmi_thunk_41, ksmi_thunk_42, ksmi_thunk_43, ksmi_thunk_44, ksmi_thunk_45, ksmi_thunk_46, ksmi_thunk_47, ksmi_thunk_48, ksmi_thunk_49, ksmi_thunk_50, ksmi_thunk_51, ksmi_thunk_52, ksmi_thunk_53, ksmi_thunk_54, ksmi_thunk_55, ksmi_thunk_56, ksmi_thunk_57, ksmi_thunk_58, ksmi_thunk_59, ksmi_thunk_60, ksmi_thunk_61, ksmi_thunk_62, ksmi_thunk_63, ksmi_thunk_64, ksmi_thunk_65, ksmi_thunk_66, ksmi_thunk_67, ksmi_thunk_68, ksmi_thunk_69, ksmi_thunk_70, ksmi_thunk_71, ksmi_thunk_72, ksmi_thunk_73, ksmi_thunk_74, ksmi_thunk_75, ksmi_thunk_76, ksmi_thunk_77, ksmi_thunk_78, ksmi_thunk_79, ksmi_thunk_80, ksmi_thunk_81, ksmi_thunk_82, ksmi_thunk_83, ksmi_thunk_84, ksmi_thunk_85, ksmi_thunk_86, ksmi_thunk_87};
+static const int ksmi_n_thunks = 90;
+static const char* const ksmi_thunk_sigs[] = {"ipppfppiii", "ipppfpppiii", "ipppzp", "p", "pi", "pii", "piiidpppppffipppp", "piiidpppppffppppppppiiii", "piiiipppi", "piiiipppif", "piipppippppppdlii", "piipppipppppppdlii", "piipppipppppppidlii", "pipipiiiii", "pipippipiiii", "plipii", "pp", "ppi", "ppiiii", "ppiiiii", "ppiiiiii", "ppiiiiiiii", "ppiiiiiiiiiiii", "ppiiiiiiiiiiiii", "ppiiili", "ppiiilii", "ppilii", "ppipiiiiipppi", "ppippiiiiii", "ppippppiiiiipppi", "ppl", "ppli", "pplif", "pppfpppli", "pppi", "pppiiiifi", "pppiiiii", "pppiiiiifi", "pppiiiiifufupi", "pppiiiiii", "pppiiiiiii", "pppiiilii", "pppippiii", "pppippiiiii", "pppipppiii", "pppipppppiiii", "pppli", "ppplif", "pppliiufuufupi", "ppplpffff", "ppplufupi", "ppppiiii", "ppppiiiii", "ppppiiiiipppfi", "ppppiilf", "ppppiliufupi", "ppppliifi", "pppplpffffff", "pppplpffffffip", "pppppiiii", "pppppiiiii", "pppppiiiiii", "pppppiiiiufupi", "pppppiili", "pppppilii", "ppppplii", "ppppppiifi", "ppppppiiiifi", "ppppppiiiifuffuffuiiiip", "ppppppiiiii", "ppppppiiiiiii", "ppppppilii", "ppppppipiii", "pppppppdlii", "pppppppidlii", "pppppppiiiii", "pppppppiiiiifi", "pppppppiiiiifufupi", "pppppppiiiiiifi", "ppppppppdlifi", "ppppppppdlii", "ppppppppidlii", "ppppppppiiii", "pppppppppii", "ppppppppppiiiii", "pppppppppppiipiiiiiifi", "ppppppppppppiiiii", "ppppppppppppppppppii", "ppppziiiiiii", "pz"};
+static const ksmi_thunk_fn ksmi_thunks[] = {ksmi_thunk_0, ksmi_thunk_1, ksmi_thunk_2, ksmi_thunk_3, ksmi_thunk_4, ksmi_thunk_5, ksmi_thunk_6, ksmi_thunk_7, ksmi_thunk_8, ksmi_thunk_9, ksmi_thunk_10, ksmi_thunk_11, ksmi_thunk_12, ksmi_thunk_13, ksmi_thunk_14, ksmi_thunk_15, ksmi_thunk_16, ksmi_thunk_17, ksmi_thunk_18, ksmi_thunk_19, ksmi_thunk_20, ksmi_thunk_21, ksmi_thunk_22, ksmi_thunk_23, ksmi_thunk_24, ksmi_thunk_25, ksmi_thunk_26, ksmi_thunk_27, ksmi_thunk_28, ksmi_thunk_29, ksmi_thunk_30, ksmi_thunk_31, ksmi_thunk_32, ksmi_thunk_33, ksmi_thunk_34, ksmi_thunk_35, ksmi_thunk_36, ksmi_thunk_37, ksmi_thunk_38, ksmi_thunk_39, ksmi_thunk_40, ksmi_thunk_41, ksmi_thunk_42, ksmi_thunk_43, ksmi_thunk_44, ksmi_thunk_45, ksmi_thunk_46, ksmi_thunk_47, ksmi_thunk_48, ksmi_thunk_49, ksmi_thunk_50, ksmi_thunk_51, ksmi_thunk_52, ksmi_thunk_53, ksmi_thunk_54, ksmi_thunk_55, ksmi_thunk_56, ksmi_thunk_57, ksmi_thunk_58, ksmi_thunk_59, ksmi_thunk_60, ksmi_thunk_61, ksmi_thunk_62, ksmi_thunk_63, ksmi_thunk_64, ksmi_thunk_65, ksmi_thunk_66, ksmi_thunk_67, ksmi_thunk_68, ksmi_thunk_69, ksmi_thunk_70, ksmi_thunk_71, ksmi_thunk_72, ksmi_thunk_73, ksmi_thunk_74, ksmi_thunk_75, ksmi_thunk_76, ksmi_thunk_77, ksmi_thunk_78, ksmi_thunk_79, ksmi_thunk_80, ksmi_thunk_81, ksmi_thunk_82, ksmi_thunk_83, ksmi_thunk_84, ksmi_thunk_85, ksmi_thunk_86, ksmi_thunk_87, ksmi_thunk_88, ksmi_thunk_89};
diff --git a/kurosiwo_amd/runtime.py b/kurosiwo_amd/runtime.py
--- a/kurosiwo_amd/runtime.py
+++ b/kurosiwo_amd/runtime.py
@@ -39,6 +39,7 @@
         self.g = None
         self.needs_grad = needs_grad
         self.ginit = False
+        self.nwrites = 0
         self.consumers = []
         self.dtype, self.device = dtype, device
 
@@ -50,6 +51,7 @@
     def take_acc_flag(self):
         acc = 1 if self.ginit else 0
         self.ginit = True
+        self.nwrites += 1
         return acc
 
 
diff --git a/kurosiwo_amd/snunet_plan.py b/kurosiwo_amd/snunet_plan.py
--- a/kurosiwo_amd/snunet_plan.py
+++ b/kurosiwo_amd/snunet_plan.py
@@ -40,6 +40,7 @@
         self.logits = torch.empty((B, 3, H, W), dtype=torch.float32, device=self.dev)
         self.dlogits = torch.empty_like(self.logits) if with_backward else None
         self.bwd_builders = []
+        self.block_bwd = {}
 
         def A(name, lvl, ch):
             return Act(name, B, H >> lvl, W >> lvl, ch, dtype, self.dev)
@@ -119,6 +120,13 @@
         self.fwd.add_wait(src, dst)
         a, b = back
         self.bwd_builders.append((0, lambda: self.bwd.add_wait(a, b)))
+
+    def _gate_of(self, act):
+        src = getattr(act, "gate_src", None)
+        if (src is None or getattr(act, "consumers", []) or os.environ.get("KSMI_NO_GATE") is not None
+                or os.environ.get("KSMI_GATE_REST", "1") == "0" or self.sync_bn or not self.bn_fused or self.dtype != torch.bfloat16):
+            return None
+        return src
 
     def _rows(self, npix):
         return max(1, min(512, npix // 256))
@@ -265,7 +273,20 @@
             gy = y.grad()
             s2 = [SrcSpec(gy, Cc)]
             acc = x.take_acc_flag()
-            if up_gemm:
+            gsrc = self._gate_of(x) if up_gemm else None
+            grows = self.lib.ksmi_up_dgrad_gate_rows(B, H, W, Cc) if gsrc is not None else 0
+            if grows > 0 and self.lib.ksmi_bn_fused_supported(Cc, Cc, self.dt):
+                assert not acc and x.gated is None, f"{name}: the gated input gradient must be the only producer of d {x.name}"
+                g_out, g_z, g_sv = gsrc
+                gx = x.grad()
+                st = torch.empty(grows * 2 * Cc, dtype=torch.float32, device=self.dev)
+                self.keep.append(st)
+                self.bwd.add("ksmi_up_dgrad_gated", lambda: (gy.data_ptr(), wb.data_ptr(), gx.data_ptr(), 0, g_out.data_ptr(), g_z.data_ptr(),
+                                                             g_sv.mean, g_sv.rstd, st.data_ptr(), B, H, W, Cc),
+                             {"kind": "up_gemm_dgrad_gated", "bytes": B * H * W * Cc * 7 * es, "flops": 2 * B * H * W * Cc * 4 * Cc,
+                              "tag": f"K={4 * Cc} N={Cc} {H}x{W}"})
+                x.gated = (st, grows, Cc)
+            elif up_gemm:
                 gx = x.grad()
                 self.bwd.add("ksmi_up_dgrad", lambda: (gy.data_ptr(), wb.data_ptr(), gx.data_ptr(), acc, B, H, W, Cc),
                              {"kind": "up_gemm_dgrad", "bytes": B * H * W * Cc * (5 + acc) * es, "flops": 2 * B * H * W * Cc * 4 * Cc,
@@ -384,10 +405,15 @@
             self.fwd.add("ksmi_bn_add_relu", lambda: (z_act.t.data_ptr(), i_act.t.data_ptr(), sv2.scale, sv2.shift,
                                                       out.t.data_ptr(), npix, Cc, dt))
 
+        out.gate_src, out.gated = (out.t, z_act.t, sv2), None
+
         def build_bwd():
             self._level(H)
             gated = self._emit_dgrad(out, gate=(out.t, z_act.t, sv2)) if os.environ.get("KSMI_NO_GATE") is None else self._emit_dgrad(out)
             gated = gated if isinstance(gated, tuple) else None
+            if out.gated is not None:
+                assert gated is None and out.nwrites == 1, f"{name}: d {out.name} has a second producer behind the gating one"
+                gated = out.gated
             rows = self._rows(npix)
             self.need(sR, rows * 2 * Cc * 4)
             sums1 = torch.zeros((2, Cc), dtype=torch.float32, device=self.dev)
@@ -395,6 +421,7 @@
             dz = torch.empty_like(z_act.t)
             r = torch.empty_like(i_act.t)
             self.keep += [sums1, sums2, dz, r]
+            self.block_bwd[f"{name}{branch}"] = (out, dz)
             gout = out.grad().data_ptr()
             s1p, s2p = sums1.data_ptr(), sums2.data_ptr()
             a_bn2 = self._acc_param(f"{name}.bn2")
@@ -522,8 +549,7 @@
             ws_b = torch.empty(self.lib.ksmi_ecam_bwd_workspace(B, HW, n, 3), dtype=torch.uint8, device=dev)
             ws_m = torch.empty(self.lib.ksmi_ecam_mlp_bwd_workspace(B, n), dtype=torch.uint8, device=dev)
             garr = (C.c_void_p * 4)(*[a.grad().data_ptr() for a in xs])
-            for a in xs:
-                a.take_acc_flag()
+            accs = [a.take_acc_flag() for a in xs]
             for key in ("conv_final.weight", "conv_final.bias", "ca.fc1.weight", "ca.fc2.weight", "ca1.fc1.weight", "ca1.fc2.weight"):
                 self._acc_param(key)
             self.keep += [dca, dca1, davg, dmax, ws_b, ws_m, garr]
@@ -538,9 +564,23 @@
                 P("ca.fc1.weight"), P("ca.fc2.weight"), P("ca1.fc1.weight"), P("ca1.fc2.weight"), davg.data_ptr(), dmax.data_ptr(),
                 G("ca.fc1.weight"), G("ca.fc2.weight"), G("ca1.fc1.weight"), G("ca1.fc2.weight"), ws_m.data_ptr(), B, n))
             self._mark("ca.fc1.weight", "ca.fc2.weight", "ca1.fc1.weight", "ca1.fc2.weight")
-            self.bwd.add("ksmi_ecam_final_backward_dx", lambda: (
-                garr, dl, ca.data_ptr(), P("conv_final.weight"), davg.data_ptr(), dmax.data_ptr(), argmax.data_ptr(), B, HW, n, 3, dt),
-                {"kind": "ecam_final_backward_dx", "bytes": 4 * T0 + B * HW * 3 * 4, "flops": 2 * B * HW * 4 * n * 3})
+            x3 = xs[3]
+            gsrc = self._gate_of(x3)
+            grows = self.lib.ksmi_ecam_gate_rows(B, HW, n, dt) if gsrc is not None else 0
+            if grows > 0 and self.lib.ksmi_bn_fused_supported(n, n, dt):
+                assert x3.gated is None and not accs[3], f"head: the gated dx must be the only producer of d {x3.name}"
+                g_out, g_z, g_sv = gsrc
+                st = torch.empty(grows * 2 * n, dtype=torch.float32, device=dev)
+                self.keep.append(st)
+                self.bwd.add("ksmi_ecam_final_backward_dx_gated", lambda: (
+                    garr, dl, ca.data_ptr(), P("conv_final.weight"), davg.data_ptr(), dmax.data_ptr(), argmax.data_ptr(),
+                    g_out.data_ptr(), g_z.data_ptr(), g_sv.mean, g_sv.rstd, st.data_ptr(), B, HW, n, 3, dt),
+                    {"kind": "ecam_final_backward_dx_gated", "bytes": 6 * T0 + B * HW * 3 * 4, "flops": 2 * B * HW * 4 * n * 3})
+                x3.gated = (st, grows, n)
+            else:
+                self.bwd.add("ksmi_ecam_final_backward_dx", lambda: (
+                    garr, dl, ca.data_ptr(), P("conv_final.weight"), davg.data_ptr(), dmax.data_ptr(), argmax.data_ptr(), B, HW, n, 3, dt),
+                    {"kind": "ecam_final_backward_dx", "bytes": 4 * T0 + B * HW * 3 * 4, "flops": 2 * B * HW * 4 * n * 3})
         self.bwd_builders.append((self.fwd.cur_lane, build_bwd))
 
     def run_forward(self, xA, xB, tail=None):
```

Result: no change. 2183 tiles/s, median of 6 (+0.3%).
